# DerekRowell/AudioSDR

Hardware: AMD Instinct MI355X
Metric: Msamples/s through full SSB demod chain, batched 128-sample blocks (higher is better)
Workload: dtype f32

## Files before the change

audiosdr_amd/binding.py:

```python
import ctypes as C
import os

import numpy as np

BLOCK = 128
ALL = -1
STREAM_BATCH = (1 << 64) - 1
LSBmode, USBmode, CW_LSBmode, CW_USBmode, AMmode, SAMmode, WSPRmode = range(7)
(audioAM, audioCW, audioWSPR, audio2100, audio2300, audio2500, audio2700, audio2900, audio3100, audio3300,
 audioBypass) = range(11)
AGCoff, AGCfast, AGCmedium, AGCslow = range(4)
TAPS = ["SCALED_I", "SCALED_Q", "NB_I", "NB_Q", "IF_I", "IF_Q", "MIX_I", "MIX_Q", "DEMOD", "AUDIO_FILT", "AGC", "ALS"]

_HERE = os.path.dirname(os.path.abspath(__file__))


class AsdrError(RuntimeError):
    pass


def library_path():
    return os.path.join(_HERE, "libasdr_hip.so")


def library_sha256(path=None):
    import hashlib
    with open(path or library_path(), "rb") as f:
        return hashlib.sha256(f.read()).hexdigest()


_f, _i, _u = C.c_float, C.c_int, C.c_uint
_SETTERS_VOID = ["init", "enableAudioFilter", "disableAudioFilter", "enableALSfilter", "disableALSfilter",
                 "setALSfilterNotch", "setALSfilterPeak", "setALSfilterAdaptive", "setALSfilterStatic", "enableAGC",
                 "disableAGC", "enableNoiseBlanker", "disableNoiseBlanker"]
_SETTERS_F = ["setInputGain", "setIQgainBalance", "setOutputGain", "setAGCthreshold", "setAGCslope", "setAGCkneeWidth",
              "setAGCattackTime", "setAGCreleaseTime", "setAGChangTime", "setAGCstaticGain", "setNoiseBlankerThreshold",
              "setNoiseBlankerThresholdDb"]
_SETTERS_I = ["setMute", "setAudioFilter", "setAGCmode"]
_GETTERS_F = ["getTuningOffset", "getBPFlower", "getBPFupper", "getAGCthreshold", "getAGCslope", "getAGCkneeWidth",
              "getAGCattack", "getAGCrelease", "getAAGalphaAttack", "getAGCbetaAttack", "getAGCalphaRelease",
              "getAGCbetaRelease", "getAGCstaticGain", "getAMcarrierLevel", "getSAMfrequency"]
_GETTERS_I = ["getMute", "getAudioFilter", "ALSfilterIsEnabled", "ALSfilterIsNotch", "ALSfilterIsPeak",
              "ALSfilterIsAdaptive", "AGCisEnabled", "AGCisActive", "NoiseBlankerisEnabled", "NoiseBlankerDetection",
              "getSAMphaseLockStatus"]

EXPORTS = (["asdr_create", "asdr_destroy", "asdr_last_error", "asdr_n_channels", "asdr_update", "asdr_update_device",
            "asdr_synchronize", "asdr_setDemodMode", "asdr_getDemodMode", "asdr_setALSfilterParams", "asdr_getAGClookup",
            "asdr_read_status", "asdr_control_plane_flush", "asdr_params_uniform_groups", "asdr_get_chain_constants", "asdr_stream_pipeline_launches", "asdr_schedule_layout", "asdr_set_exact_unknown_mode", "asdr_get_exact_unknown_mode", "asdr_stream_pipeline_recoveries", "asdr_stream_pipeline_max_groups", "asdr_set_stream_fir_helpers", "asdr_stream_pipeline_h3_calls", "asdr_set_stream_pipeline", "asdr_set_sam_launch_form", "asdr_set_als_launch_form", "asdr_debug_set_stream_spin_limit", "asdr_debug_set_stream_max_groups", "asdr_enable_taps", "asdr_read_taps", "asdr_last_kernel_ms", "asdr_version",
            "asdr_kernel_timing_begin", "asdr_kernel_timing_end", "asdr_set_launch_timing", "asdr_region_timing_begin", "asdr_region_timing_end", "asdr_update_device_strided", "asdr_capture_open",
            "asdr_capture_close", "asdr_capture_capacity", "asdr_capture_position", "asdr_capture_rewind",
            "asdr_capture_device_ptr", "asdr_capture_update_device", "asdr_capture_read",
            "asdr_create_sharded", "asdr_n_shards", "asdr_shard", "asdr_shard_first_channel", "asdr_shard_device",
            "asdr_host_alloc", "asdr_host_free", "asdr_host_register", "asdr_host_unregister", "asdr_set_host_chunks",
            "asdr_host_path_info", "asdr_stream_pipeline_alloc_failures", "asdr_set_launch_split", "asdr_order_after", "asdr_order_before", "asdr_lane_calls", "asdr_sam_role_calls", "asdr_sam_chunk_calls", "asdr_als_role_calls", "asdr_set_lanes"] +
           ["asdr_" + n for n in _SETTERS_VOID + _SETTERS_F + _SETTERS_I + _GETTERS_F + _GETTERS_I])

_lib = None


def host_autopin(on=-1):
    return int(load_library().asdr_host_autopin(int(on)))


def host_autopin_clear():
    load_library().asdr_host_autopin_clear()


def host_autopin_info():
    out = (C.c_long * 4)()
    load_library().asdr_host_autopin_info(out)
    return {"registered_now": int(out[0]), "registrations": int(out[1]), "released": int(out[2]), "refused": int(out[3])}


def kernels_launched(reset=False):
    L = load_library()
    out = {}
    for i in range(L.asdr_kernels_count()):
        n = int(L.asdr_kernels_launches(i))
        if n:
            out[L.asdr_kernels_name(i).decode()] = n
    if reset:
        L.asdr_kernels_launches_reset()
    return out


def load_library(path=None):
    global _lib
    if _lib is not None and path is None:
        return _lib
    p = path or library_path()
    if not os.path.exists(p):
        raise AsdrError("%s not found: build it with `python -m audiosdr_amd.build` (hipcc, gfx950). "
                        "There is no CPU fallback." % p)
    L = C.CDLL(p)
    vp, i16p = C.c_void_p, C.POINTER(C.c_int16)
    L.asdr_create.argtypes = [_i, _i]; L.asdr_create.restype = vp
    L.asdr_destroy.argtypes = [vp]; L.asdr_destroy.restype = None
    L.asdr_last_error.restype = C.c_char_p
    L.asdr_version.restype = C.c_char_p
    L.asdr_set_pool_priority.argtypes = [_i]; L.asdr_set_pool_priority.restype = _i
    L.asdr_host_autopin.argtypes = [_i]; L.asdr_host_autopin.restype = _i
    L.asdr_host_autopin_clear.restype = None
    L.asdr_host_autopin_info.argtypes = [C.POINTER(C.c_long)]; L.asdr_host_autopin_info.restype = _i
    L.asdr_kernels_count.restype = _i
    L.asdr_kernels_name.argtypes = [_i]; L.asdr_kernels_name.restype = C.c_char_p
    L.asdr_kernels_launches.argtypes = [_i]; L.asdr_kernels_launches.restype = C.c_ulonglong
    L.asdr_kernels_launches_reset.restype = None
    L.asdr_n_channels.argtypes = [vp]; L.asdr_n_channels.restype = _i
    L.asdr_update.argtypes = [vp, i16p, i16p, i16p, _i]; L.asdr_update.restype = _i
    L.asdr_update_device.argtypes = [vp, vp, vp, vp, _i, vp]; L.asdr_update_device.restype = _i
    L.asdr_synchronize.argtypes = [vp]; L.asdr_synchronize.restype = _i
    L.asdr_update_device_strided.argtypes = [vp, vp, vp, vp, _i, C.c_long, C.c_long, vp]; L.asdr_update_device_strided.restype = _i
    L.asdr_capture_open.argtypes = [vp, C.c_long]; L.asdr_capture_open.restype = _i
    for n in ("asdr_capture_close", "asdr_capture_rewind"):
        getattr(L, n).argtypes = [vp]; getattr(L, n).restype = _i
    for n in ("asdr_capture_capacity", "asdr_capture_position"):
        getattr(L, n).argtypes = [vp]; getattr(L, n).restype = C.c_long
    L.asdr_capture_device_ptr.argtypes = [vp]; L.asdr_capture_device_ptr.restype = vp
    L.asdr_capture_update_device.argtypes = [vp, vp, vp, _i, C.c_long, vp]; L.asdr_capture_update_device.restype = _i
    L.asdr_capture_read.argtypes = [vp, _i, C.c_long, C.c_long, i16p]; L.asdr_capture_read.restype = _i
    L.asdr_last_kernel_ms.argtypes = [vp]; L.asdr_last_kernel_ms.restype = _f
    for n in _SETTERS_VOID:
        fn = getattr(L, "asdr_" + n); fn.argtypes = [vp, _i]; fn.restype = None
    for n in _SETTERS_F:
        fn = getattr(L, "asdr_" + n); fn.argtypes = [vp, _i, _f]; fn.restype = None
    for n in _SETTERS_I:
        fn = getattr(L, "asdr_" + n); fn.argtypes = [vp, _i, _i]; fn.restype = None
    for n in _GETTERS_F:
        fn = getattr(L, "asdr_" + n); fn.argtypes = [vp, _i]; fn.restype = _f
    for n in _GETTERS_I:
        fn = getattr(L, "asdr_" + n); fn.argtypes = [vp, _i]; fn.restype = _i
    L.asdr_setDemodMode.argtypes = [vp, _i, _i]; L.asdr_setDemodMode.restype = _f
    L.asdr_getDemodMode.argtypes = [vp, _i]; L.asdr_getDemodMode.restype = C.c_int16
    L.asdr_setALSfilterParams.argtypes = [vp, _i, _u, _f, _f]; L.asdr_setALSfilterParams.restype = None
    L.asdr_getAGClookup.argtypes = [vp, _i, _i]; L.asdr_getAGClookup.restype = _f
    i32p, fp = C.POINTER(C.c_int32), C.POINTER(C.c_float)
    L.asdr_read_status.argtypes = [vp, i32p, i32p, i32p, fp, fp]; L.asdr_read_status.restype = _i
    if path is None or hasattr(L, "asdr_get_chain_constants"):
        L.asdr_get_chain_constants.argtypes = [vp, _i, C.POINTER(C.c_float)]; L.asdr_get_chain_constants.restype = C.c_uint
    if path is None or hasattr(L, "asdr_control_plane_flush"):
        L.asdr_control_plane_flush.argtypes = [vp, C.POINTER(C.c_longlong)]; L.asdr_control_plane_flush.restype = _i
    if path is None or hasattr(L, "asdr_params_uniform_groups"):
        L.asdr_params_uniform_groups.argtypes = [vp, C.POINTER(C.c_long)]; L.asdr_params_uniform_groups.restype = _i
    L.asdr_enable_taps.argtypes = [vp, _i]; L.asdr_enable_taps.restype = _i
    L.asdr_read_taps.argtypes = [vp, fp]; L.asdr_read_taps.restype = _i
    L.asdr_kernel_timing_begin.argtypes = [vp, _i]; L.asdr_kernel_timing_begin.restype = _i
    if path is None or hasattr(L, "asdr_stream_pipeline_launches"):
        L.asdr_stream_pipeline_launches.argtypes = [vp]; L.asdr_stream_pipeline_launches.restype = C.c_long
    if path is None or hasattr(L, "asdr_set_stream_pipeline"):
        L.asdr_stream_pipeline_recoveries.argtypes = [vp]; L.asdr_stream_pipeline_recoveries.restype = C.c_long
        L.asdr_stream_pipeline_max_groups.argtypes = [vp]; L.asdr_stream_pipeline_max_groups.restype = _i
        if hasattr(L, "asdr_set_stream_fir_helpers"):
            L.asdr_set_stream_fir_helpers.argtypes = [vp, _i]; L.asdr_set_stream_fir_helpers.restype = _i
            L.asdr_stream_pipeline_h3_calls.argtypes = [vp]; L.asdr_stream_pipeline_h3_calls.restype = C.c_long
        L.asdr_set_stream_pipeline.argtypes = [vp, _i]; L.asdr_set_stream_pipeline.restype = _i
        L.asdr_set_sam_launch_form.argtypes = [vp, _i, _i]; L.asdr_set_sam_launch_form.restype = _i
        if hasattr(L, "asdr_set_als_launch_form"):
            L.asdr_set_als_launch_form.argtypes = [vp, _i]; L.asdr_set_als_launch_form.restype = _i
        L.asdr_debug_set_stream_spin_limit.argtypes = [vp, _u]; L.asdr_debug_set_stream_spin_limit.restype = _i
        L.asdr_debug_set_stream_max_groups.argtypes = [vp, _i]; L.asdr_debug_set_stream_max_groups.restype = _i
    if path is None or hasattr(L, "asdr_set_exact_unknown_mode"):
        L.asdr_set_exact_unknown_mode.argtypes = [vp, _i]; L.asdr_set_exact_unknown_mode.restype = _i
        L.asdr_get_exact_unknown_mode.argtypes = [vp]; L.asdr_get_exact_unknown_mode.restype = _i
    if path is None or hasattr(L, "asdr_schedule_layout"):
        L.asdr_schedule_layout.argtypes = [vp, C.POINTER(C.c_int)]; L.asdr_schedule_layout.restype = _i
    if path is None or hasattr(L, "asdr_region_timing_begin"):
        L.asdr_set_launch_timing.argtypes = [vp, _i]; L.asdr_set_launch_timing.restype = _i
        L.asdr_region_timing_begin.argtypes = [vp, vp]; L.asdr_region_timing_begin.restype = _i
        L.asdr_region_timing_end.argtypes = [vp, C.POINTER(C.c_float), C.POINTER(C.c_long)]; L.asdr_region_timing_end.restype = _i
    L.asdr_kernel_timing_end.argtypes = [vp, fp, _i]; L.asdr_kernel_timing_end.restype = _i
    if path is None or hasattr(L, "asdr_create_sharded"):
        L.asdr_create_sharded.argtypes = [_i, _i, C.POINTER(C.c_int)]; L.asdr_create_sharded.restype = vp
        L.asdr_n_shards.argtypes = [vp]; L.asdr_n_shards.restype = _i
        L.asdr_shard.argtypes = [vp, _i]; L.asdr_shard.restype = vp
        L.asdr_shard_first_channel.argtypes = [vp, _i]; L.asdr_shard_first_channel.restype = _i
        L.asdr_shard_device.argtypes = [vp, _i]; L.asdr_shard_device.restype = _i
        L.asdr_host_alloc.argtypes = [C.c_size_t]; L.asdr_host_alloc.restype = vp
        L.asdr_host_free.argtypes = [vp]; L.asdr_host_free.restype = None
        L.asdr_host_register.argtypes = [vp, C.c_size_t]; L.asdr_host_register.restype = _i
        L.asdr_host_unregister.argtypes = [vp]; L.asdr_host_unregister.restype = _i
        L.asdr_set_host_chunks.argtypes = [vp, _i]; L.asdr_set_host_chunks.restype = _i
        L.asdr_host_path_info.argtypes = [vp, C.POINTER(C.c_int)]; L.asdr_host_path_info.restype = _i
        L.asdr_stream_pipeline_alloc_failures.argtypes = [vp]; L.asdr_stream_pipeline_alloc_failures.restype = C.c_long
        L.asdr_set_launch_split.argtypes = [vp, _i, _i]; L.asdr_set_launch_split.restype = _i
        L.asdr_order_after.argtypes = [vp, vp]; L.asdr_order_after.restype = _i
        L.asdr_order_before.argtypes = [vp, vp]; L.asdr_order_before.restype = _i
        L.asdr_lane_calls.argtypes = [vp]; L.asdr_lane_calls.restype = C.c_long
        L.asdr_sam_role_calls.argtypes = [vp]; L.asdr_sam_role_calls.restype = C.c_long
        L.asdr_als_role_calls.argtypes = [vp]; L.asdr_als_role_calls.restype = C.c_long
        L.asdr_sam_chunk_calls.argtypes = [vp]; L.asdr_sam_chunk_calls.restype = C.c_long
        L.asdr_set_lanes.argtypes = [vp, _i, _i]; L.asdr_set_lanes.restype = _i
    if path is None or hasattr(L, "asdr_lanes_overlap_probe"):
        L.asdr_lanes_overlap_probe.argtypes = [vp]; L.asdr_lanes_overlap_probe.restype = _i
        L.asdr_lanes_enabled.argtypes = [vp]; L.asdr_lanes_enabled.restype = _i
        L.asdr_stream_pipeline_headroom_refusals.argtypes = [vp]; L.asdr_stream_pipeline_headroom_refusals.restype = C.c_long
    if path is None:
        _lib = L
    return L


class AudioSDRBatch:

    def __init__(self, n_channels, device=0, devices=None, _handle=None, _owner=None):
        self._L = load_library()
        self._owner = _owner
        if _handle is not None:
            self._h = _handle
        elif devices is not None:
            devs = (C.c_int * len(devices))(*[int(d) for d in devices])
            self._h = self._L.asdr_create_sharded(int(n_channels), len(devices), devs)
        else:
            self._h = self._L.asdr_create(int(n_channels), int(device))
        if not self._h:
            raise AsdrError("asdr_create failed: " + self._L.asdr_last_error().decode())
        self.n_channels = int(n_channels)
        self.device = int(device) if devices is None else None

    def close(self):
        if getattr(self, "_h", None):
            if self._owner is None:
                self._L.asdr_destroy(self._h)
            self._h = None

    @property
    def n_shards(self):
        return int(self._L.asdr_n_shards(self._h))

    def shard(self, g):
        h = self._L.asdr_shard(self._h, int(g))
        if not h:
            raise AsdrError("no such shard")
        lo, hi = self.shard_range(g)
        v = AudioSDRBatch(hi - lo, device=self._L.asdr_shard_device(self._h, int(g)), _handle=h, _owner=self)
        return v

    def shard_range(self, g):
        return int(self._L.asdr_shard_first_channel(self._h, int(g))), int(self._L.asdr_shard_first_channel(self._h, int(g) + 1))

    def order_after(self, stream):
        self._chk(self._L.asdr_order_after(self._h, C.c_void_p(stream)))

    def order_before(self, stream):
        self._chk(self._L.asdr_order_before(self._h, C.c_void_p(stream)))

    def lane_calls(self):
        return int(self._L.asdr_lane_calls(self._h))

    def sam_role_calls(self):
        return int(self._L.asdr_sam_role_calls(self._h))

    def sam_chunk_calls(self):
        return int(self._L.asdr_sam_chunk_calls(self._h))

    def als_role_calls(self):
        return int(self._L.asdr_als_role_calls(self._h))

    def lanes_overlap_probe(self):
        return int(self._L.asdr_lanes_overlap_probe(self._h))

    def lanes_enabled(self):
        return bool(self._L.asdr_lanes_enabled(self._h))

    def stream_pipeline_headroom_refusals(self):
        return int(self._L.asdr_stream_pipeline_headroom_refusals(self._h))

    def set_lanes(self, on=True, min_waves=0):
        self._chk(self._L.asdr_set_lanes(self._h, 1 if on else 0, int(min_waves)))

    def set_launch_split(self, pieces, min_waves=0):
        self._chk(self._L.asdr_set_launch_split(self._h, int(pieces), int(min_waves)))

    def set_host_chunks(self, chunks):
        self._chk(self._L.asdr_set_host_chunks(self._h, int(chunks)))

    def host_path_info(self):
        out = (C.c_int * 2)()
        self._chk(self._L.asdr_host_path_info(self._h, out))
        return {"chunks": int(out[0]), "pinned": bool(out[1])}

    def stream_pipeline_alloc_failures(self):
        return int(self._L.asdr_stream_pipeline_alloc_failures(self._h))

    def update_into(self, I, Q, out):
        n_blocks = I.size // (self.n_channels * BLOCK)
        p = C.POINTER(C.c_int16)
        self._chk(self._L.asdr_update(self._h, I.ctypes.data_as(p), Q.ctypes.data_as(p), out.ctypes.data_as(p), n_blocks))
        return out

    def __del__(self):
        try:
            self.close()
        except Exception:
            pass

    def _chk(self, rc):
        if rc != 0:
            raise AsdrError(self._L.asdr_last_error().decode())

    def update(self, I, Q):
        I = np.ascontiguousarray(I, dtype=np.int16)
        Q = np.ascontiguousarray(Q, dtype=np.int16)
        assert I.shape == Q.shape and I.size % (self.n_channels * BLOCK) == 0
        n_blocks = I.size // (self.n_channels * BLOCK)
        out = np.empty((self.n_channels, n_blocks, BLOCK), dtype=np.int16)
        p = C.POINTER(C.c_int16)
        self._chk(self._L.asdr_update(self._h, I.ctypes.data_as(p), Q.ctypes.data_as(p), out.ctypes.data_as(p), n_blocks))
        return out

    def update_device(self, dI, dQ, dOut, n_blocks, stream=0):
        self._chk(self._L.asdr_update_device(self._h, C.c_void_p(dI), C.c_void_p(dQ), C.c_void_p(dOut), int(n_blocks),
                                             C.c_void_p(stream)))

    def update_device_strided(self, dI, dQ, dOut, n_blocks, in_stride_blocks, out_stride_blocks, stream=0):
        self._chk(self._L.asdr_update_device_strided(self._h, C.c_void_p(dI), C.c_void_p(dQ), C.c_void_p(dOut), int(n_blocks),
                                                     int(in_stride_blocks), int(out_stride_blocks), C.c_void_p(stream)))

    def synchronize(self):
        self._chk(self._L.asdr_synchronize(self._h))

    def capture_open(self, capacity_blocks):
        self._chk(self._L.asdr_capture_open(self._h, int(capacity_blocks)))

    def capture_close(self):
        self._chk(self._L.asdr_capture_close(self._h))

    def capture_rewind(self):
        self._chk(self._L.asdr_capture_rewind(self._h))

    @property
    def capture_position(self):
        return int(self._L.asdr_capture_position(self._h))

    @property
    def capture_capacity(self):
        return int(self._L.asdr_capture_capacity(self._h))

    def capture_device_ptr(self):
        return int(self._L.asdr_capture_device_ptr(self._h) or 0)

    def capture_update_device(self, dI, dQ, n_blocks, in_stride_blocks=None, stream=0):
        self._chk(self._L.asdr_capture_update_device(self._h, C.c_void_p(dI), C.c_void_p(dQ), int(n_blocks),
                                                     int(n_blocks if in_stride_blocks is None else in_stride_blocks), C.c_void_p(stream)))

    def capture_read(self, ch, first_block=0, n_blocks=None):
        if n_blocks is None:
            n_blocks = self.capture_position - first_block
        out = np.empty(int(n_blocks) * BLOCK, dtype=np.int16)
        self._chk(self._L.asdr_capture_read(self._h, int(ch), int(first_block), int(n_blocks), out.ctypes.data_as(C.POINTER(C.c_int16))))
# ... 165 lines not shown
```

audiosdr_amd/csrc/asdr_device.h:

```cpp
#ifndef ASDR_DEVICE_H_
#define ASDR_DEVICE_H_

#include <stdint.h>

#define ASDR_N 128
#define ASDR_PLL_WRAP_MAX 64

#define ASDR_F_NB_EN        (1u << 0)
#define ASDR_F_AF_EN        (1u << 1)
#define ASDR_F_AGC_EN       (1u << 2)
#define ASDR_F_ALS_EN       (1u << 3)
#define ASDR_F_ALS_NOTCH    (1u << 4)
#define ASDR_F_ALS_ADAPTIVE (1u << 5)
#define ASDR_F_MUTED        (1u << 6)

#define ASDR_R_IF   (1u << 0)
#define ASDR_R_AF   (1u << 1)
#define ASDR_R_NB   (1u << 2)
#define ASDR_R_ALS  (1u << 3)
#define ASDR_R_IMG  (1u << 4)
#define ASDR_R_ALL  (1u << 5)

typedef struct {
  uint32_t mode;
// ... 31 lines not shown
} ChanSmall;

#define ASDR_S_AGC_ACTIVE  (1u << 0)
#define ASDR_S_NB_DETECTED (1u << 1)
#define ASDR_S_PLL_LOCKED  (1u << 2)

#define ASDR_NB_MASK_ROW 160
#define ASDR_NB_MASK_USED 138
#define ASDR_AGC_TAB_ROW 132

typedef struct {
  double inv_two_pi_d;
  double sin_index_scale_d;
  double half_pi_d;
  float if_center;
  float two_pi_f;
  float half_pi_f;
  float phase_inc_unit;
  float nb_alpha, nb_beta;
  float pll_b0, pll_b1, pll_a1;
  float pll_alpha_freq, pll_beta_freq, pll_f_conv, pll_lock_lo, pll_lock_hi;
} ChainConsts;

typedef struct {
  int32_t ch;
  uint32_t mode, flags;
  uint32_t lo;
} SlotInfo;
#define ASDR_LO_ENTRIES 8
#define ASDR_LO_WRITER 0x100u
#define ASDR_LO_WRITER_LANE(l) (0x100u << (l))

typedef struct {
  uint32_t key_phase, key_inc;
  float phase_end;
  uint32_t pad_;
  float c[ASDR_N], s[ASDR_N];
} LoEntry;

typedef struct {
  const ChanParams *params;
  ChanSmall *small;
  int16_t *nb_hist;
  uint8_t *nb_mask;
  float *hil_q, *hil_i, *als_x, *als_w;
  float *audio_prev;
  const float *agc_tab;
  const SlotInfo *sched;
  int32_t n_sched;
  int32_t n_channels;
  const int16_t *in_i, *in_q;
  int16_t *out;
  int32_t n_blocks;
  uint32_t nb_phase;
  uint32_t als_phase;
  LoEntry *lo_cache;
  uint32_t lo_parity;
  uint32_t lo_write;
  uint32_t lo_writer_bit;
  uint32_t direct_lo;
  int32_t direct_ch0;
  uint32_t direct_mode, direct_flags;
  int32_t in_stride;
  int32_t out_stride;
  float *taps;
  float *xch_a;
  float *xch_b;
  float *xch_c;
  uint32_t *stream_prog;
  uint32_t *stream_err;
  uint32_t stream_spin_limit;
  const uint32_t *run_if;
  int32_t stream_waves;
  float *xch_sam;
  uint32_t *sam_lock;
  uint32_t sam_set, sam_sets;
  uint32_t sam_set_stride, sam_lock_stride;
  float *als_stage;
  uint32_t als_stage_cur, als_stage_prev;
  LoEntry *lo_ring;
  ChainConsts k;
  ChanParams uni;
  uint32_t uni_valid;
  uint32_t pad_uni_;
} UpdateArgs;
#define ASDR_ALS_STAGE_SLOTS 32
#define ASDR_ALS_CHUNK 8
#define ASDR_STREAM_DEPTH 4
#define ASDR_LO_RING 8
#define ASDR_STREAM_SPIN_LIMIT (1u << 18)
#define ASDR_STREAM_FAIL 0xFFFFFFFFu
#define ASDR_SNAP_BYTES (448 + 1536 + ASDR_NB_MASK_ROW + 1024 + 1024 + 512)

#define ASDR_KERNEL_PLAIN 0
#define ASDR_KERNEL_SAM 1
#define ASDR_KERNEL_ALS 2
#define ASDR_KERNEL_ALS_SMALL 3
#define ASDR_KERNEL_SAM_ALS 4
#define ASDR_KERNEL_KINDS 5
#ifndef ASDR_SAM_WAVES
#define ASDR_SAM_WAVES 4
#endif

#endif
```

audiosdr_amd/csrc/asdr_host.cpp:

```cpp
#include <hip/hip_runtime.h>

#include <algorithm>
#include <atomic>
#include <chrono>
#include <condition_variable>
#include <functional>
#include <memory>
#include <mutex>
#include <thread>
#include <cmath>
#include <cstdio>
#include <cstring>
#include <string>
#include <unordered_map>
#include <vector>

#include "../../include/asdr.h"
#include "asdr_device.h"
#include "asdr_tables.h"

#ifndef ASDR_SAM_CHUNK
#define ASDR_SAM_CHUNK 8
#define ASDR_SAM_CHUNK_SETS 32
#define ASDR_SAM_CHUNK_MAX_WAVES 512
#endif
#ifndef ASDR_ALS_ROLE_MAX_WAVES
#define ASDR_ALS_ROLE_MAX_WAVES 512
#endif
#ifndef ASDR_PER_BLOCK_LAUNCH_WAVES
#define ASDR_PER_BLOCK_LAUNCH_WAVES 1024
#endif
#ifndef ASDR_STREAM_MAX_WAVES
#define ASDR_STREAM_MAX_WAVES 1024
#endif
#ifndef ASDR_STREAM_MIN_BLOCKS
#define ASDR_STREAM_MIN_BLOCKS 8
#endif
#ifndef ASDR_STREAM_SIDE_MARGIN
#define ASDR_STREAM_SIDE_MARGIN 16
#endif
#ifndef ASDR_STREAM_SIDE_WAVES
#define ASDR_STREAM_SIDE_WAVES 64
#endif
extern "C" int asdr_launch_stream(const UpdateArgs *a, hipStream_t stream, int fir_helpers);
extern "C" int asdr_stream_capacity(int device, int *compute_units, int fir_helpers);
extern "C" int asdr_launch_stream_snapshot(const UpdateArgs *a, void *snap, int restore, hipStream_t stream);
extern "C" int asdr_launch_stream_ack(uint32_t *err, hipStream_t stream);
extern "C" int asdr_kernels_upload_tables(void);
namespace { void autopin_batch_created(); void autopin_batch_gone(); }
extern "C" int asdr_launch_update(const UpdateArgs *a, int variant, int uniform, hipStream_t stream);
extern "C" int asdr_launch_sam_role(const UpdateArgs *a, int variant, int uniform, int role, hipStream_t stream);
extern "C" int asdr_launch_als_role(const UpdateArgs *a, int role, hipStream_t stream);
extern "C" int asdr_launch_als_stage_seed(const UpdateArgs *a, int ch0, int n, hipStream_t stream);
extern "C" int asdr_launch_reset(const UpdateArgs *a, const uint32_t *d_reset_bits, int first_row, int n_rows, hipStream_t stream);

namespace {

constexpr double kPI = 3.1415926535897932384626433832795;
constexpr float kFs = 44100.0f;
constexpr float kIFcenter = 6890.0f, kBWssb = 3000.0f, kBWcw = 1000.0f, kBWwspr = 1000.0f, kBWam = 8500.0f;

thread_local std::string g_err;
int fail(const std::string &m) { g_err = m; return -1; }
#define HIPCHK(expr)                                                                                   \
  do {                                                                                                 \
    hipError_t e_ = (expr);                                                                            \
    if (e_ != hipSuccess) return fail(std::string(#expr) + ": " + hipGetErrorString(e_));              \
  } while (0)

struct Chan {
  float in_gain = 1.0f, in_gain_i = 1.0f, in_gain_q = 1.0f, gain_balance = 1.0f;
  float output_gain = 0.5f, out_gain = 1.0f, current_out_gain = 1.0f;
  float freq_shift = 0.0f;
  uint16_t mode = 0;
  bool muted = true;
  int16_t current_filter = 0;
  bool af_en = false;
  int if_table = ASDR_TBL_IF_SSB, audio_table = ASDR_TBL_AUDIO_BASE + ASDR_audio2700;
  int16_t als_m = 55, als_delay = 3;
  float als_lambda = 0.5f;
  bool als_en = false, als_notch = true, als_adaptive = true;
  float agc_alpha_att = 0, agc_beta_att = 0, agc_alpha_rel = 0, agc_beta_rel = 0;
  float agc_attack_ms = 0, agc_release_ms = 0, agc_knee = 0, agc_slope = 0, agc_threshold = 0;
  float agc_static_gain = 10.0f;
  float agc_slot129 = 100.0f;
  uint32_t agc_hang_count = 0;
  bool agc_en = true;
  int agc_table = -1;
  float nb_threshold = 1.2f;
  bool nb_en = true;
};

struct AgcTable {
  float thr, slope, knee;
  float v[ASDR_AGC_TAB_ROW];
};

float log2_approx(float input) {
  int exponent;
  float mantissa = frexpf(fabsf(input), &exponent);
  return (((1.23149591368684f * mantissa - 4.11852516267426f) * mantissa + 6.02197014179219f) * mantissa -
          3.13396450166353f) + exponent;
}

void build_agc_table(AgcTable &t) {
  const float thr = t.thr, slope = t.slope, knee = t.knee;
  const float lin_lo = expf((float)(2.3025 * ((double)thr - (double)knee / 2.0) / 20.0));
  const float lin_hi = expf((float)(2.3025 * ((double)thr + (double)knee / 2.0) / 20.0));
  for (int i = 0; i < 130; i++) {
    const float input = (float)((double)(float)i / 128.0);
    const float in_db = (float)(6.026 * (double)log2_approx(input));
    if (input < lin_lo) {
      t.v[i] = 1.0f;
    } else if (input > lin_hi) {
      const float out_db = thr + (in_db - thr) * slope;
      t.v[i] = expf((float)(2.3025 * (double)(out_db - in_db) / 20.0));
    } else {
      const double u = (double)(in_db - thr) + (double)knee / 2.0;
      const float out_db = (float)((double)in_db + (((double)slope - 1.0) * u * u) / (2.0 * (double)knee));
      t.v[i] = expf((float)(2.3025 * (double)(out_db - in_db) / 20.0));
    }
  }
  t.v[130] = t.v[131] = 0.0f;
}

float time_constant(float ms) {
  return (float)exp(log(0.1) / ((double)(kFs * ms) / 1000.0));
}

}

namespace {
class CopyPool {
// ... 77 lines not shown
  size_t agc_tab_cap = 0;
  SlotInfo *d_sched = nullptr;
  uint32_t *d_reset = nullptr;
  int16_t *d_io[3] = {nullptr, nullptr, nullptr};
  int16_t *h_io[3] = {nullptr, nullptr, nullptr};
  size_t h_io_cap = 0;
  hipStream_t h2d_stream = nullptr, d2h_stream = nullptr;
  std::vector<hipEvent_t> ev_host;
  HostPlan host_plan;
  std::unique_ptr<CopyPool> copy_pool;
  int host_chunks_forced = 0;
  hipStream_t lane[ASDR_LANES + 1] = {};
  hipEvent_t ev_lane[ASDR_LANES + 1] = {};
  int n_lanes = 2, n_lanes_sam = 3;
  int sched_lanes = 2;
  bool lanes_pending = false;
  bool sched_sam_heavy = false;
  bool last_was_lanes = false;
  int lanes_min_waves = 1024;
  bool lanes_enabled = true;
  bool lanes_forced = false;
  long stat_lane_calls = 0;
  int launch_split = 1, launch_split_min_waves = 2048;
  int stat_host_chunks = 0, stat_host_pinned = 0;
  std::vector<asdr_batch *> shards;
  std::vector<int> shard_first;
  void *workers = nullptr;
  int16_t *d_capture = nullptr;
  long capture_cap = 0, capture_pos = 0;
  size_t io_cap = 0;
  bool taps_on = false;
  hipEvent_t ev0 = nullptr, ev1 = nullptr;
  bool ev_valid = false;
  bool time_calls = false;
  hipEvent_t rev0 = nullptr, rev1 = nullptr;
  hipStream_t region_stream = nullptr;
  bool region_on_lanes = false;
  long region_calls = -1;
  std::vector<hipEvent_t> tev;
  size_t tev_used = 0;
  hipStream_t last_stream = nullptr;
  hipEvent_t ev_last = nullptr;
  hipStream_t aux[ASDR_AUX_STREAMS] = {};
  hipEvent_t ev_fork = nullptr, ev_join[ASDR_AUX_STREAMS] = {};
  bool ev_last_valid = false;
  LoEntry *d_lo = nullptr;
  float *d_xch_a = nullptr, *d_xch_b = nullptr;
  uint32_t *d_stream_prog = nullptr;
  LoEntry *d_lo_ring = nullptr;
  bool sam_fused = false;
  int sam_split_min = 512;
  bool stream_pipeline = true;
  int stream_query_waves = 0;
  int stream_max_waves = 0;
  int stream_cap_workgroups = 0;
  int stream_cap_h3 = 0, stream_cus = 0;
  int stream_h3 = -1;
  long stat_stream_h3_calls = 0;
  uint32_t stream_spin_limit = ASDR_STREAM_SPIN_LIMIT;
  void *d_stream_snap = nullptr;
  long stat_stream_recoveries = 0;
  bool sam_split = false;
  int als_split_min = 0x7fffffff;
  bool als_split = false;
  float *d_xch_sam = nullptr;
  size_t xch_sam_slots = 0;
  hipEvent_t ev_role[6] = {};
  bool sam_role_streams = true;
  long stat_sam_role_calls = 0;
  float *d_xch_sam_chunk = nullptr; size_t xch_sam_chunk_slots = 0;
  long stat_sam_chunk_calls = 0;
  hipEvent_t ev_samc[3 * (ASDR_SAM_CHUNK_SETS / ASDR_SAM_CHUNK)] = {};
  float *d_als_stage = nullptr;
  hipEvent_t ev_als[3 * (ASDR_ALS_STAGE_SLOTS / ASDR_ALS_CHUNK)] = {};
  int als_role_stages = 3;
  bool als_role_streams = true;
  long stat_als_role_calls = 0;
  bool plain_uniform_ssb = false;
  bool stream_launched = false;
  long stat_stream_launches = 0;
  long stat_stream_headroom_refusals = 0;
  long stat_stream_alloc_failures = 0;
  uint32_t lo_parity = 0;
  uint32_t nb_phase = 0;
  uint32_t als_phase = 0;
  ChainConsts k{};
};

namespace {

int sharded_update(asdr_batch *b, const int16_t *I, const int16_t *Q, int16_t *out, int n_blocks);
void shard_workers_stop(asdr_batch *b);
inline bool is_sharded(const asdr_batch *b);

uint64_t agc_hash(float thr, float slope, float knee) {
  uint32_t a, b2, c;
  memcpy(&a, &thr, 4); memcpy(&b2, &slope, 4); memcpy(&c, &knee, 4);
  uint64_t h = 1469598103934665603ull;
  for (uint32_t w : {a, b2, c}) { h ^= w; h *= 1099511628211ull; }
  return h;
}

int find_agc_table(asdr_batch *b, float thr, float slope, float knee) {
  std::vector<int> &bucket = b->agc_index[agc_hash(thr, slope, knee)];
  for (int i : bucket) {
    const AgcTable &t = b->agc_pool[i];
    if (memcmp(&t.thr, &thr, 4) == 0 && memcmp(&t.slope, &slope, 4) == 0 && memcmp(&t.knee, &knee, 4) == 0) return i;
  }
  AgcTable t;
  t.thr = thr; t.slope = slope; t.knee = knee;
  build_agc_table(t);
  b->agc_pool.push_back(t);
  b->agc_refs.push_back(0);
  bucket.push_back((int)b->agc_pool.size() - 1);
  b->agc_pool_dirty = true;
  return (int)b->agc_pool.size() - 1;
}

void rebuild_agc(asdr_batch *b, Chan &c) {
  const int old = c.agc_table;
  c.agc_table = find_agc_table(b, c.agc_threshold, c.agc_slope, c.agc_knee);
  b->agc_refs[c.agc_table]++;
  b->agc_refs_changed = true;
  if (old >= 0 && old < (int)b->agc_refs.size() && b->agc_refs[old] > 0) b->agc_refs[old]--;
  c.agc_slot129 = b->agc_pool[c.agc_table].v[129];
}

void compact_agc_pool(asdr_batch *b) {
  if (!b->agc_refs_changed) return;
  b->agc_refs_changed = false;
  size_t live = 0;
  for (uint32_t r : b->agc_refs) live += (r != 0);
  if (b->agc_pool.size() < 64 || b->agc_pool.size() <= 2 * live) return;
  std::vector<int> remap(b->agc_pool.size(), -1);
  std::vector<AgcTable> pool;
  std::vector<uint32_t> refs;
  for (size_t i = 0; i < b->agc_pool.size(); i++)
    if (b->agc_refs[i]) { remap[i] = (int)pool.size(); pool.push_back(b->agc_pool[i]); refs.push_back(b->agc_refs[i]); }
  b->agc_pool.swap(pool); b->agc_refs.swap(refs);
  b->agc_index.clear();
  for (size_t i = 0; i < b->agc_pool.size(); i++) b->agc_index[agc_hash(b->agc_pool[i].thr, b->agc_pool[i].slope, b->agc_pool[i].knee)].push_back((int)i);
  for (Chan &c : b->ch) c.agc_table = remap[c.agc_table];
  b->agc_pool_dirty = true; b->all_dirty = true; b->sched_dirty = true;
}

void mark_reset(asdr_batch *b, int i, uint32_t bits) {
  b->reset[i] |= bits;
  b->reset_pending = true;
  if (i < b->reset_lo) b->reset_lo = i;
  if (i > b->reset_hi) b->reset_hi = i;
}

float set_mode(asdr_batch *b, int idx, int new_mode) {
  Chan &c = b->ch[idx];
  c.mode = (uint16_t)new_mode;
  int tbl = -1;
  if (c.mode == ASDR_USBmode) { c.freq_shift = (float)((double)kIFcenter - (double)kBWssb / 2.0); tbl = ASDR_TBL_IF_SSB; }
  else if (c.mode == ASDR_LSBmode) { c.freq_shift = (float)((double)kIFcenter + (double)kBWssb / 2.0); tbl = ASDR_TBL_IF_SSB; }
  else if (c.mode == ASDR_WSPRmode) { c.freq_shift = (float)((double)kIFcenter - (double)kBWssb / 2.0); tbl = ASDR_TBL_IF_WSPR; }
  else if (c.mode == ASDR_CW_USBmode) { c.freq_shift = (float)((double)kIFcenter - (double)kBWcw / 2.0); tbl = ASDR_TBL_IF_CW; }
  else if (c.mode == ASDR_CW_LSBmode) { c.freq_shift = (float)((double)kIFcenter + (double)kBWcw / 2.0); tbl = ASDR_TBL_IF_CW; }
  else if (c.mode == ASDR_AMmode || c.mode == ASDR_SAMmode) { c.freq_shift = kIFcenter; tbl = ASDR_TBL_IF_AM; }
  if (tbl >= 0) { c.if_table = tbl; mark_reset(b, idx, ASDR_R_IF); }
  return c.freq_shift;
}

// ... 384 lines not shown
    ok = ok && hipStreamSynchronize(s0) == hipSuccess && hipStreamSynchronize(s1) == hipSuccess;
    ok = ok && hipEventElapsedTime(&one, ev[0], ev[1]) == hipSuccess && hipEventElapsedTime(&both, ev[0], ev[2]) == hipSuccess;
    if (!ok) break;
    rounds++;
    if (std::max(one, both) < 1.5f * alone) votes++;
  }
  for (hipEvent_t e : ev) if (e) (void)hipEventDestroy(e);
  if (!ok || rounds == 0) { (void)hipGetLastError(); return -1; }
  const int verdict = (2 * votes > rounds) ? 1 : 0;
  g_lanes_probe_last[device] = verdict;
  if (verdict == 1 || ++g_lanes_probe_tries[device] >= 3) g_lanes_probe[device] = verdict;
  return verdict;
}
hipStream_t aux_stream(asdr_batch *b, int i) {
  if (!b->aux[i]) b->aux[i] = pool_stream(b->device, i + 1);
  return b->aux[i];
}
hipStream_t lane_stream(asdr_batch *b, int l) {
  if (!b->lane[l]) b->lane[l] = pool_stream(b->device, l);
  return b->lane[l];
}
bool needs_flush(const asdr_batch *b) {
  return b->all_dirty || !b->dirty.empty() || b->sched_dirty || b->agc_pool_dirty || b->reset_pending || b->agc_refs_changed;
}
int lanes_join_into(asdr_batch *b, hipStream_t stream) {
  for (int i = 0; i <= b->sched_lanes; i++) {
    const int l = (i == b->sched_lanes) ? ASDR_LANES : i;
    if (!b->lane[l]) continue;
    HIPCHK(hipEventRecord(b->ev_lane[l], b->lane[l])); HIPCHK(hipStreamWaitEvent(stream, b->ev_lane[l], 0));
  }
  return 0;
}
int sync_all(asdr_batch *b) {
  HIPCHK(hipStreamSynchronize(b->last_stream));
  HIPCHK(hipStreamSynchronize(b->stream));
  if (b->lanes_pending) { for (int l = 0; l < ASDR_LANES + 1; l++) if (b->lane[l]) HIPCHK(hipStreamSynchronize(b->lane[l])); b->lanes_pending = false; }

  return 0;
}

int check_stream_error(asdr_batch *b) {
  if (!b->stream_launched || !b->d_stream_prog) return 0;
  if (sync_all(b) != 0) return -1;
  uint32_t *word = b->d_stream_prog + 3 * ((b->n + 7) / 8) + 1, v[2] = {0, 0};
  HIPCHK(hipMemcpy(v, word, sizeof v, hipMemcpyDeviceToHost));
  b->stream_launched = false;
  b->stat_stream_recoveries = (long)v[1];
  if (v[0]) return fail("streaming pipeline: error word still set after the recovery launches (internal error)");
  return 0;
}

int read_small(asdr_batch *b, int ch, ChanSmall &s) {
  if (!b || ch < 0 || ch >= b->n) return fail("bad channel");
  if (is_sharded(b)) b = shard_of(b, ch);
  if (b->device == ASDR_NO_DEVICE) return fail("control-plane-only batch has no device state");
  HIPCHK(hipSetDevice(b->device));
  if (sync_all(b) != 0) return -1;
  if (check_stream_error(b) != 0) return -1;
  if (apply_resets(b, b->stream) != 0) return -1;
  HIPCHK(hipMemcpy(&s, b->d_small + ch, sizeof s, hipMemcpyDeviceToHost));
  return 0;
}

}

#define FOR_SHARDS(b, call) do { if (is_sharded(b)) { for (asdr_batch *sh_ : (b)->shards) { const int rc_ = (call); if (rc_ != 0) return rc_; } return 0; } } while (0)

extern "C" {

const char *asdr_last_error(void) { return g_err.c_str(); }
}
int asdr_internal_fail(const std::string &m) { return fail(m); }
extern "C" {
const char *asdr_version(void) { return "asdr-hip 0.1 (gfx950, wave64, -ffp-contract=off)"; }

asdr_batch_t *asdr_create(int n_channels, int device) {
  if (n_channels <= 0 || n_channels > (1 << 20)) { fail("n_channels must be in 1..1048576"); return nullptr; }
  asdr_batch *b = new asdr_batch();
  b->n = n_channels; b->device = device;
  b->sam_fused = getenv("ASDR_SAM_FUSED") != nullptr;
  b->sam_split_min = getenv("ASDR_SAM_SPLIT_MIN") ? atoi(getenv("ASDR_SAM_SPLIT_MIN")) : ASDR_SAM_SPLIT_MIN_CHANNELS;
  b->stream_pipeline = getenv("ASDR_NO_STREAM_PIPELINE") == nullptr;
  b->uniform_params = getenv("ASDR_NO_UNIFORM_PARAMS") == nullptr;
  b->als_split_min = getenv("ASDR_ALS_SPLIT_MIN") ? atoi(getenv("ASDR_ALS_SPLIT_MIN")) : 0x7fffffff;
  if (getenv("ASDR_LAUNCH_SPLIT")) b->launch_split = std::max(1, std::min(atoi(getenv("ASDR_LAUNCH_SPLIT")), 8));
  if (getenv("ASDR_LAUNCH_SPLIT_MIN_WAVES")) b->launch_split_min_waves = std::max(8, atoi(getenv("ASDR_LAUNCH_SPLIT_MIN_WAVES")));
  const size_t rows = (size_t)n_channels + 1;
  if (device != ASDR_NO_DEVICE) {
    int ndev = 0;
    if (hipGetDeviceCount(&ndev) != hipSuccess || ndev <= 0) { delete b; fail("no HIP device: libasdr_hip has no CPU path"); return nullptr; }
    if (device < 0 || device >= ndev) { delete b; fail("bad device ordinal"); return nullptr; }
    if (device >= 16) { delete b; fail("device ordinal >= 16: the per-device stream pool of this library has 16 entries"); return nullptr; }
    if (hipSetDevice(device) != hipSuccess) { delete b; fail("hipSetDevice failed"); return nullptr; }
    autopin_batch_created();
    bool ok = true;
    auto alloc = [&](void **p, size_t bytes) { if (ok && hipMalloc(p, bytes) != hipSuccess) ok = false; };
    alloc((void **)&b->d_params, rows * sizeof(ChanParams));
    alloc((void **)&b->d_small, rows * sizeof(ChanSmall));
    alloc((void **)&b->d_nb_hist, rows * 768 * sizeof(int16_t));
    alloc((void **)&b->d_nb_mask, rows * ASDR_NB_MASK_ROW * sizeof(uint8_t));
    alloc((void **)&b->d_hil_q, rows * 256 * sizeof(float));
    alloc((void **)&b->d_hil_i, rows * 256 * sizeof(float));
    alloc((void **)&b->d_als_x, rows * 256 * sizeof(float));
    alloc((void **)&b->d_als_w, rows * 128 * sizeof(float));
    alloc((void **)&b->d_audio_prev, rows * 128 * sizeof(float));
    if (ok && hipMemset(b->d_audio_prev, 0, rows * 128 * sizeof(float)) != hipSuccess) ok = false;
    alloc((void **)&b->d_sched, (rows + 32) * sizeof(SlotInfo));
    alloc((void **)&b->d_reset, rows * sizeof(uint32_t));
    alloc((void **)&b->d_lo, (1 + ASDR_LANES) * 2 * ASDR_LO_ENTRIES * sizeof(LoEntry));
    if (ok && hipMemset(b->d_lo, 0xFF, (1 + ASDR_LANES) * 2 * ASDR_LO_ENTRIES * sizeof(LoEntry)) != hipSuccess) ok = false;
    if (ok && hipStreamSynchronize(nullptr) != hipSuccess) ok = false;
    for (int i = 0; i < ASDR_LANES + 1 && ok; i++)
      if (hipEventCreateWithFlags(&b->ev_lane[i], hipEventDisableTiming) != hipSuccess) ok = false;
    b->lanes_enabled = getenv("ASDR_NO_LANES") == nullptr;
    b->sam_role_streams = getenv("ASDR_NO_SAM_ROLE_STREAMS") == nullptr;
    b->als_role_streams = getenv("ASDR_NO_ALS_ROLE_STREAMS") == nullptr;
    if (getenv("ASDR_ALS_ROLE_STAGES")) b->als_role_stages = atoi(getenv("ASDR_ALS_ROLE_STAGES")) == 2 ? 2 : 3;
    if (ok && (b->stream = pool_stream(device, 0)) == nullptr) ok = false;
    if (ok && hipEventCreate(&b->ev0) != hipSuccess) ok = false;
    if (ok && hipEventCreate(&b->ev1) != hipSuccess) ok = false;
    if (ok && hipEventCreate(&b->rev0) != hipSuccess) ok = false;
    if (ok && hipEventCreate(&b->rev1) != hipSuccess) ok = false;
    if (ok && hipEventCreateWithFlags(&b->ev_last, hipEventDisableTiming) != hipSuccess) ok = false;
    if (ok && hipEventCreateWithFlags(&b->ev_fork, hipEventDisableTiming) != hipSuccess) ok = false;
    for (int i = 0; i < ASDR_AUX_STREAMS && ok; i++)
      if (hipEventCreateWithFlags(&b->ev_join[i], hipEventDisableTiming) != hipSuccess) ok = false;
    if (ok && asdr_kernels_upload_tables() != 0) ok = false;
    if (ok) {
      int cus = 0;
      const int cap = asdr_stream_capacity(device, &cus, 1);
      const int cap3 = asdr_stream_capacity(device, nullptr, 3);
      b->stream_cap_h3 = cap3 > 0 ? cap3 : 0; b->stream_cus = cus;
      { const char *e = getenv("ASDR_STREAM_H3"); if (e) b->stream_h3 = atoi(e) != 0 ? 1 : 0; }
      b->stream_cap_workgroups = cap > 0 ? cap : 0;
      b->stream_max_waves = cap >= 3 ? cap / 3 : 0;
      if (b->stream_max_waves > ASDR_STREAM_MAX_WAVES) b->stream_max_waves = ASDR_STREAM_MAX_WAVES;
      b->stream_query_waves = b->stream_max_waves;
    }
    if (!ok) { fail("device allocation / table upload failed"); asdr_destroy(b); return nullptr; }
  }

  ChainConsts &k = b->k;
  k.if_center = kIFcenter;
  k.two_pi_f = (float)(2.0 * kPI);
  k.half_pi_f = (float)(0.5 * kPI);
  k.inv_two_pi_d = 1.0 / (double)k.two_pi_f;
  k.sin_index_scale_d = (65535.0 / (double)k.two_pi_f) * (1.0 + 0x1p-49);
  k.half_pi_d = kPI / 2.0;
  k.phase_inc_unit = k.two_pi_f / kFs;
  k.nb_alpha = 0.995f;
  k.nb_beta = (float)(1.0 - (double)k.nb_alpha);
  {
    const float wn = 0.07f, zeta = 0.707f, Ka = 1000.f;
    const float tau1 = Ka / (wn * wn);
    const float tau2 = 2 * zeta / wn;
    k.pll_b0 = (float)((double)(2 * Ka / tau1) * (1.0 + 2.0 * (double)tau2));
    k.pll_b1 = (float)((double)(2 * Ka / tau1) * (1.0 - 2.0 * (double)tau2));
    k.pll_a1 = -1.0f;
  }
  k.pll_alpha_freq = 0.995f;
  k.pll_beta_freq = (float)(1.0 - (double)k.pll_alpha_freq);
  k.pll_f_conv = kFs / k.two_pi_f;
  k.pll_lock_lo = (float)((double)kIFcenter - 1000.0);
  k.pll_lock_hi = (float)((double)kIFcenter + 1000.0);

  b->ch.assign(rows, Chan());
// ... 165 lines not shown
  {
    const uintptr_t in_bytes = ((uintptr_t)(b->n - 1) * (uintptr_t)in_stride_blocks + (uintptr_t)n_blocks) * ASDR_N * sizeof(int16_t);
    const uintptr_t out_bytes = ((uintptr_t)(b->n - 1) * (uintptr_t)out_stride_blocks + (uintptr_t)n_blocks) * ASDR_N * sizeof(int16_t);
    const uintptr_t o0 = (uintptr_t)dOut, o1 = o0 + out_bytes;
    for (uintptr_t i0 : {(uintptr_t)dI, (uintptr_t)dQ}) io_alias = io_alias || (o0 < i0 + in_bytes && i0 < o1);
  }
  int pipe_sub = -1, other_waves = 0;
  for (int i = 0; i < n_sub; i++) { if (subs[i].kind == ASDR_KERNEL_PLAIN && subs[i].uniform) pipe_sub = i; else other_waves += subs[i].slots / 8; }
  bool take_pipeline = parts == 1 && b->stream_pipeline && !io_alias && n_blocks >= ASDR_STREAM_MIN_BLOCKS && pipe_sub >= 0 && b->plain_uniform_ssb &&
                       other_waves <= ASDR_STREAM_SIDE_WAVES && !sam_split && !als_split &&
#ifndef ASDR_TIMELINE
                       !b->taps_on &&
#endif
                       subs[pipe_sub].slots / 8 <= b->stream_max_waves;
  if (take_pipeline && other_waves > 0 && b->stream_cap_workgroups > 0 &&
      3 * (subs[pipe_sub].slots / 8) + other_waves + ASDR_STREAM_SIDE_MARGIN > b->stream_cap_workgroups) { take_pipeline = false; b->stat_stream_headroom_refusals++; }
  if (take_pipeline) {
    if (!b->d_xch_a) {
      float *xa = nullptr, *xb = nullptr; uint32_t *prog = nullptr; LoEntry *ring = nullptr; void *snap = nullptr;
      const size_t n_prog = (size_t)(3 * ((b->n + 7) / 8) + 3);
      bool ok = hipMalloc(&xa, (size_t)(b->n + 1) * ASDR_STREAM_DEPTH * 2 * ASDR_N * sizeof(float)) == hipSuccess &&
                hipMalloc(&xb, (size_t)(b->n + 1) * ASDR_STREAM_DEPTH * (ASDR_N + 1) * sizeof(float)) == hipSuccess &&
                hipMalloc(&prog, n_prog * sizeof(uint32_t)) == hipSuccess &&
                hipMalloc(&ring, ASDR_LO_RING * sizeof(LoEntry)) == hipSuccess &&
                hipMalloc(&snap, (size_t)(((b->n + 7) / 8) * 8) * ASDR_SNAP_BYTES) == hipSuccess &&
                hipMemsetAsync(prog, 0, n_prog * sizeof(uint32_t), stream) == hipSuccess;
      if (!ok) {
        for (void *p : {(void *)xa, (void *)xb, (void *)prog, (void *)ring, snap}) if (p) hipFree(p);
        (void)hipGetLastError();
        b->stream_pipeline = false; b->stat_stream_alloc_failures++; take_pipeline = false;
      } else {
        b->d_xch_a = xa; b->d_xch_b = xb; b->d_stream_prog = prog; b->d_lo_ring = ring; b->d_stream_snap = snap;
      }
    }
  }
  if (take_pipeline) {
    const UpdateArgs a_side = a;
    const int w = subs[pipe_sub].slots / 8;
    HIPCHK(hipMemsetAsync(b->d_stream_prog, 0, (size_t)(3 * w + 1) * sizeof(uint32_t), stream));
    if (n_sub > 1) HIPCHK(hipEventRecord(b->ev_fork, stream));
    a.sched = b->d_sched + subs[pipe_sub].first; a.n_sched = subs[pipe_sub].slots;
    a.direct_ch0 = -1; a.uni_valid = 0u;
    if (b->kind_direct[ASDR_KERNEL_PLAIN]) { const SlotInfo &s0 = b->sched[subs[pipe_sub].first]; a.direct_ch0 = s0.ch; a.direct_mode = s0.mode; a.direct_flags = s0.flags; a.direct_lo = s0.lo; set_uni(b, a, s0.ch); }
    a.lo_write = 0u;
    a.xch_a = b->d_xch_a; a.xch_b = b->d_xch_b; a.xch_c = b->d_xch_b + (size_t)(b->n + 1) * ASDR_STREAM_DEPTH * ASDR_N; a.stream_prog = b->d_stream_prog; a.stream_err = b->d_stream_prog + 3 * ((b->n + 7) / 8) + 1;
    a.stream_waves = w; a.lo_ring = b->d_lo_ring; a.stream_spin_limit = b->stream_spin_limit;
    if (e0) HIPCHK(hipEventRecord(e0, stream));
    if (asdr_launch_stream_snapshot(&a, b->d_stream_snap, 0, stream) != 0) return fail("stream snapshot launch failed");
    const bool h3 = b->stream_h3 != 0 && b->stream_cap_h3 > 0 && 3 * w + other_waves + ASDR_STREAM_SIDE_MARGIN <= b->stream_cap_h3 &&
                    (b->stream_h3 == 1 || 3 * w <= b->stream_cus);
    if (h3) b->stat_stream_h3_calls++;
    if (asdr_launch_stream(&a, stream, h3 ? 3 : 1) != 0) return fail("stream kernel launch failed");
    if (asdr_launch_stream_snapshot(&a, b->d_stream_snap, 1, stream) != 0) return fail("stream restore launch failed");
    {
      UpdateArgs f = a;
      f.run_if = a.stream_err; f.stream_waves = 0; f.xch_a = nullptr; f.xch_b = nullptr; f.xch_c = nullptr; f.stream_prog = nullptr; f.lo_ring = nullptr;
      if (asdr_launch_update(&f, ASDR_KERNEL_PLAIN, 1, stream) != 0) return fail("stream fallback launch failed");
    }
    if (asdr_launch_stream_ack(a.stream_err, stream) != 0) return fail("stream acknowledge launch failed");
    {
      int n_aux = 0;
      for (int i = 0; i < n_sub; i++) {
        if (i == pipe_sub) continue;
        hipStream_t s = aux_stream(b, n_aux++);
        if (!s) return fail("stream creation failed");
        HIPCHK(hipStreamWaitEvent(s, b->ev_fork, 0));
        UpdateArgs o = a_side;
        o.sched = b->d_sched + subs[i].first; o.n_sched = subs[i].slots; o.direct_ch0 = -1; o.uni_valid = 0u; o.lo_write = 1u;
        if (subs[i].uniform && b->kind_direct[subs[i].kind]) { const SlotInfo &s0 = b->sched[subs[i].first]; o.direct_ch0 = s0.ch; o.direct_mode = s0.mode; o.direct_flags = s0.flags; o.direct_lo = s0.lo; set_uni(b, o, s0.ch); }
        if (asdr_launch_update(&o, subs[i].kind, subs[i].uniform, s) != 0) return fail("update kernel launch failed");
        HIPCHK(hipEventRecord(b->ev_join[n_aux - 1], s));
      }
      for (int j = 0; j < n_aux; j++) HIPCHK(hipStreamWaitEvent(stream, b->ev_join[j], 0));
    }
    if (e1) HIPCHK(hipEventRecord(e1, stream));
    b->stream_launched = true; b->stat_stream_launches++;
    b->ev_last_valid = true;
    b->ev_valid = (e0 != nullptr && e0 == b->ev0);
    if (b->region_calls >= 0) b->region_calls++;
    b->last_stream = stream; b->last_was_lanes = false;
    b->nb_phase = (b->nb_phase + (uint32_t)(n_blocks % 3)) % 3u;
    b->als_phase = (b->als_phase + (uint32_t)n_blocks) & 1u;
    b->lo_parity ^= 1u;
    return 0;
  }
  const int n_launch = per_block ? n_blocks : 1;
  float *const taps = a.taps;
  if (e0 && part == 0) HIPCHK(hipEventRecord(e0, stream));
  if (use_lanes) {
    if (batch_stream) {
      if (b->ev_last_valid && !b->last_was_lanes) {
        HIPCHK(hipEventRecord(b->ev_last, b->last_stream));
        for (int i = 0; i <= b->sched_lanes; i++) { hipStream_t ls = lane_stream(b, i == b->sched_lanes ? ASDR_LANES : i); if (!ls) return fail("stream creation failed"); HIPCHK(hipStreamWaitEvent(ls, b->ev_last, 0)); }
      }
    } else {
      HIPCHK(hipEventRecord(b->ev_fork, stream));
      for (int i = 0; i <= b->sched_lanes; i++) { hipStream_t ls = lane_stream(b, i == b->sched_lanes ? ASDR_LANES : i); if (!ls) return fail("stream creation failed"); HIPCHK(hipStreamWaitEvent(ls, b->ev_fork, 0)); }
    }
    const int NL = b->sched_lanes;
    for (int l = 0; l <= NL; l++) {
      hipStream_t ls = lane_stream(b, (l == NL) ? ASDR_LANES : l);
      if (!ls) return fail("stream creation failed");
      for (int lb = 0; lb < n_launch; lb++) {
        for (int i = 0; i < n_sub; i++) {
          const Sub &su = subs[i];
          const long w = su.slots / 8;
          int lo = (int)(w * l / NL) * 8, cnt = (int)(w * (l + 1) / NL) * 8 - lo;
          if (l == NL) { lo = 0; cnt = su.uniform ? 0 : su.slots; } else if (!su.uniform) cnt = 0;
          const int first = su.first + lo;
          if (cnt == 0) continue;
          UpdateArgs al = a;
          al.sched = b->d_sched + first; al.n_sched = cnt;
          al.direct_ch0 = -1; al.uni_valid = 0u;
          if (su.uniform && b->kind_direct[su.kind]) { const SlotInfo &s0 = b->sched[su.first]; al.direct_ch0 = s0.ch + lo; al.direct_mode = s0.mode; al.direct_flags = s0.flags; al.direct_lo = s0.lo; set_uni(b, al, s0.ch); }
          al.lo_cache = b->d_lo + (size_t)(1 + (l % ASDR_LANES)) * 2 * ASDR_LO_ENTRIES;
          al.lo_write = 1u;
          al.lo_writer_bit = ASDR_LO_WRITER_LANE(l % ASDR_LANES);
          if (sam_split && (su.kind == ASDR_KERNEL_SAM || su.kind == ASDR_KERNEL_SAM_ALS)) set_sam_rows(al, su.kind, first, 0);
          const int form = (als_split && su.kind == ASDR_KERNEL_ALS_SMALL && su.uniform) ? 2 : su.uniform;
          if (per_block) {
            al.in_i = dI + (size_t)lb * ASDR_N; al.in_q = dQ + (size_t)lb * ASDR_N; al.out = dOut + (size_t)lb * ASDR_N; al.n_blocks = 1;
            al.nb_phase = (b->nb_phase + (uint32_t)(lb % 3)) % 3u;
            al.als_phase = (b->als_phase + (uint32_t)lb) & 1u;
            al.lo_parity = b->lo_parity ^ (uint32_t)(lb & 1);
          }
          if (asdr_launch_update(&al, su.kind, form, ls) != 0) return fail("update kernel launch failed");
        }
      }
    }
    if (!batch_stream) { if (lanes_join_into(b, stream) != 0) return -1; b->lanes_pending = false; b->last_was_lanes = false; b->last_stream = stream; }
    else { b->lanes_pending = true; b->last_was_lanes = true; }
    b->ev_last_valid = true; b->ev_valid = false; b->stat_lane_calls++;
    if (b->region_calls >= 0) b->region_calls++;
    b->nb_phase = (b->nb_phase + (uint32_t)(n_blocks % 3)) % 3u;
    b->als_phase = (b->als_phase + (uint32_t)n_blocks) & 1u;
    b->lo_parity ^= (uint32_t)(n_launch & 1);
    return 0;
  }
  struct Item { int sub, first, slots; };
  Item items[ASDR_AUX_STREAMS + 1]; int n_items = 0;
  for (int i = 0; i < n_sub; i++) {
    const long w = subs[i].slots / 8;
    const int lo = (int)(w * part / parts) * 8, cnt = (int)(w * (part + 1) / parts) * 8 - lo;
    if (cnt == 0) continue;
    int pieces = 1;
    if (b->launch_split > 1 && cnt / 8 >= b->launch_split_min_waves) pieces = std::min(b->launch_split, ASDR_AUX_STREAMS + 1 - n_items - (n_sub - 1 - i));
    if (pieces < 1) pieces = 1;
    for (int q = 0; q < pieces; q++) {
      const int qlo = (int)((long)(cnt / 8) * q / pieces) * 8, qhi = (int)((long)(cnt / 8) * (q + 1) / pieces) * 8;
      if (qhi > qlo && n_items < ASDR_AUX_STREAMS + 1) items[n_items++] = Item{i, subs[i].first + lo + qlo, qhi - qlo};
    }
  }
  int main_item = 0;
  for (int i = 1; i < n_items; i++) if (items[i].slots > items[main_item].slots) main_item = i;
  const bool sam_roles = b->sam_role_streams && per_block && n_launch >= 2 && parts == 1 && n_items == 1 && taps == nullptr && sam_split &&
                         (subs[items[0].sub].kind == ASDR_KERNEL_SAM || subs[items[0].sub].kind == ASDR_KERNEL_SAM_ALS);
  hipStream_t s_pre = nullptr, s_pll = nullptr;
  if (sam_roles) {
    s_pre = aux_stream(b, 0); s_pll = aux_stream(b, 1);
    if (!s_pre || !s_pll) return fail("stream creation failed");
    for (int i = 0; i < 6; i++) if (!b->ev_role[i]) HIPCHK(hipEventCreateWithFlags(&b->ev_role[i], hipEventDisableTiming));
    HIPCHK(hipEventRecord(b->ev_fork, stream));
    HIPCHK(hipStreamWaitEvent(s_pre, b->ev_fork, 0)); HIPCHK(hipStreamWaitEvent(s_pll, b->ev_fork, 0));
    b->stat_sam_role_calls++;
  }
  bool sam_chunks = sam_roles && subs[items[0].sub].kind == ASDR_KERNEL_SAM && subs[items[0].sub].uniform && n_blocks >= 2 * ASDR_SAM_CHUNK &&
                    items[0].slots <= 8 * ASDR_SAM_CHUNK_MAX_WAVES && getenv("ASDR_NO_SAM_CHUNKS") == nullptr;
  auto chunk_tiles = [&](int slots) -> bool {
    if ((size_t)slots <= b->xch_sam_chunk_slots) return true;
    if (hipStreamSynchronize(stream) != hipSuccess) return false;
    float *grown = nullptr;
    const size_t per_set = (size_t)slots * 2 * ASDR_N * sizeof(float) + (size_t)slots * sizeof(uint32_t);
    if (hipMalloc(&grown, ASDR_SAM_CHUNK_SETS * per_set) != hipSuccess) { (void)hipGetLastError(); return false; }
    if (b->d_xch_sam_chunk) hipFree(b->d_xch_sam_chunk);
    b->d_xch_sam_chunk = grown; b->xch_sam_chunk_slots = (size_t)slots;
    return true;
  };
  if (sam_chunks && !chunk_tiles(items[0].slots)) sam_chunks = false;
  int parity_launches_sam = -1;
  if (sam_chunks) {
    constexpr int S = ASDR_SAM_CHUNK_SETS, G = ASDR_SAM_CHUNK, R = S / G;
    static_assert(S % G == 0 && R >= 4, "tile sets for four chunks");
    for (int i = 0; i < 3 * R; i++) if (!b->ev_samc[i]) HIPCHK(hipEventCreateWithFlags(&b->ev_samc[i], hipEventDisableTiming));
    const int i0 = items[0].sub, first0 = items[0].first;
    const size_t slots = b->xch_sam_chunk_slots;
    a.sched = b->d_sched + first0; a.n_sched = items[0].slots; a.direct_ch0 = -1; a.uni_valid = 0u; a.lo_write = 1u;
    if (b->kind_direct[subs[i0].kind]) { const SlotInfo &s0 = b->sched[subs[i0].first]; a.direct_ch0 = s0.ch; a.direct_mode = s0.mode; a.direct_flags = s0.flags; a.direct_lo = s0.lo; set_uni(b, a, s0.ch); }
    a.xch_sam = b->d_xch_sam_chunk; a.sam_lock = reinterpret_cast<uint32_t *>(b->d_xch_sam_chunk + (size_t)S * slots * 2 * ASDR_N);
    a.sam_sets = (uint32_t)S; a.sam_set_stride = (uint32_t)(slots * 2 * ASDR_N); a.sam_lock_stride = (uint32_t)slots;
    a.taps = nullptr;
    const int n_chunks = (n_blocks + G - 1) / G;
    auto chunk_args = [&](int k) {
      const int b0 = k * G, g = (n_blocks - b0 < G) ? n_blocks - b0 : G;
      a.in_i = dI + (size_t)b0 * ASDR_N; a.in_q = dQ + (size_t)b0 * ASDR_N; a.out = dOut + (size_t)b0 * ASDR_N; a.n_blocks = g;
      a.nb_phase = (b->nb_phase + (uint32_t)(b0 % 3)) % 3u;
      a.als_phase = (b->als_phase + (uint32_t)b0) & 1u;
      a.lo_parity = b->lo_parity ^ (uint32_t)(k & 1);
      a.sam_set = (uint32_t)(b0 % S);
    };
    for (int k = 0; k <= n_chunks; k++) {
      if (k < n_chunks) {
        const int kr = k % R;
        chunk_args(k);
        if (asdr_launch_sam_role(&a, ASDR_KERNEL_SAM, 1, 0, stream) != 0) return fail("update kernel launch failed");
        HIPCHK(hipEventRecord(b->ev_samc[kr], stream)); HIPCHK(hipStreamWaitEvent(s_pll, b->ev_samc[kr], 0));
        if (asdr_launch_sam_role(&a, ASDR_KERNEL_SAM, 1, 1, s_pll) != 0) return fail("update kernel launch failed");
        HIPCHK(hipEventRecord(b->ev_samc[R + kr], s_pll));
      }
      if (k >= 1) {
        chunk_args(k - 1);
        HIPCHK(hipStreamWaitEvent(stream, b->ev_samc[R + (k - 1) % R], 0));
        if (asdr_launch_sam_role(&a, ASDR_KERNEL_SAM, 1, 2, stream) != 0) return fail("update kernel launch failed");
      }
    }
    parity_launches_sam = n_chunks;
    b->stat_sam_chunk_calls++;
  }
  const bool als_role_call = als_roles && n_items == 1 && taps == nullptr;
  int parity_launches = n_launch;
  if (als_role_call) {
    constexpr int S = ASDR_ALS_STAGE_SLOTS, G = ASDR_ALS_CHUNK, R = S / G;
    static_assert(S % G == 0 && R >= 3, "the stage holds at least three chunks");
    hipStream_t s_chain = aux_stream(b, 0);
    if (!s_chain) return fail("stream creation failed");
    for (int i = 0; i < 2 * R; i++) if (!b->ev_als[i]) HIPCHK(hipEventCreateWithFlags(&b->ev_als[i], hipEventDisableTiming));
    HIPCHK(hipEventRecord(b->ev_fork, stream));
    HIPCHK(hipStreamWaitEvent(s_chain, b->ev_fork, 0));
    const int i0 = items[0].sub, first0 = items[0].first;
    a.sched = b->d_sched + first0; a.n_sched = items[0].slots; a.direct_ch0 = -1; a.uni_valid = 0u; a.lo_write = 1u;
    if (b->kind_direct[subs[i0].kind]) { const SlotInfo &s0 = b->sched[subs[i0].first]; a.direct_ch0 = s0.ch; a.direct_mode = s0.mode; a.direct_flags = s0.flags; a.direct_lo = s0.lo; set_uni(b, a, s0.ch); }
    a.als_stage = b->d_als_stage; a.als_stage_cur = 0u; a.als_stage_prev = (uint32_t)(S - 1); a.als_phase = b->als_phase;
    if (asdr_launch_als_stage_seed(&a, 0, b->n, s_chain) != 0) return fail("update kernel launch failed");
    const int n_chunks = (n_blocks + G - 1) / G;
    static_assert(ASDR_SAM_CHUNK == ASDR_ALS_CHUNK, "the two chunked forms share the tile sets");
    constexpr int RT = ASDR_SAM_CHUNK_SETS / G;
    static_assert(RT == R, "the front stage's wait indexes ev_als[(k - RT) % R]: the event of back chunk k - RT only while tile sets and stage slots hold the same number of chunks");
    hipStream_t s_front = nullptr;
    bool three = b->als_role_stages == 3 && chunk_tiles(items[0].slots);
    if (three) { s_front = aux_stream(b, 1); if (!s_front) three = false; }
    if (three) {
      for (int i = 2 * R; i < 3 * R; i++) if (!b->ev_als[i]) HIPCHK(hipEventCreateWithFlags(&b->ev_als[i], hipEventDisableTiming));
      HIPCHK(hipStreamWaitEvent(s_front, b->ev_fork, 0));
      const size_t slots = b->xch_sam_chunk_slots;
      a.xch_sam = b->d_xch_sam_chunk; a.sam_lock = reinterpret_cast<uint32_t *>(b->d_xch_sam_chunk + (size_t)ASDR_SAM_CHUNK_SETS * slots * 2 * ASDR_N);
      a.sam_sets = (uint32_t)ASDR_SAM_CHUNK_SETS; a.sam_set_stride = (uint32_t)(slots * 2 * ASDR_N); a.sam_lock_stride = (uint32_t)slots;
    }
    for (int k = 0; k < n_chunks; k++) {
      const int b0 = k * G, g = (n_blocks - b0 < G) ? n_blocks - b0 : G;
      a.in_i = dI + (size_t)b0 * ASDR_N; a.in_q = dQ + (size_t)b0 * ASDR_N; a.out = dOut + (size_t)b0 * ASDR_N; a.n_blocks = g;
      a.nb_phase = (b->nb_phase + (uint32_t)(b0 % 3)) % 3u;
      a.als_phase = (b->als_phase + (uint32_t)b0) & 1u;
      a.lo_parity = b->lo_parity ^ (uint32_t)(k & 1);
      a.als_stage_cur = (uint32_t)(b0 % S); a.als_stage_prev = (uint32_t)((b0 + S - 1) % S);
      a.sam_set = (uint32_t)(b0 % ASDR_SAM_CHUNK_SETS);
      if (three) {
        if (k >= RT) HIPCHK(hipStreamWaitEvent(s_front, b->ev_als[(k - RT) % R], 0));
        if (asdr_launch_als_role(&a, 2, s_front) != 0) return fail("update kernel launch failed");
        HIPCHK(hipEventRecord(b->ev_als[2 * R + k % R], s_front)); HIPCHK(hipStreamWaitEvent(s_chain, b->ev_als[2 * R + k % R], 0));
      }
      if (k >= R - 1) HIPCHK(hipStreamWaitEvent(s_chain, b->ev_als[R + (k + 1) % R], 0));
      if (asdr_launch_als_role(&a, three ? 3 : 0, s_chain) != 0) return fail("update kernel launch failed");
      HIPCHK(hipEventRecord(b->ev_als[k % R], s_chain)); HIPCHK(hipStreamWaitEvent(stream, b->ev_als[k % R], 0));
      if (asdr_launch_als_role(&a, 1, stream) != 0) return fail("update kernel launch failed");
      HIPCHK(hipEventRecord(b->ev_als[R + k % R], stream));
    }
    parity_launches = n_chunks;
    b->stat_als_role_calls++;
  }
  if (parity_launches_sam >= 0) parity_launches = parity_launches_sam;
  for (int lb = 0; lb < ((als_role_call || sam_chunks) ? 0 : n_launch); lb++) {
    if (per_block) {
      a.in_i = dI + (size_t)lb * ASDR_N; a.in_q = dQ + (size_t)lb * ASDR_N; a.out = dOut + (size_t)lb * ASDR_N; a.n_blocks = 1;
      a.nb_phase = (b->nb_phase + (uint32_t)(lb % 3)) % 3u;
      a.als_phase = (b->als_phase + (uint32_t)lb) & 1u;
      a.lo_parity = b->lo_parity ^ (uint32_t)(lb & 1);
      a.taps = (lb == n_launch - 1) ? taps : nullptr;
    }
    if (n_items > 1) HIPCHK(hipEventRecord(b->ev_fork, stream));
    int n_aux = 0;
    for (int it = 0; it < n_items; it++) {
      const int i = items[it].sub, first = items[it].first;
      hipStream_t s = (it == main_item) ? stream : aux_stream(b, n_aux++);
      if (!s && it != main_item) return fail("stream creation failed");
      if (it != main_item) HIPCHK(hipStreamWaitEvent(s, b->ev_fork, 0));
      a.sched = b->d_sched + first; a.n_sched = items[it].slots;
      a.direct_ch0 = -1; a.uni_valid = 0u;
      a.lo_write = 1u;
      if (subs[i].uniform && b->kind_direct[subs[i].kind]) {
        const SlotInfo &s0 = b->sched[subs[i].first];
        a.direct_ch0 = s0.ch + (first - subs[i].first); a.direct_mode = s0.mode; a.direct_flags = s0.flags; a.direct_lo = s0.lo; set_uni(b, a, s0.ch);
        if (first != subs[i].first) a.lo_write = 0u;
      }
      const bool sam3 = sam_split && (subs[i].kind == ASDR_KERNEL_SAM || subs[i].kind == ASDR_KERNEL_SAM_ALS);
      if (sam3) set_sam_rows(a, subs[i].kind, first, sam_roles ? (lb & 1) : 0);
      const int form = (als_split && subs[i].kind == ASDR_KERNEL_ALS_SMALL && subs[i].uniform) ? 2 : subs[i].uniform;
      if (sam_roles) {
        const int pa = lb & 1;
        if (lb >= 2) HIPCHK(hipStreamWaitEvent(s_pre, b->ev_role[4 + pa], 0));
        if (asdr_launch_sam_role(&a, subs[i].kind, form, 0, s_pre) != 0) return fail("update kernel launch failed");
        HIPCHK(hipEventRecord(b->ev_role[pa], s_pre)); HIPCHK(hipStreamWaitEvent(s_pll, b->ev_role[pa], 0));
        if (asdr_launch_sam_role(&a, subs[i].kind, form, 1, s_pll) != 0) return fail("update kernel launch failed");
        HIPCHK(hipEventRecord(b->ev_role[2 + pa], s_pll)); HIPCHK(hipStreamWaitEvent(stream, b->ev_role[2 + pa], 0));
        if (asdr_launch_sam_role(&a, subs[i].kind, form, 2, stream) != 0) return fail("update kernel launch failed");
        HIPCHK(hipEventRecord(b->ev_role[4 + pa], stream));
        continue;
      }
      if (asdr_launch_update(&a, subs[i].kind, form, s) != 0) return fail("update kernel launch failed");
      if (it != main_item) HIPCHK(hipEventRecord(b->ev_join[n_aux - 1], s));
    }
    for (int j = 0; j < n_aux; j++) HIPCHK(hipStreamWaitEvent(stream, b->ev_join[j], 0));
  }
  if (part + 1 < parts) return 0;
  if (e1) HIPCHK(hipEventRecord(e1, stream));
  b->ev_last_valid = true;
  b->ev_valid = (e0 != nullptr && e0 == b->ev0);
  if (b->region_calls >= 0) b->region_calls++;
  b->last_stream = stream; b->last_was_lanes = false;
  b->nb_phase = (b->nb_phase + (uint32_t)(n_blocks % 3)) % 3u;
  b->als_phase = (b->als_phase + (uint32_t)n_blocks) & 1u;
  b->lo_parity ^= (uint32_t)(parity_launches & 1);
  return 0;
}

extern "C" {
int asdr_update_device_strided(asdr_batch_t *b, const int16_t *dI, const int16_t *dQ, int16_t *dOut, int n_blocks,
                               long in_stride_blocks, long out_stride_blocks, void *stream_) {
  if (is_sharded(b)) {
    if (!dI || !dQ) return 0;
    if (!dOut) return fail("null output");
    for (asdr_batch *sh : b->shards) if (sh->device != b->shards[0]->device || sh->device == ASDR_NO_DEVICE)
      return fail("sharded batch over several devices: device pointers go to the shards (asdr_shard), host rows to asdr_update");
    for (size_t g = 0; g < b->shards.size(); g++) {
      const size_t f = (size_t)b->shard_first[g];
      if (update_device_part(b->shards[g], dI + f * (size_t)in_stride_blocks * ASDR_N, dQ + f * (size_t)in_stride_blocks * ASDR_N,
                             dOut + f * (size_t)out_stride_blocks * ASDR_N, n_blocks, in_stride_blocks, out_stride_blocks, stream_, 0, 1) != 0) return -1;
    }
    return 0;
  }
  return update_device_part(b, dI, dQ, dOut, n_blocks, in_stride_blocks, out_stride_blocks, stream_, 0, 1);
}

int asdr_update_device(asdr_batch_t *b, const int16_t *dI, const int16_t *dQ, int16_t *dOut, int n_blocks, void *stream_) {
  return asdr_update_device_strided(b, dI, dQ, dOut, n_blocks, n_blocks, n_blocks, stream_);
}

int asdr_capture_open(asdr_batch_t *b, long capacity_blocks) {
  if (!b) return fail("null batch");
  FOR_SHARDS(b, asdr_capture_open(sh_, capacity_blocks));
  if (b->device == ASDR_NO_DEVICE) return fail("control-plane-only batch (ASDR_NO_DEVICE): the capture sink lives in HBM");
  if (capacity_blocks <= 0 || capacity_blocks > 0x7fffffffL) return fail("bad capture capacity");
  HIPCHK(hipSetDevice(b->device));
  if (b->d_capture) { HIPCHK(hipDeviceSynchronize()); HIPCHK(hipFree(b->d_capture)); b->d_capture = nullptr; }
  const size_t bytes = (size_t)b->n * (size_t)capacity_blocks * ASDR_N * sizeof(int16_t);
  if (hipMalloc(&b->d_capture, bytes) != hipSuccess) { b->d_capture = nullptr; return fail("capture sink: out of device memory"); }
  b->capture_cap = capacity_blocks; b->capture_pos = 0;
  return 0;
}

int asdr_capture_close(asdr_batch_t *b) {
  if (!b) return fail("null batch");
  FOR_SHARDS(b, asdr_capture_close(sh_));
  if (b->d_capture) { HIPCHK(hipSetDevice(b->device)); HIPCHK(hipDeviceSynchronize()); HIPCHK(hipFree(b->d_capture)); }
  b->d_capture = nullptr; b->capture_cap = 0; b->capture_pos = 0;
  return 0;
}

long asdr_capture_capacity(const asdr_batch_t *b) { return b ? (is_sharded(b) ? b->shards[0]->capture_cap : b->capture_cap) : 0; }
long asdr_capture_position(const asdr_batch_t *b) { return b ? (is_sharded(b) ? b->shards[0]->capture_pos : b->capture_pos) : 0; }
int16_t *asdr_capture_device_ptr(asdr_batch_t *b) { return (b && !is_sharded(b)) ? b->d_capture : nullptr; }
int asdr_capture_rewind(asdr_batch_t *b) { if (!b) return fail("null batch"); FOR_SHARDS(b, asdr_capture_rewind(sh_)); b->capture_pos = 0; return 0; }

int asdr_capture_update_device(asdr_batch_t *b, const int16_t *dI, const int16_t *dQ, int n_blocks, long in_stride_blocks, void *stream) {
  if (!b) return fail("null batch");
  if (is_sharded(b)) {
    if (!dI || !dQ) return 0;
    for (asdr_batch *sh : b->shards) if (sh->device != b->shards[0]->device || sh->device == ASDR_NO_DEVICE)
      return fail("sharded batch over several devices: device pointers go to the shards (asdr_shard)");
    for (size_t g = 0; g < b->shards.size(); g++) {
      const size_t f = (size_t)b->shard_first[g] * (size_t)in_stride_blocks * ASDR_N;
      if (asdr_capture_update_device(b->shards[g], dI + f, dQ + f, n_blocks, in_stride_blocks, stream) != 0) return -1;
    }
    return 0;
  }
  if (!b->d_capture) return fail("capture sink is not open");
  if (!dI || !dQ) return 0;
  if (n_blocks <= 0) return 0;
  if (b->capture_pos + n_blocks > b->capture_cap) return fail("capture sink overflow");
  int16_t *dst = b->d_capture + (size_t)b->capture_pos * ASDR_N;
  if (asdr_update_device_strided(b, dI, dQ, dst, n_blocks, in_stride_blocks, b->capture_cap, stream) != 0) return -1;
  b->capture_pos += n_blocks;
  return 0;
}

int asdr_capture_read(asdr_batch_t *b, int ch, long first_block, long n_blocks, int16_t *host_out) {
  if (!b) return fail("null batch");
  if (is_sharded(b)) { asdr_batch *sh = shard_of(b, ch); if (!sh) return fail("bad channel"); return asdr_capture_read(sh, ch, first_block, n_blocks, host_out); }
  if (!b->d_capture) return fail("capture sink is not open");
  if (ch < 0 || ch >= b->n) return fail("bad channel");
  if (first_block < 0 || n_blocks < 0 || first_block + n_blocks > b->capture_pos) return fail("capture read beyond the write position");
  if (n_blocks == 0) return 0;
  if (!host_out) return fail("null output");
  HIPCHK(hipSetDevice(b->device));
  if (sync_all(b) != 0) return -1;
// ... 288 lines not shown
  ShardWorkers &w = *static_cast<ShardWorkers *>(b->workers);
  int dev0 = -1;
  const bool have_dev = hipGetDevice(&dev0) == hipSuccess;
  if (!have_dev) (void)hipGetLastError();
  ShardWorkers::Job j; j.I = I; j.Q = Q; j.out = out; j.n_blocks = n_blocks;
  { std::lock_guard<std::mutex> lk(w.m); w.job = j; w.pending = G - 1; w.gen++; }
  w.cv_go.notify_all();
  ShardWorkers::run_shard(b, 0, j, w.rc[0], w.err[0]);
  { std::unique_lock<std::mutex> lk(w.m); w.cv_done.wait(lk, [&] { return w.pending == 0; }); }
  if (have_dev) (void)hipSetDevice(dev0);
  for (size_t g = 0; g < G; g++) if (w.rc[g] != 0) return fail("shard " + std::to_string(g) + ": " + w.err[g]);
  return 0;
}

}

extern "C" {
int asdr_update(asdr_batch_t *b, const int16_t *I, const int16_t *Q, int16_t *out, int n_blocks) {
  if (!b) return fail("null batch");
  if (is_sharded(b)) return sharded_update(b, I, Q, out, n_blocks);
  if (b->device == ASDR_NO_DEVICE) return fail("control-plane-only batch (ASDR_NO_DEVICE): the signal path needs a HIP device");
  if (!I || !Q) return 0;
  if (!out) return fail("null output");
  if (n_blocks <= 0) return 0;
  return host_update(b, I, Q, out, n_blocks);
}

void *asdr_host_alloc(size_t bytes) {
  void *p = nullptr;
  if (hipHostMalloc(&p, bytes ? bytes : 1, hipHostMallocPortable) != hipSuccess) { (void)hipGetLastError(); fail("asdr_host_alloc: hipHostMalloc failed"); return nullptr; }
  return p;
}
void asdr_host_free(void *p) { if (p) (void)hipHostFree(p); }
int asdr_host_register(void *p, size_t bytes) {
  if (!p || !bytes) return fail("asdr_host_register: null buffer");
  HIPCHK(hipHostRegister(p, bytes, hipHostRegisterPortable));
  return 0;
}
int asdr_host_unregister(void *p) {
  if (!p) return fail("asdr_host_unregister: null buffer");
  HIPCHK(hipHostUnregister(p));
  return 0;
}
int asdr_set_pool_priority(int level) {
  if (level < 0 || level > 2) return fail("asdr_set_pool_priority: 0 = normal, 1 = highest, 2 = lowest");
  if (g_pool_created) return fail("asdr_set_pool_priority: the stream pool exists already (call it before the first asdr_create)");
  g_pool_priority = level;
  return 0;
}
int asdr_host_autopin(int on) { std::lock_guard<std::mutex> lk(g_autopin.m); const int was = g_autopin.on() ? 1 : 0; if (on >= 0) g_autopin.enabled = on ? 1 : 0; return was; }
void asdr_host_autopin_clear(void) { g_autopin.clear(); }
int asdr_host_autopin_info(long out[4]) {
  if (!out) return fail("null output");
  std::lock_guard<std::mutex> lk(g_autopin.m);
  long n_reg = 0; for (const AutoPin::Ent &e : g_autopin.ents) n_reg += e.registered ? 1 : 0;
  out[0] = n_reg; out[1] = g_autopin.stat_registered; out[2] = g_autopin.stat_evicted; out[3] = g_autopin.stat_failed;
  return 0;
}
int asdr_order_before(asdr_batch_t *b, void *stream_) {
  if (!b) return fail("null batch");
  FOR_SHARDS(b, asdr_order_before(sh_, stream_));
  if (b->device == ASDR_NO_DEVICE) return 0;
  if (stream_ == ASDR_STREAM_BATCH) return fail("asdr_order_before: name one of your own streams");
  HIPCHK(hipSetDevice(b->device));
  hipStream_t stream = (hipStream_t)stream_;
  if (b->lanes_pending && lanes_join_into(b, stream) != 0) return -1;
  if (b->ev_last_valid && b->last_stream != stream && !b->last_was_lanes) {
    HIPCHK(hipEventRecord(b->ev_last, b->last_stream));
    HIPCHK(hipStreamWaitEvent(stream, b->ev_last, 0));
  }
  return 0;
}
int asdr_order_after(asdr_batch_t *b, void *stream_) {
  if (!b) return fail("null batch");
  FOR_SHARDS(b, asdr_order_after(sh_, stream_));
  if (b->device == ASDR_NO_DEVICE) return 0;
  if (stream_ == ASDR_STREAM_BATCH) return fail("asdr_order_after: name one of your own streams");
  HIPCHK(hipSetDevice(b->device));
  HIPCHK(hipEventRecord(b->ev_fork, (hipStream_t)stream_));
  for (int l = 0; l < ASDR_LANES + 1; l++) if (b->lane[l] || l < b->sched_lanes || l == ASDR_LANES) { hipStream_t ls = lane_stream(b, l); if (!ls) return fail("stream creation failed"); HIPCHK(hipStreamWaitEvent(ls, b->ev_fork, 0)); }
  HIPCHK(hipStreamWaitEvent(b->stream, b->ev_fork, 0));
  return 0;
}
long asdr_lane_calls(asdr_batch_t *b) {
  if (is_sharded(b)) { long t = 0; for (asdr_batch *sh : b->shards) t += sh->stat_lane_calls; return t; }
  return b ? b->stat_lane_calls : -1;
}
int asdr_lanes_overlap_probe(asdr_batch_t *b) {
  if (!b) return -1;
  if (is_sharded(b)) { int r = 1; for (asdr_batch *sh : b->shards) { const int v = asdr_lanes_overlap_probe(sh); if (v < r) r = v; } return r; }
  return (b->device >= 0 && b->device < kPoolDevices) ? g_lanes_probe_last[b->device] : -1;
}
int asdr_lanes_enabled(asdr_batch_t *b) {
  if (!b) return -1;
  if (is_sharded(b)) { for (asdr_batch *sh : b->shards) if (!asdr_lanes_enabled(sh)) return 0; return 1; }
  if (!b->lanes_enabled) return 0;
  const int probe = (b->device >= 0 && b->device < kPoolDevices) ? g_lanes_probe_last[b->device] : -1;
  return (probe == 0 && !b->lanes_forced) ? 0 : 1;
}
long asdr_sam_chunk_calls(asdr_batch_t *b) {
  if (is_sharded(b)) { long t = 0; for (asdr_batch *sh : b->shards) t += sh->stat_sam_chunk_calls; return t; }
  return b ? b->stat_sam_chunk_calls : -1;
}
long asdr_als_role_calls(asdr_batch_t *b) {
  if (is_sharded(b)) { long t = 0; for (asdr_batch *sh : b->shards) t += sh->stat_als_role_calls; return t; }
  return b ? b->stat_als_role_calls : -1;
}
long asdr_sam_role_calls(asdr_batch_t *b) {
  if (is_sharded(b)) { long t = 0; for (asdr_batch *sh : b->shards) t += sh->stat_sam_role_calls; return t; }
  return b ? b->stat_sam_role_calls : -1;
}
int asdr_set_lanes(asdr_batch_t *b, int on, int min_waves) {
  if (!b) return fail("null batch");
  if (on < 0 || on > ASDR_LANES) return fail("lanes: 0 (off), 1 (on), or the number of lanes 2..8");
  FOR_SHARDS(b, asdr_set_lanes(sh_, on, min_waves));
  if (b->device != ASDR_NO_DEVICE && b->lanes_pending) { HIPCHK(hipSetDevice(b->device)); if (sync_all(b) != 0) return -1; }
  b->lanes_enabled = on != 0;
  b->lanes_forced = on != 0;
  if (on >= 2) { b->n_lanes = on; b->n_lanes_sam = on; b->sched_dirty = true; }
  if (min_waves > 0) b->lanes_min_waves = std::max(2 * ASDR_LANES, min_waves);
  return 0;
}
int asdr_set_launch_split(asdr_batch_t *b, int pieces, int min_waves) {
  if (!b) return fail("null batch");
  if (pieces < 1 || pieces > 8) return fail("launch split must be in 1..8");
  FOR_SHARDS(b, asdr_set_launch_split(sh_, pieces, min_waves));
  b->launch_split = pieces;
  if (min_waves > 0) b->launch_split_min_waves = std::max(8, min_waves);
  return 0;
}
int asdr_set_host_chunks(asdr_batch_t *b, int chunks) {
  if (!b) return fail("null batch");
  if (chunks < 0 || chunks > 4096) return fail("bad chunk count");
  if (is_sharded(b)) { for (asdr_batch *s : b->shards) s->host_chunks_forced = chunks; return 0; }
  b->host_chunks_forced = chunks;
  return 0;
}
int asdr_debug_host_plan(asdr_batch_t *b, int chunks, int *bound, int *need_in, int *last_part) {
  if (!b || is_sharded(b)) return fail("asdr_debug_host_plan: a plain batch");
  if (chunks < 1 || chunks > b->n || b->sched_dirty) return fail("asdr_debug_host_plan: bad chunk count, or no schedule yet");
  HostPlan hp;
  build_host_plan(b, hp, chunks);
  for (int j = 0; j <= chunks; j++) if (bound) bound[j] = hp.bound[j];
  for (int j = 0; j < chunks; j++) { if (need_in) need_in[j] = hp.need_in[j]; if (last_part) last_part[j] = hp.last_part[j]; }
  return 0;
}
int asdr_debug_part_slots(asdr_batch_t *b, int part, int parts, int *out) {
  if (!b || is_sharded(b) || !out || parts < 1 || part < 0 || part >= parts || b->sched_dirty) return fail("asdr_debug_part_slots: bad argument");
  int n = 0;
  auto sub = [&](int first, int slots) {
    const long w = slots / 8;
    const int lo = (int)(w * part / parts) * 8, cnt = (int)(w * (part + 1) / parts) * 8 - lo;
    if (cnt > 0 && n < 16) { out[2 * n] = first + lo; out[2 * n + 1] = cnt; n++; }
  };
  if (b->left_slots > 0) sub(b->left_first, b->left_slots);
  for (int k = 0; k < ASDR_KERNEL_KINDS; k++) {
    const int nu = b->kind_uniform_slots[k], nm = b->kind_slots[k] - nu;
    if (nu > 0) sub(b->kind_first[k], nu);
    if (nm > 0) sub(b->kind_first[k] + nu, nm);
  }
  return n;
}
int asdr_debug_schedule(asdr_batch_t *b, int *channels, int cap) {
  if (!b || is_sharded(b) || b->sched_dirty) return fail("asdr_debug_schedule: no schedule yet");
  for (size_t i = 0; i < b->sched.size() && (int)i < cap; i++) channels[i] = b->sched[i].ch;
  return (int)b->sched.size();
// ... 452 lines not shown
```

audiosdr_amd/csrc/asdr_kernels.hip:

```cpp
#include <hip/hip_runtime.h>
#include <stdint.h>
#include <stddef.h>
#include <string.h>
#include <stdlib.h>
#include <type_traits>

#include "asdr_device.h"
#include "asdr_tables.h"
#include "../../include/asdr.h"

#define W0 0
#define W1 128
#define PH 256
#define XP 0
#ifndef ASDR_STRIDE
#define ASDR_STRIDE 388
#endif
#ifndef ASDR_AGC_QUIET_PATH
#define ASDR_AGC_QUIET_PATH 1
#endif
#ifndef ASDR_MW_OWN_STORES
#define ASDR_MW_OWN_STORES 1
#endif
#ifndef ASDR_AGC_LEAN
// ... 316 lines not shown
        v2f t = B0 * P[2 + k]; t += B1 * P[1 + k]; t += B2 * P[k];
        p[k] = t.x; p[k + 4] = t.y;
      }
    }
    } else
#endif
    {
#pragma unroll
    for (int j = 0; j < C; ++j) {
      const float xm1 = (j >= 1) ? x[j - 1] : x1, xm2 = (j >= 2) ? x[j - 2] : ((j == 1) ? x1 : x2);
      float t = b0 * x[j]; t += b1 * xm1; t += b2 * xm2;
      p[j] = t;
    }
    }
#pragma unroll
    for (int j = 0; j < C; ++j) {
      const float ym1 = (j >= 1) ? y[j - 1] : y1, ym2 = (j >= 2) ? y[j - 2] : ((j == 1) ? y1 : y2);
      float t = p[j] + a1 * ym1; t += a2 * ym2;
      y[j] = t;
    }
    const bool act = !EDGE || ((cn >= 0) && (cn < ASDR_N / C));
    if (act) { x1 = x[C - 1]; x2 = x[C - 2]; y1 = y[C - 1]; y2 = y[C - 2]; }
#pragma unroll
    for (int j = 0; j < C; ++j) yo[j] = y[j];
    if (on && act && st == 3) {
#pragma unroll
      for (int q = 0; q < C / 4; ++q) reinterpret_cast<float4 *>(row)[cn * (C / 4) + q] = make_float4(y[4 * q], y[4 * q + 1], y[4 * q + 2], y[4 * q + 3]);
    }
  };
#if defined(ASDR_PIPE_ONE_LOOP) || ASDR_PIPE_CHUNK != 8
#pragma unroll 1
  for (int c = 0; c < NSTEP; ++c) step(std::true_type{}, c);
#else
#pragma unroll 1
  for (int c = 0; c < 3; ++c) step(std::true_type{}, c);
#pragma unroll 1
  for (int c = 3; c < 15; c += 2) { step(std::false_type{}, c); step(std::false_type{}, c + 1); }
  step(std::false_type{}, 15);
#pragma unroll 1
  for (int c = 16; c < NSTEP; ++c) step(std::true_type{}, c);
#endif
  if constexpr (SIGNAL) { if (sig) asm volatile("ds_write_b32 %0, %1" :: "v"(prog_lds), "v"(ASDR_N / C) : "memory"); }
  sv[0] = x1; sv[1] = x2; sv[2] = y1; sv[3] = y2;
}

__device__ __forceinline__ void load16(const float *p, float *v) {
  const float4 *q = reinterpret_cast<const float4 *>(p);
#pragma unroll
  for (int r = 0; r < 4; ++r) { float4 t = q[r]; v[4 * r] = t.x; v[4 * r + 1] = t.y; v[4 * r + 2] = t.z; v[4 * r + 3] = t.w; }
}
__device__ __forceinline__ void load8(const float *p, float *v) {
  const float4 *q = reinterpret_cast<const float4 *>(p);
  const float4 a = q[0], b = q[1];
  v[0] = a.x; v[1] = a.y; v[2] = a.z; v[3] = a.w; v[4] = b.x; v[5] = b.y; v[6] = b.z; v[7] = b.w;
}
__device__ __forceinline__ void load4(const float *p, float *v) {
  const float4 a = *reinterpret_cast<const float4 *>(p);
  v[0] = a.x; v[1] = a.y; v[2] = a.z; v[3] = a.w;
}
__device__ __forceinline__ void store4(float *p, const float *v) { *reinterpret_cast<float4 *>(p) = make_float4(v[0], v[1], v[2], v[3]); }
__device__ __forceinline__ void store4_nt(float *p, const float *v) {
  typedef float f4v __attribute__((ext_vector_type(4)));
  const f4v tv = {v[0], v[1], v[2], v[3]};
  __builtin_nontemporal_store(tv, reinterpret_cast<f4v *>(p));
}
#ifndef ASDR_NT_LOADS
#define ASDR_NT_LOADS 2
#endif
__device__ __forceinline__ int4 load_int4_nt(const int4 *p) {
  typedef int i4v __attribute__((ext_vector_type(4)));
  const i4v t = __builtin_nontemporal_load(reinterpret_cast<const i4v *>(p));
  return make_int4(t[0], t[1], t[2], t[3]);
}
__device__ __forceinline__ void load4_nt(const float *p, float *v) {
  typedef float f4v __attribute__((ext_vector_type(4)));
  const f4v t = __builtin_nontemporal_load(reinterpret_cast<const f4v *>(p));
  v[0] = t[0]; v[1] = t[1]; v[2] = t[2]; v[3] = t[3];
}
__device__ __forceinline__ void store_int4_nt(int4 *p, int4 v) {
  typedef int i4v __attribute__((ext_vector_type(4)));
  const i4v tv = {v.x, v.y, v.z, v.w};
  __builtin_nontemporal_store(tv, reinterpret_cast<i4v *>(p));
}
__device__ __forceinline__ void store4e(float *p, const float *v) { *reinterpret_cast<float4 *>(p) = make_float4(v[0], v[2], v[4], v[6]); }
__device__ __forceinline__ void store8(float *p, const float *v) {
  float4 *q = reinterpret_cast<float4 *>(p);
  q[0] = make_float4(v[0], v[1], v[2], v[3]); q[1] = make_float4(v[4], v[5], v[6], v[7]);
}

__device__ __forceinline__ double div_i16_by_32767(double x) {
  return __builtin_fma(x, 0x1.0002000400080p-15, x * 0x1.0002000400080p-75);
}
__device__ __forceinline__ void scale8(const int16_t *s, double g, float *out, bool unit = false) {
  if (unit) {
#pragma unroll
    for (int j = 0; j < 8; ++j) { const float x = (float)s[j]; out[j] = __builtin_fmaf(x, 0x1.0002p-15f, x * 0x1.0002p-45f); }
    return;
  }
#pragma unroll
  for (int j = 0; j < 8; ++j) {
#ifdef ASDR_OLD_SCALE
    out[j] = (float)(div_by_const((double)s[j], 32767.0, 1.0 / 32767.0) * g);
#else
    out[j] = (float)(div_i16_by_32767((double)s[j]) * g);
#endif
    if ((j & 1) == 1) SCHED_FENCE();
  }
}
#define ASDR_MASK_MAGIC 0x14c4005000006ull
__device__ __forceinline__ float mask_decode_byte(float tabv, uint32_t group4, uint32_t word, int k) {
  const uint32_t sh = (k == 0) ? (word << 2) : (word >> (8 * k - 2));
  const uint32_t addr = (sh & 0x1Cu) | group4;
  return __int_as_float(__builtin_amdgcn_ds_bpermute((int)addr, __float_as_int(tabv)));
}
__device__ __forceinline__ uint32_t mask_encode(float v) {
  const uint32_t idx = (__float_as_uint(v) >> 21) & 0x1Fu;
  return (uint32_t)(ASDR_MASK_MAGIC >> ((idx * 3u - 36u) & 63u)) & 7u;
}
__device__ __forceinline__ uint32_t mask_encode4(float4 mv) {
  const uint32_t c0 = mask_encode(mv.x), c1 = mask_encode(mv.y), c2 = mask_encode(mv.z), c3 = mask_encode(mv.w);
  return c0 | (c1 << 8) | (c2 << 16) | (c3 << 24);
}

#define ALS_TAP(q, wh) ((((q) & 1) ? (wh) : 0) + ((q) >> 1))
template <bool CHECKED, int WH>
__device__ __forceinline__ float als_dot(const float *w, const float *x, int top, int M) {
  float y = 0.0f;
  int q = 0;
#pragma unroll 2
  for (; q + 4 <= M; q += 4) {
    const float2 we = *reinterpret_cast<const float2 *>(w + (q >> 1)), wo = *reinterpret_cast<const float2 *>(w + WH + (q >> 1));
    const int t = top - q;
    float x0, x1, x2, x3;
    if (CHECKED) {
      x0 = (t >= 0 && t < 256) ? x[t] : 0.0f; x1 = (t - 1 >= 0 && t - 1 < 256) ? x[t - 1] : 0.0f;
      x2 = (t - 2 >= 0 && t - 2 < 256) ? x[t - 2] : 0.0f; x3 = (t - 3 >= 0 && t - 3 < 256) ? x[t - 3] : 0.0f;
    } else {
      x0 = x[t]; x1 = x[t - 1]; x2 = x[t - 2]; x3 = x[t - 3];
    }
    float p;
    p = we.x * x0; y += p; p = wo.x * x1; y += p; p = we.y * x2; y += p; p = wo.y * x3; y += p;
  }
  for (; q < M; ++q) {
    const int t = top - q;
    const float xv = CHECKED ? ((t >= 0 && t < 256) ? x[t] : 0.0f) : x[t];
    const float p = w[ALS_TAP(q, WH)] * xv;
    y += p;
  }
  return y;
}

__device__ __forceinline__ float dpp_row_shl4(float v) {
  return __int_as_float(__builtin_amdgcn_update_dpp(0, __float_as_int(v), 0x104, 0xF, 0xF, true));
}

struct AlsGroup { float4 w; float x0, x1, x2, x3; };
__device__ __forceinline__ void als_group_load(AlsGroup &G, const float *wh, const float *xh, int g) {
  G.w = *reinterpret_cast<const float4 *>(wh + 4 * g);
  G.x0 = xh[-8 * g]; G.x1 = xh[-8 * g - 2]; G.x2 = xh[-8 * g - 4]; G.x3 = xh[-8 * g - 6];
}
__device__ __forceinline__ float als_group_sum(float y, const AlsGroup &G) {
  const float p0 = G.w.x * G.x0, p1 = G.w.y * G.x1, p2 = G.w.z * G.x2, p3 = G.w.w * G.x3;
  y += p0; y += dpp_row_shl4(p0); y += p1; y += dpp_row_shl4(p1);
  y += p2; y += dpp_row_shl4(p2); y += p3; y += dpp_row_shl4(p3);
  return y;
}
// ... 353 lines not shown
#pragma unroll 1
      for (int ep = -1; ep < 32; ++ep) {
        const int base = (ep < 0) ? 0 : 4 * ep + 1;
        const int cntn = (ep < 0) ? 1 : ((ep == 31) ? 3 : 4);
        const int n = base + (s8 & 3);
        const bool mine = als_en && adaptive && (s8 < cntn);
        if (als_safe) {
          const int i = 128 + n, h = s8 >> 2;
          float y = 0.0f;
          if (als_m_default) y = als_dot_split_const<ALS_M_DEFAULT>(L + AW + WH * h, L + XB + (i - D - h), h);
          else if (als_m_uniform) y = als_dot_split_uniform(L + AW + WH * h, L + XB + (i - D - h), M_u, h);
          else if (als_en && adaptive) y = als_dot_split(L + AW + WH * h, L + XB + (i - D - h), M, h);
          if (mine) {
            const float e = L[XB + i] - y;
            L[OUT + n] = notch ? e : y;
            if ((n & 3) == 0) L[SCR] = e;
          }
        } else if (mine) {
          if constexpr (!COMPACT) {
            const int i = 128 + n;
            const float y = als_dot<true, WH>(L + AW, L + XB, i - D, M);
            const float e = L[XB + i] - y;
            L[OUT + n] = notch ? e : y;
            if ((n & 3) == 0) L[SCR] = e;
          }
        }
        WAVE_SYNC();
        const int nu = (ep < 0) ? 0 : 4 * ep + 4;
        if (als_en && adaptive && nu < ASDR_N) {
          const float e = L[SCR];
          const int iu = 128 + nu;
          if (als_m_default) {
            als_tap_update_const<ALS_M_DEFAULT>(L + XB + iu - D - s8, L + AW + ALS_TAP(s8, WH), e, lam, s8);
          } else if (als_m_uniform && als_safe) {
            const float *xq = L + XB + iu - D - s8;
            float *wq = L + AW + ALS_TAP(s8, WH);
            const int nk = (M_u - s8 + 7) >> 3, nk_max = (M_u + 7) >> 3;
#pragma unroll 1
            for (int k0 = 0; k0 < nk_max; k0 += 8) {
              float xv[8], wv[8];
#pragma unroll
              for (int j = 0; j < 8; ++j) { xv[j] = xq[-8 * (k0 + j)]; wv[j] = wq[4 * (k0 + j)]; }
#pragma unroll
              for (int j = 0; j < 8; ++j) { const float gq = e * xv[j]; const float dq = lam * gq; const float wn = wv[j] + dq; wv[j] = (k0 + j < nk) ? wn : wv[j]; }
#pragma unroll
              for (int j = 0; j < 8; ++j) wq[4 * (k0 + j)] = wv[j];
            }
          } else if (als_safe) {
#pragma unroll 2
            for (int q = s8; q < M; q += 8) { const float gq = e * L[XB + iu - D - q]; const float dq = lam * gq; L[AW + ALS_TAP(q, WH)] += dq; }
          } else {
            if constexpr (!COMPACT) {
              for (int q = s8; q < M; q += 8) { const float gq = e * (((iu - D - q) >= 0 && (iu - D - q) < 256) ? L[XB + (iu - D - q)] : 0.0f); const float dq = lam * gq; L[AW + ALS_TAP(q, WH)] += dq; }
            }
          }
        }
        WAVE_SYNC();
      }
    }
}
template <int STRIDE, bool HAS_ALS, bool HAS_SAM, bool UNIFORM, int WAVES, int ROLE = 0, bool ONEBLK_ = false, int FIR_HELPERS = 1, bool UPAR = false>
__device__ __forceinline__ void asdr_update_body(const UpdateArgs &a, float *lds_wg) {
  constexpr bool C16 = (STRIDE == 320);
  constexpr bool PRE_ROLE = (ROLE == 4 || ROLE == 8), POST_ROLE = (ROLE == 5 || ROLE == 9 || ROLE == 10), LOOPED_ROLE = (ROLE == 7 || ROLE == 8 || ROLE == 9 || ROLE == 10);
  constexpr bool DO1 = (ROLE == 0 || ROLE == 1 || PRE_ROLE || ROLE == 6 || ROLE == 7), DO2 = (ROLE == 0 || ROLE == 2 || POST_ROLE || ROLE == 6 || ROLE == 7),
                 DO3 = (ROLE == 0 || ROLE == 3 || POST_ROLE || ROLE == 6 || ROLE == 7);
  constexpr bool TO_ALS = (ROLE == 6 || ROLE == 7 || ROLE == 10);
#ifndef ASDR_ALS_FULL_OPT
#define ASDR_ALS_FULL_OPT 2
#endif
  constexpr bool ALS_LOOPFREE = (ASDR_ONEBLK_ALS != 0) && (ONEBLK_ || (ROLE >= 4 && !LOOPED_ROLE && ASDR_ONEBLK_ROLES));
  constexpr bool ALS_FULL_OPT = (ASDR_ALS_FULL_OPT >= 1) && ASDR_COMPACT_ROWS(STRIDE) && ALS_LOOPFREE,
                 ALS_FULL_OPT2 = (ASDR_ALS_FULL_OPT >= 2) && ASDR_COMPACT_ROWS(STRIDE) && ALS_LOOPFREE;
  constexpr bool STREAM = (ROLE >= 1 && ROLE <= 3);
  constexpr bool PIPE_PK = ((ASDR_PIPE_PK_MASK & 1) && HAS_ALS) || ((ASDR_PIPE_PK_MASK & 2) && !HAS_ALS && !HAS_SAM && ROLE == 0) ||
                           ((ASDR_PIPE_PK_MASK & 4) && (HAS_SAM || ROLE > 3)) || ((ASDR_PIPE_PK_MASK & 8) && STREAM);
  if (ROLE == 0 && a.run_if != nullptr && *a.run_if == 0u) return;
  constexpr bool MW = (WAVES > 1) && !HAS_SAM && (ROLE == 0);
  constexpr int MW_SHARE = MW ? ASDR_MW_SHARE : 0;
  const int wave = (WAVES > 1) ? (int)(threadIdx.x >> 6) : 0;
#ifndef ASDR_MW_ROT
#define ASDR_MW_ROT 0
#endif
  const uint32_t mw_b = blockIdx.x;
  const uint32_t mw_rot = (ASDR_MW_ROT == 0) ? mw_b : (ASDR_MW_ROT == 1) ? (mw_b >> 3) : (ASDR_MW_ROT == 2) ? ((mw_b >> 3) + (mw_b >> 8)) :
                          (ASDR_MW_ROT == 3) ? ((mw_b * 0x9E3779B1u) >> 30) : (ASDR_MW_ROT == 4) ? ((mw_b >> 3) % 3u) : (mw_b >> 5);
  const int mw_rel = MW ? (int)(((uint32_t)wave - mw_rot) & (uint32_t)(WAVES - 1)) : 0;
  float *const mwx = lds_wg + WAVES * 8 * STRIDE;
#ifndef ASDR_MW_STRAGGLER_PRIO
#define ASDR_MW_STRAGGLER_PRIO 0
#endif
  int *const mw_prog = reinterpret_cast<int *>(lds_wg + WAVES * 8 * STRIDE + 8 * WAVES * 16 + 260);
  int *const mw_flags = mw_prog + 4;
  constexpr bool PIPE_AGC = MW && WAVES == 4 && (MW_SHARE & 7) == 7 && (ASDR_MW_AGC_PIPELINED != 0) && (ASDR_AGC_LEAN != 0) && (ASDR_MW_OWN_STORES != 0) && ABL_ON(ABL_AGC) && ABL_ON(ABL_AF) && ABL_ON(ABL_NB);
  if constexpr (PIPE_AGC) { if (threadIdx.x < 3) mw_flags[1 + threadIdx.x] = 0; }
  if constexpr (MW && ASDR_MW_STRAGGLER_PRIO != 0) { if ((threadIdx.x & 63) == 0) mw_prog[wave] = 0; }
  auto mw_straggler = [&](int point) {
    if constexpr (MW && ASDR_MW_STRAGGLER_PRIO != 0) {
      if ((threadIdx.x & 63) == 0) mw_prog[wave] = point;
      const int4 pr = *reinterpret_cast<const int4 *>(mw_prog);
      const int behind = (pr.x < point) + (pr.y < point) + (pr.z < point) + (pr.w < point);
      const bool last = __builtin_amdgcn_readfirstlane(behind) == 0;
      if (last) __builtin_amdgcn_s_setprio(ASDR_MW_STRAGGLER_PRIO); else __builtin_amdgcn_s_setprio(0);
    }
  };
  constexpr int MWX = 16;
  auto mw_channel = [&](int q) -> int { const int sidx = (int)blockIdx.x * (8 * WAVES) + q; return (sidx < a.n_sched) ? a.direct_ch0 + sidx : a.n_channels; };
  const int wave_g = STREAM ? (int)blockIdx.x % a.stream_waves : (int)blockIdx.x * WAVES + wave;
  float *const lds = lds_wg + wave * 8 * STRIDE;
  const int lane = threadIdx.x & 63, c8 = lane >> 3, s8_ = lane & 7;
#ifndef ASDR_MW_SINE_LDS
#define ASDR_MW_SINE_LDS 0
#endif
  constexpr bool MW_SINE = MW && (ASDR_MW_SINE_LDS != 0);
  constexpr bool MW_SINE_LAZY = MW_SINE && (ASDR_MW_SINE_LDS == 2) && (MW_SHARE & 2) != 0 && WAVES == 4;
  constexpr bool SINE_LDS = HAS_SAM || (MW_SINE && !MW_SINE_LAZY);
  constexpr bool SINE_LDS_PC = HAS_SAM || MW_SINE;
  float *const sine_tab = HAS_SAM ? lds_wg + WAVES * 8 * STRIDE : (MW_SINE ? lds_wg + WAVES * 8 * STRIDE + 8 * WAVES * 16 : nullptr);
  float *const sine = SINE_LDS ? sine_tab : nullptr;
  int *const mw_sflag = reinterpret_cast<int *>(lds_wg + WAVES * 8 * STRIDE + 8 * WAVES * 16 + 260) + 8;
  if (HAS_SAM) for (int i = lane; i < ASDR_SINE_TABLE_LEN; i += 64) sine_tab[i] = c_sine[i];
  if (MW_SINE && !MW_SINE_LAZY) { for (int i = (int)threadIdx.x; i < ASDR_SINE_TABLE_LEN; i += 64 * WAVES) sine_tab[i] = c_sine[i]; __syncthreads(); }

  int4 slot = make_int4(a.n_channels, 0, 0, 0);
  const bool mw_pad = MW && (wave_g * 8 >= a.n_sched);
  if (UNIFORM && a.direct_ch0 >= 0) slot = make_int4(mw_pad ? a.n_channels : a.direct_ch0 + wave_g * 8 + c8, (int)a.direct_mode, (int)a.direct_flags, (int)((a.direct_lo & 0xFFu) | (wave_g == 0 ? a.lo_writer_bit : 0u)));
  else if (WAVES == 1 || wave_g * 8 < a.n_sched) slot = *reinterpret_cast<const int4 *>(a.sched + wave_g * 8 + c8);
  else { const ChanParams *pd = a.params + a.n_channels; slot.y = (int)pd->mode; slot.z = (int)pd->flags; }
  const int ch_ = slot.x;
  const bool valid = (UNIFORM && !mw_pad) || (ch_ < a.n_channels);
  const int loff_ = c8 * STRIDE;
#define P (*Pp)
  const ChainConsts K = a.k;
  auto pv = [](float x) -> float { if constexpr (UPAR) asm volatile("" : "+v"(x)); return x; };

  const uint32_t mode = UNIFORM ? (uint32_t)__builtin_amdgcn_readfirstlane(slot.y) : (uint32_t)slot.y;
  const uint32_t pflags = UNIFORM ? (uint32_t)__builtin_amdgcn_readfirstlane(slot.z) : (uint32_t)slot.z;
  const uint32_t lo_slot = UNIFORM ? (uint32_t)__builtin_amdgcn_readfirstlane(slot.w) : 0u;
  const bool is_ssb = DO2 && ((mode == ASDR_USBmode) || (mode == ASDR_LSBmode) || (mode == ASDR_CW_USBmode) ||
                              (mode == ASDR_CW_LSBmode) || (mode == ASDR_WSPRmode));
#ifndef ASDR_MW_NO_AM
#define ASDR_MW_NO_AM 0
#endif
  const bool is_am = !C16 && !(MW && ASDR_MW_NO_AM) && (mode == ASDR_AMmode), is_sam = (HAS_SAM || ROLE >= 4) && (mode == ASDR_SAMmode);
  const bool sub_q = (mode == ASDR_USBmode) || (mode == ASDR_CW_USBmode) || (mode == ASDR_WSPRmode);
  const bool nb_en = DO1 && (pflags & ASDR_F_NB_EN), af_en = DO3 && (pflags & ASDR_F_AF_EN), agc_en = DO3 && (pflags & ASDR_F_AGC_EN);
  if constexpr (MW_SINE_LAZY) {
    if (!(ABL_ON(ABL_NB) && __any(nb_en))) {
      for (int i = (int)threadIdx.x; i < ASDR_SINE_TABLE_LEN; i += 64 * WAVES) sine_tab[i] = c_sine[i];
      __syncthreads();
    }
  }
  const bool als_en = HAS_ALS && (pflags & ASDR_F_ALS_EN);
  const bool muted = pflags & ASDR_F_MUTED;
  const float two_pi = K.two_pi_f;
  WAVE_SYNC();
  uint32_t seen_in = 0u, seen_free = 0u, seen_lo = 0u, sig_pending = 0u;
  float carry_phase = 0.0f, carry_fsh = 0.0f;
  uint32_t carry_hs = 0u;
#ifndef ASDR_STREAM_PREFETCH_IN
#define ASDR_STREAM_PREFETCH_IN 1
#endif
  int4 pf_in[4] = {make_int4(0, 0, 0, 0), make_int4(0, 0, 0, 0), make_int4(0, 0, 0, 0), make_int4(0, 0, 0, 0)};
#ifndef ASDR_STREAM_R2_ONE_TRIP
#define ASDR_STREAM_R2_ONE_TRIP 1
#endif
#ifndef ASDR_STREAM_R2_PREFETCH
#define ASDR_STREAM_R2_PREFETCH 1
#endif
  constexpr bool R2_ONE_TRIP = (ROLE == 2) && (FIR_HELPERS == 3) && (ASDR_STREAM_R2_ONE_TRIP != 0);
  constexpr bool R2_PREFETCH = R2_ONE_TRIP && (ASDR_STREAM_R2_PREFETCH != 0);
  v4f r2n_key = (v4f){0.f, 0.f, 0.f, 0.f}, r2n_c4[4], r2n_s4[4], r2n_vi[4], r2n_vq[4];
  bool r2_pref = false;
  uint32_t r2_look_in = 0u, r2_look_lo = 0u;
#ifndef ASDR_STREAM_R1_CARRY
#define ASDR_STREAM_R1_CARRY 0
#endif
  float4 r1_if_s4 = make_float4(0.f, 0.f, 0.f, 0.f);
  float r1_if_cf[5] = {0.f, 0.f, 0.f, 0.f, 0.f}, r1_gain_i = 0.f, r1_gain_q = 0.f;
  uint32_t *const my_prog = STREAM ? a.stream_prog + (ROLE - 1) * a.stream_waves + wave_g : nullptr;

  constexpr bool ONEBLK = (!HAS_ALS || ASDR_ONEBLK_ALS) && (ONEBLK_ || (ROLE >= 4 && !LOOPED_ROLE && ASDR_ONEBLK_ROLES));
  constexpr bool UNIT_OK = (ASDR_UNIT_SCALE != 0) && ((ONEBLK && ROLE == 0) || ROLE == 1);
  static_assert(!C16 || (ONEBLK && UNIFORM && !HAS_ALS && !HAS_SAM && WAVES == 1 && ROLE == 0), "the 16-waves-per-CU form is the plain uniform one-block kernel");
#pragma unroll 1
  for (int blk = 0; blk < (ONEBLK ? 1 : a.n_blocks); ++blk) {
    int s8 = s8_; asm volatile("" : "+v"(s8));
    int loff = loff_; asm volatile("" : "+v"(loff));
    int ch = ch_; asm volatile("" : "+v"(ch));
    int lane_i = lane; asm volatile("" : "+v"(lane_i));
#ifdef ASDR_TIMELINE
    if (STREAM && a.taps != nullptr && wave_g == 0 && lane == 0) (reinterpret_cast<unsigned long long *>(a.taps) + 64 * (3 + ROLE) + 32 * (blk & 1))[16] = clock64();
#endif
    if (STREAM) {
      uint32_t *prog = a.stream_prog, *err = a.stream_err;
      const uint32_t b1 = (uint32_t)blk + 1u, freed = (blk >= ASDR_STREAM_DEPTH) ? (uint32_t)(blk - ASDR_STREAM_DEPTH + 1) : 0u;
      const bool need_in = (ROLE != 1) && seen_in < b1, need_free = (ROLE != 3) && seen_free < freed;
      if ((need_in || need_free) && sig_pending) { stream_signal(my_prog, sig_pending, lane); sig_pending = 0u; }
      if (need_in) { seen_in = stream_wait(prog + (ROLE - 2) * a.stream_waves + wave_g, b1, err, a.stream_spin_limit); if (seen_in == ASDR_STREAM_FAIL) break; }
      if (need_free) { seen_free = stream_wait(prog + ROLE * a.stream_waves + wave_g, freed, err, a.stream_spin_limit); if (seen_free == ASDR_STREAM_FAIL) break; }
    }
    const ChanParams *Pp = UPAR ? &a.uni : row_ptr(a.params, (uint32_t)ch * (uint32_t)sizeof(ChanParams));
    ChanSmall *S = row_ptr(a.small, (uint32_t)ch * (uint32_t)sizeof(ChanSmall));
    float *L = lds + loff;
    int *Li = reinterpret_cast<int *>(L);
    constexpr bool PLB = (ASDR_PIPE_BANK_SELECT != 0);
#define pl_st (PLB ? ((lane_i & 15) >> 2) : (s8 & 3))
#define pl_iq (PLB ? (lane_i & 1) : (s8 >> 2))
#define pl_c (PLB ? (2 * (lane_i >> 4) + ((lane_i >> 1) & 1)) : (lane_i >> 3))
#define pa_c (PLB ? (2 * (lane_i >> 4) + (lane_i & 1)) : (lane_i >> 3))
#define pa_real (PLB ? ((lane_i & 3) < 2) : ((lane_i & 7) < 4))
#if ASDR_PIPE_BANK_SELECT
#define PL_CH(c) (__builtin_amdgcn_ds_bpermute((c) << 5, ch))
#define Sp row_ptr(a.small, (uint32_t)PL_CH(pl_c) * (uint32_t)sizeof(ChanSmall))
#define Spa row_ptr(a.small, (uint32_t)PL_CH(pa_c) * (uint32_t)sizeof(ChanSmall))
#define Ppl (UPAR ? &a.uni : row_ptr(a.params, (uint32_t)PL_CH(pl_c) * (uint32_t)sizeof(ChanParams)))
#define Ppa (UPAR ? &a.uni : row_ptr(a.params, (uint32_t)PL_CH(pa_c) * (uint32_t)sizeof(ChanParams)))
#define Lp (lds + pl_c * STRIDE)
#define Lpa (lds + pa_c * STRIDE)
#else
#define PL_CH(c) ch
#define Sp S
#define Spa S
#define Ppl Pp
#define Ppa Pp
#define Lp L
#define Lpa L
#endif
    const bool af_en_pa = (PLB && !UNIFORM) ? (__builtin_amdgcn_ds_bpermute(pa_c << 5, af_en ? 1 : 0) != 0) : af_en;
    const int k0 = 16 * s8, kA = 8 * s8, kF = 4 * s8;
    const bool lead = (s8 == 0);
#ifdef ASDR_TIMELINE
    const int tl_wg = ((int)blockIdx.x == 0) ? 0 : (((int)blockIdx.x == 683) ? 1 : (((int)blockIdx.x == 1365) ? 2 : (((int)blockIdx.x == 2047) ? 3 : -1)));
    const int tl_slot = STREAM ? ((wave_g == 0) ? 2 * (3 + ROLE) + (blk & 1) : -1)
                               : (MW ? ((tl_wg < 0) ? -1 : 4 * tl_wg + wave)
                                     : ((wave_g == 0) ? 0 : ((wave_g == 2731) ? 1 : ((wave_g == 5461) ? 2 : ((wave_g == 8191) ? 3 : -1)))));
    unsigned long long *tl = reinterpret_cast<unsigned long long *>(a.taps) + 32 * (tl_slot < 0 ? 0 : tl_slot);
#define TL(i) do { if (a.taps != nullptr && tl_slot >= 0 && lane == 0) tl[i] = clock64(); } while (0)
    const bool tap_on = false;
    TL(0);
    if (MW && a.taps != nullptr && tl_slot >= 0 && lane == 0) { uint32_t hw; asm volatile("s_getreg_b32 %0, hwreg(HW_REG_HW_ID)" : "=s"(hw)); tl[29] = hw; }
#else
#define TL(i) do { } while (0)
    const bool tap_on = (a.taps != nullptr) && valid && (blk == a.n_blocks - 1);
#endif
    float *tap_base = tap_on ? a.taps + (size_t)ch * ASDR_N + kA : nullptr;
    const size_t tap_stride = (size_t)a.n_channels * ASDR_N;
#define TAP8(id, h, v) do { if (tap_on) store8(tap_base + (size_t)(id) * tap_stride + 64 * (h), v); } while (0)
#define TAP4(id, m, v) do { if (tap_on) store4(tap_base - kA + kF + (size_t)(id) * tap_stride + 32 * (m), v); } while (0)
#define TAP_ROW(id, rowoff) do { if (tap_on) { for (int h_ = 0; h_ < 2; ++h_) { float tv_[8]; load8(L + (rowoff) + kA + 64 * h_, tv_); \
                                  store8(tap_base + (size_t)(id) * tap_stride + 64 * h_, tv_); } } } while (0)

    uint32_t status = S->status;
    const uint32_t status_in = status;
    const bool mix_early = is_ssb || (DO2 && is_am);
    float mphase = 0.0f, minc = 0.0f, mphase_end = 0.0f;
    float fsh_raw = 0.0f;
    if (mix_early) {
      if (ROLE == 2 && blk > 0) { mphase = carry_phase; fsh_raw = carry_fsh; }
      else { mphase = is_ssb ? S->phase_ssb : S->phase_am; fsh_raw = P.freq_shift; }
    }
    const float nb_thr = P.nb_threshold;
    const uint32_t lo_e = (lo_slot & 0xFFu) ? (lo_slot & 0xFFu) - 1u : 0u;
    const bool lo_has = (ROLE == 2) || ((lo_slot & 0xFFu) != 0u);
    const LoEntry *lo_rd = (ROLE == 2) ? a.lo_ring + (blk % ASDR_LO_RING) : a.lo_cache + (a.lo_parity & 1u) * ASDR_LO_ENTRIES + lo_e;
    uint32_t lo_kp, lo_ki;
    float lo_end;
    v4f r2_c4[4], r2_s4[4], r2_vi[4], r2_vq[4];
    if (ROLE == 2) {
      v4f key;
      if (R2_PREFETCH && r2_pref) {
        key = r2n_key;
#pragma unroll
        for (int m = 0; m < 4; ++m) { r2_c4[m] = r2n_c4[m]; r2_s4[m] = r2n_s4[m]; r2_vi[m] = r2n_vi[m]; r2_vq[m] = r2n_vq[m]; }
        r2_pref = false;
      } else {
      if (seen_lo < (uint32_t)blk + 1u) { seen_lo = stream_wait(a.stream_prog + 3 * a.stream_waves, (uint32_t)blk + 1u, a.stream_err, a.stream_spin_limit); if (seen_lo == ASDR_STREAM_FAIL) break; }
      if (R2_ONE_TRIP) {
        const float *lp = lo_rd->c + 4 * s8_, *xp = a.xch_a + ((size_t)ch * ASDR_STREAM_DEPTH + (size_t)(blk % ASDR_STREAM_DEPTH)) * (2 * ASDR_N) + 4 * s8_;
        asm volatile("global_load_dwordx4 %0, %17, off sc1\n\t"
                     "global_load_dwordx4 %1, %18, off sc1\n\tglobal_load_dwordx4 %2, %18, off offset:128 sc1\n\tglobal_load_dwordx4 %3, %18, off offset:256 sc1\n\tglobal_load_dwordx4 %4, %18, off offset:384 sc1\n\t"
                     "global_load_dwordx4 %5, %18, off offset:512 sc1\n\tglobal_load_dwordx4 %6, %18, off offset:640 sc1\n\tglobal_load_dwordx4 %7, %18, off offset:768 sc1\n\tglobal_load_dwordx4 %8, %18, off offset:896 sc1\n\t"
                     "global_load_dwordx4 %9, %19, off sc1\n\tglobal_load_dwordx4 %10, %19, off offset:128 sc1\n\tglobal_load_dwordx4 %11, %19, off offset:256 sc1\n\tglobal_load_dwordx4 %12, %19, off offset:384 sc1\n\t"
                     "global_load_dwordx4 %13, %19, off offset:512 sc1\n\tglobal_load_dwordx4 %14, %19, off offset:640 sc1\n\tglobal_load_dwordx4 %15, %19, off offset:768 sc1\n\tglobal_load_dwordx4 %16, %19, off offset:896 sc1\n\t"
                     "s_waitcnt vmcnt(0)"
                     : "=&v"(key), "=&v"(r2_c4[0]), "=&v"(r2_c4[1]), "=&v"(r2_c4[2]), "=&v"(r2_c4[3]), "=&v"(r2_s4[0]), "=&v"(r2_s4[1]), "=&v"(r2_s4[2]), "=&v"(r2_s4[3]),
                       "=&v"(r2_vi[0]), "=&v"(r2_vi[1]), "=&v"(r2_vi[2]), "=&v"(r2_vi[3]), "=&v"(r2_vq[0]), "=&v"(r2_vq[1]), "=&v"(r2_vq[2]), "=&v"(r2_vq[3])
                     : "v"(lo_rd), "v"(lp), "v"(xp) : "memory");
      } else
      asm volatile("global_load_dwordx4 %0, %1, off sc1\n\ts_waitcnt vmcnt(0)" : "=&v"(key) : "v"(lo_rd) : "memory");
      }
      lo_kp = __float_as_uint(key[0]); lo_ki = __float_as_uint(key[1]); lo_end = key[2];
    } else {
      lo_kp = lo_rd->key_phase; lo_ki = lo_rd->key_inc; lo_end = lo_rd->phase_end;
    }
    const uint32_t ns = (a.nb_phase + (uint32_t)blk) % 3u;
    const uint32_t hs = (ROLE == 2 && blk > 0) ? carry_hs : (S->hil_slot & 1u);
    const uint32_t ns_mid = (ns + 1u) % 3u, ns_new = (ns + 2u) % 3u;
    float carrier_now = 0.0f;
    bool carrier_fresh = false;
    const size_t io = ((size_t)ch * a.in_stride + blk) * ASDR_N + kA;
    const size_t io_out = ((size_t)ch * a.out_stride + blk) * ASDR_N + kA;
    const bool nb_wave = ABL_ON(ABL_NB) && __any(nb_en);
    int16_t *hist = row_ptr(a.nb_hist, (uint32_t)ch * 1536u);
    uint32_t *mrow = reinterpret_cast<uint32_t *>(row_ptr(a.nb_mask, (uint32_t)ch * ASDR_NB_MASK_ROW + 4u * (uint32_t)s8));

    union Raw8 { int4 v; int16_t s[8]; };
    Raw8 ri[2], rq[2], roi[2], roq[2], rmi[2], rmq[2];
    ri[0].v = ri[1].v = rq[0].v = rq[1].v = make_int4(0, 0, 0, 0);
    roi[0].v = roi[1].v = roq[0].v = roq[1].v = rmi[0].v = rmi[1].v = rmq[0].v = rmq[1].v = make_int4(0, 0, 0, 0);
    uint32_t mkc[5] = {0x01010101u, 0x01010101u, 0x01010101u, 0x01010101u, 0x01010101u};
    float gain_i, gain_q;
    if (ROLE == 1 && ASDR_STREAM_R1_CARRY && blk > 0) { gain_i = r1_gain_i; gain_q = r1_gain_q; }
    else { gain_i = pv(P.in_gain_i); gain_q = pv(P.in_gain_q); if (ROLE == 1) { r1_gain_i = gain_i; r1_gain_q = gain_q; } }
    float g_oi = gain_i, g_oq = gain_q, g_mi = 0.0f, g_mq = 0.0f, nb_avg0 = 0.0f;
    uint32_t agc_hc_early = 0u, agc_hang_early = 0u;
    bool agc_piped = false;
    if (nb_wave && nb_en) {
      g_oi = S->nb_gain[ns][0]; g_oq = S->nb_gain[ns][1]; g_mi = S->nb_gain[ns_mid][0]; g_mq = S->nb_gain[ns_mid][1];
      nb_avg0 = S->nb_avg;
      if constexpr (PIPE_AGC) { agc_hc_early = S->agc_hang_counter; agc_hang_early = P.agc_hang_count; }
      const int4 *old4 = reinterpret_cast<const int4 *>(hist + ns * 256 + kA), *mid4 = reinterpret_cast<const int4 *>(hist + ns_mid * 256 + kA);
#if ASDR_NT_LOADS >= 2
      rmi[0].v = mid4[0]; rmi[1].v = mid4[8]; rmq[0].v = mid4[16]; rmq[1].v = mid4[24];
      roi[0].v = load_int4_nt(old4); roi[1].v = load_int4_nt(old4 + 8); roq[0].v = load_int4_nt(old4 + 16); roq[1].v = load_int4_nt(old4 + 24);
#else
      rmi[0].v = mid4[0]; rmi[1].v = mid4[8]; rmq[0].v = mid4[16]; rmq[1].v = mid4[24];
      roi[0].v = old4[0]; roi[1].v = old4[8]; roq[0].v = old4[16]; roq[1].v = old4[24];
#endif
#pragma unroll
      for (int r = 0; r < 5; ++r) mkc[r] = mrow[8 * r];
      if constexpr (C16) {
        const uint32_t all1 = (mkc[0] & mkc[1] & mkc[2] & mkc[3] & mkc[4]) == 0x01010101u && (mkc[0] | mkc[1] | mkc[2] | mkc[3] | mkc[4]) == 0x01010101u ? 0x01010101u : 0u;
#pragma unroll
        for (int r = 0; r < 5; ++r) mkc[r] = all1;
      }
    }
    if (DO1 && valid) {
      const int4 *pi = reinterpret_cast<const int4 *>(a.in_i + io);
      const int4 *pq = reinterpret_cast<const int4 *>(a.in_q + io);
      if constexpr (ROLE == 1 && ASDR_STREAM_PREFETCH_IN != 0) {
        if (blk == 0) { ri[0].v = load_int4_nt(pi); ri[1].v = load_int4_nt(pi + 8); rq[0].v = load_int4_nt(pq); rq[1].v = load_int4_nt(pq + 8); }
        else { ri[0].v = pf_in[0]; ri[1].v = pf_in[1]; rq[0].v = pf_in[2]; rq[1].v = pf_in[3]; }
      } else {
#if ASDR_NT_LOADS >= 1
      ri[0].v = load_int4_nt(pi); ri[1].v = load_int4_nt(pi + 8); rq[0].v = load_int4_nt(pq); rq[1].v = load_int4_nt(pq + 8);
#else
      ri[0].v = pi[0]; ri[1].v = pi[8]; rq[0].v = pq[0]; rq[1].v = pq[8];
#endif
      }
    }
    if (mix_early) minc = (is_ssb ? -fsh_raw : -K.if_center) * K.phase_inc_unit;
    bool ph_ready = false;
    bool lo_hit = false;
    if ((blk == 0 || ROLE == 2) && lo_has) lo_hit = __all(mix_early && __float_as_uint(mphase) == lo_kp && __float_as_uint(minc) == lo_ki);
    if (lo_hit && lead) { if (is_ssb) S->phase_ssb = lo_end; else S->phase_am = lo_end; }

    if (nb_wave) {
    } else if (DO1) {
      const bool unit_in = UNIT_OK && (UPAR ? (a.uni.in_gain_i == 1.0f && a.uni.in_gain_q == 1.0f) : __all(gain_i == 1.0f && gain_q == 1.0f));
#pragma unroll
      for (int h = 0; h < 2; ++h) {
        float xi[8], xq[8];
        scale8(ri[h].s, (double)gain_i, xi, unit_in); scale8(rq[h].s, (double)gain_q, xq, unit_in);
        TAP8(ASDR_TAP_SCALED_I, h, xi); TAP8(ASDR_TAP_SCALED_Q, h, xq);
        store8(L + W0 + kA + 64 * h, xi); store8(L + W1 + kA + 64 * h, xq);
        SCHED_FENCE();
      }
    }

    float4 if_s4 = make_float4(0.f, 0.f, 0.f, 0.f);
    float if_cf[5] = {0.f, 0.f, 0.f, 0.f, 0.f};
    bool if_pre = false;
    auto load_if_rows_early = [&]() {
      if_s4 = *reinterpret_cast<const float4 *>(&Sp->if_state[pl_iq][4 * pl_st]);
      const float *cf = &c_bq_pool[Ppl->if_table][5 * pl_st];
#pragma unroll
      for (int z = 0; z < 5; ++z) if_cf[z] = cf[z];
      if_pre = true;
    };
    TL(1);
    if (nb_wave) {
      float vio[16], vqo[16], mgm[16], mgt[8];
      if (!nb_en) {
#pragma unroll
        for (int h = 0; h < 2; ++h) { roi[h].v = ri[h].v; roq[h].v = rq[h].v; }
      }
      const bool own_tail = (s8 >= 1);
      if (C16 && nb_en) {
        int4 *ni = reinterpret_cast<int4 *>(hist + ns_new * 256 + kA);
        store_int4_nt(ni, ri[0].v); store_int4_nt(ni + 8, ri[1].v); store_int4_nt(ni + 16, rq[0].v); store_int4_nt(ni + 24, rq[1].v);
        if (lead) { S->nb_gain[ns_new][0] = gain_i; S->nb_gain[ns_new][1] = gain_q; }
      }
      const bool unit_ring = UNIT_OK && __all(g_oi == 1.0f && g_oq == 1.0f && (!nb_en || (g_mi == 1.0f && g_mq == 1.0f)));
      auto env4 = [&](const float *pw4, float *mg4) {
        if (unit_ring) {
#pragma unroll
          for (int j = 0; j < 4; ++j) mg4[j] = fast_sqrt1_short(pw4[j]);
        } else {
#pragma unroll
          for (int j = 0; j < 4; ++j) mg4[j] = fast_sqrt1(pw4[j]);
        }
      };
      if constexpr (C16) {
        auto mid_piece = [&](int h) {
          float vim[8], vqm[8], bm8[8], pw[8];
          scale8(rmi[h].s, (double)g_mi, vim, unit_ring); scale8(rmq[h].s, (double)g_mq, vqm, unit_ring);
#pragma unroll
          for (int j = 0; j < 8; ++j) pw[j] = vim[j] * vim[j] + vqm[j] * vqm[j];
          env4(pw, mgm + 8 * h); env4(pw + 4, mgm + 8 * h + 4);
#pragma unroll
          for (int j = 0; j < 8; ++j) bm8[j] = K.nb_beta * mgm[8 * h + j];
          if (nb_en) store8(L + NB_B + 50 + kA + 64 * h, bm8);
        };
        mid_piece(0);
        __builtin_amdgcn_sched_barrier(0);
        if (own_tail) {
          float tio[8], tqo[8], bm8[8], pw[8];
          scale8(roi[1].s, (double)g_oi, tio, unit_ring); scale8(roq[1].s, (double)g_oq, tqo, unit_ring);
#pragma unroll
          for (int j = 0; j < 8; ++j) pw[j] = tio[j] * tio[j] + tqo[j] * tqo[j];
          env4(pw, mgt); env4(pw + 4, mgt + 4);
#pragma unroll
          for (int j = 0; j < 8; ++j) bm8[j] = K.nb_beta * mgt[j];
          if (nb_en) { if (s8 >= 2) store8(L + kA - 12, bm8); else *reinterpret_cast<float4 *>(L) = make_float4(bm8[4], bm8[5], bm8[6], bm8[7]); }
        } else {
#pragma unroll
          for (int j = 0; j < 8; ++j) mgt[j] = 0.0f;
        }
        __builtin_amdgcn_sched_barrier(0);
        mid_piece(1);
      } else {
#pragma unroll
      for (int h = 0; h < 2; ++h) {
        float vim[8], vqm[8], bm8[8], pw[8];
        scale8(roi[h].s, (double)g_oi, vio + 8 * h, unit_ring); scale8(roq[h].s, (double)g_oq, vqo + 8 * h, unit_ring);
        scale8(rmi[h].s, (double)g_mi, vim, unit_ring); scale8(rmq[h].s, (double)g_mq, vqm, unit_ring);
#pragma unroll
        for (int j = 0; j < 8; ++j) pw[j] = vim[j] * vim[j] + vqm[j] * vqm[j];
        env4(pw, mgm + 8 * h); env4(pw + 4, mgm + 8 * h + 4);
#pragma unroll
        for (int j = 0; j < 8; ++j) bm8[j] = K.nb_beta * mgm[8 * h + j];
        if (nb_en) store8(L + NB_B + 50 + kA + 64 * h, bm8);
      }
      if (own_tail) {
        float bm8[8], pw[8];
#pragma unroll
        for (int j = 0; j < 8; ++j) pw[j] = vio[8 + j] * vio[8 + j] + vqo[8 + j] * vqo[8 + j];
        env4(pw, mgt); env4(pw + 4, mgt + 4);
#pragma unroll
        for (int j = 0; j < 8; ++j) bm8[j] = K.nb_beta * mgt[j];
        if (nb_en) { if (s8 >= 2) store8(L + kA - 12, bm8); else *reinterpret_cast<float4 *>(L) = make_float4(bm8[4], bm8[5], bm8[6], bm8[7]); }
      } else {
#pragma unroll
        for (int j = 0; j < 8; ++j) mgt[j] = 0.0f;
      }
      }
      if (nb_en && !C16) {
        int4 *ni = reinterpret_cast<int4 *>(hist + ns_new * 256 + kA);
#ifndef ASDR_TEMPORAL_RINGS
        store_int4_nt(ni, ri[0].v); store_int4_nt(ni + 8, ri[1].v); store_int4_nt(ni + 16, rq[0].v); store_int4_nt(ni + 24, rq[1].v);
#else
        ni[0] = ri[0].v; ni[8] = ri[1].v; ni[16] = rq[0].v; ni[24] = rq[1].v;
#endif
        if (lead) { S->nb_gain[ns_new][0] = gain_i; S->nb_gain[ns_new][1] = gain_q; }
      }
      if (tap_on) {
#pragma unroll
        for (int h = 0; h < 2; ++h) { float xi[8], xq[8]; scale8(ri[h].s, (double)gain_i, xi); scale8(rq[h].s, (double)gain_q, xq);
                                      TAP8(ASDR_TAP_SCALED_I, h, xi); TAP8(ASDR_TAP_SCALED_Q, h, xq); }
      }
      WAVE_SYNC();
      TL(2);
#ifndef ASDR_MW_IF_PRE
#define ASDR_MW_IF_PRE 1
#endif
      if (DO1 && ABL_ON(ABL_IF) && (WAVES == 1 || (MW && ASDR_MW_IF_PRE)) && !C16) {
        if_s4 = *reinterpret_cast<const float4 *>(&Sp->if_state[pl_iq][4 * pl_st]);
        const float *cf = &c_bq_pool[Ppl->if_table][5 * pl_st];
#pragma unroll
        for (int z = 0; z < 5; ++z) if_cf[z] = cf[z];
        if_pre = true;
      }
#ifndef ASDR_CHAIN_CONSTS_IN_VGPRS
#define ASDR_CHAIN_CONSTS_IN_VGPRS 0
#endif
#ifndef ASDR_MW_OWN_STORES
#define ASDR_MW_OWN_STORES 1
#endif
      float nb_avg_end = 0.0f;
      auto nb_chain = [&](float *Lc, ChanSmall *Sc, float avg0, float phase0, float inc, bool chain_phase, bool want_phase, bool en, bool ssb) -> float {
        float avg = avg0, phase = phase0;
        float nb_alpha_v = K.nb_alpha, two_pi_v = two_pi;
        if constexpr (!C16 && ONEBLK && ASDR_CHAIN_CONSTS_IN_VGPRS) asm("" : "+v"(nb_alpha_v), "+v"(two_pi_v));
        const bool up = !(inc < 0.0f);
        const float wrapv = up ? -two_pi : two_pi, lim = up ? two_pi : 0.0f;
        const uint32_t flip = up ? 0u : 0x80000000u;
#pragma unroll
        for (int u = 0; u < 2; ++u) { const float bmu = Lc[NB_B + u]; Lc[NB_B + u] = avg; const float aa = nb_alpha_v * avg; avg = aa + bmu; }
        float bm[8];
        load8(Lc + NB_B + 2, bm);
        int c_tail = 0;
        if constexpr (C16) {
          float bn[8];
          const int n_both = chain_phase ? 16 : 0;
#pragma unroll 1
          for (int c = 0; c < 22; c += 2) {
#pragma unroll
            for (int half = 0; half < 2; ++half) {
              float *cur = half ? bn : bm, *nxt = half ? bm : bn;
              load8(Lc + NB_B + 2 + 8 * ((c + half < 21) ? c + half + 1 : 21), nxt);
              if (c < n_both) {
                float pe[4];
#pragma unroll
                for (int u = 0; u < 8; ++u) {
                  const float a0 = avg; const float aa = nb_alpha_v * avg; avg = aa + cur[u]; cur[u] = a0;
                  if ((u & 1) == 0) pe[u >> 1] = phase;
                  const float t = phase + inc, tw = t + wrapv;
                  phase = (__uint_as_float(__float_as_uint(t) ^ flip) > lim) ? tw : t;
                }
                store4(Lc + PH + 4 * (c + half), pe);
              } else {
#pragma unroll
                for (int u = 0; u < 8; ++u) { const float a0 = avg; const float aa = nb_alpha_v * avg; avg = aa + cur[u]; cur[u] = a0; }
              }
              store8(Lc + NB_B + 2 + 8 * (c + half), cur);
            }
          }
          c_tail = n_both;
        } else {
        if (chain_phase) {
        c_tail = 16;
        if (!(HAS_ALS && !ALS_FULL_OPT2) && __all(inc < 0.0f)) {
#pragma unroll 1
          for (int c = 0; c < 16; c += 2) {
            float av[8], bn[8], pv[8];
#pragma unroll
            for (int half = 0; half < 2; ++half) {
              float *cur = half ? bn : bm, *nxt = half ? bm : bn;
              load8(Lc + NB_B + 2 + 8 * (c + half + 1), nxt);
#pragma unroll
              for (int u = 0; u < 8; ++u) {
                av[u] = avg; const float aa = nb_alpha_v * avg; avg = aa + cur[u];
                pv[u] = phase;
// ... 333 lines not shown
        pf_in[0] = load_int4_nt(pi); pf_in[1] = load_int4_nt(pi + 8); pf_in[2] = load_int4_nt(pq); pf_in[3] = load_int4_nt(pq + 8);
      }
    }
    if (DO1 && ABL_ON(ABL_IF)) {
      const int iq = pl_iq, st = pl_st;
      float sv[4];
      if (HAS_ALS && !ALS_FULL_OPT && !if_pre) load_if_rows();
      sv[0] = if_s4.x; sv[1] = if_s4.y; sv[2] = if_s4.z; sv[3] = if_s4.w;
      CHAIN_PRIO_ON();
      biquad_pipe<PIPE_PK>(Lp + (iq ? W1 : W0), true, st, if_cf, sv);
      CHAIN_PRIO_OFF();
      *reinterpret_cast<float4 *>(&Sp->if_state[iq][4 * st]) = make_float4(sv[0], sv[1], sv[2], sv[3]);
      if (ROLE == 1 && ASDR_STREAM_R1_CARRY) {
        r1_if_s4 = make_float4(sv[0], sv[1], sv[2], sv[3]);
#pragma unroll
        for (int z = 0; z < 5; ++z) r1_if_cf[z] = if_cf[z];
      }
    }
    if (C16 && lo_hit) store4(lds + (lane_i >> 4) * STRIDE + PH + ((4 * lane_i) & 63), lo4);
    WAVE_SYNC();
    TL(5);
    mw_straggler(2);
    if (DO1) { TAP_ROW(ASDR_TAP_IF_I, W0); TAP_ROW(ASDR_TAP_IF_Q, W1); }
    auto store_status_bits = [&](uint32_t mask) {
      if (lead && ((status ^ status_in) & mask) != 0u) { atomicAnd(&S->status, ~mask); atomicOr(&S->status, status & mask); }
    };
    if (ROLE == 1 || ROLE == 2) {
      float *xa = a.xch_a + ((size_t)ch * ASDR_STREAM_DEPTH + (size_t)(blk % ASDR_STREAM_DEPTH)) * (2 * ASDR_N) + kF;
      if (ROLE == 1) {
        v4f vi[4], vq[4];
#pragma unroll
        for (int m = 0; m < 4; ++m) { vi[m] = *reinterpret_cast<const v4f *>(L + W0 + kF + 32 * m); vq[m] = *reinterpret_cast<const v4f *>(L + W1 + kF + 32 * m); }
        xch_store4x4(xa, vi[0], vi[1], vi[2], vi[3]); xch_store4x4(xa + ASDR_N, vq[0], vq[1], vq[2], vq[3]);
        store_status_bits(ASDR_S_NB_DETECTED);
#ifndef ASDR_STREAM_LATE_SIGNAL
#define ASDR_STREAM_LATE_SIGNAL 1
#endif
        if (ASDR_STREAM_LATE_SIGNAL) sig_pending = (uint32_t)blk + 1u;
        else stream_signal(a.stream_prog + wave_g, (uint32_t)blk + 1u, lane);
        continue;
      } else {
        v4f vi[4], vq[4];
        if (R2_ONE_TRIP) {
#pragma unroll
          for (int m = 0; m < 4; ++m) { vi[m] = r2_vi[m]; vq[m] = r2_vq[m]; }
          if (sig_pending) asm volatile("s_waitcnt vmcnt(0)" ::: "memory");
        } else { xch_load4x4(xa, vi[0], vi[1], vi[2], vi[3]); xch_load4x4(xa + ASDR_N, vq[0], vq[1], vq[2], vq[3]); }
        if (sig_pending) { if (lane == 0) __hip_atomic_store(my_prog, sig_pending, __ATOMIC_RELAXED, __HIP_MEMORY_SCOPE_AGENT); sig_pending = 0u; }
#pragma unroll
        for (int m = 0; m < 4; ++m) { *reinterpret_cast<v4f *>(L + W0 + kF + 32 * m) = vi[m]; *reinterpret_cast<v4f *>(L + W1 + kF + 32 * m) = vq[m]; }
        WAVE_SYNC();
        if constexpr (R2_PREFETCH) {
          r2_look_in = __hip_atomic_load(a.stream_prog + wave_g, __ATOMIC_RELAXED, __HIP_MEMORY_SCOPE_AGENT);
          r2_look_lo = __hip_atomic_load(a.stream_prog + 3 * a.stream_waves, __ATOMIC_RELAXED, __HIP_MEMORY_SCOPE_AGENT);
        }
      }
    }

    const uint32_t sam_set_k = (LOOPED_ROLE && a.sam_sets > 1u) ? (a.sam_set + (uint32_t)blk) % a.sam_sets : 0u;
    float *const sam_tile = (ROLE >= 4) ? a.xch_sam + (size_t)sam_set_k * a.sam_set_stride + (size_t)wave_g * (2 * ASDR_N * 8) : nullptr;
    float *const sam_lds = lds + (4 * (lane_i & 1)) * STRIDE + (((lane_i >> 1) & 1) ? W1 : W0) + (lane_i >> 2);
    if (PRE_ROLE) {
#pragma unroll
      for (int k = 0; k < 8; ++k) {
        const float *src = sam_lds + 16 * k;
        *reinterpret_cast<float4 *>(sam_tile + 4 * (lane_i + 64 * k)) = make_float4(src[0], src[STRIDE], src[2 * STRIDE], src[3 * STRIDE]);
      }
      store_status_bits(ASDR_S_NB_DETECTED);
      continue;
    }
    bool pll_locked = false;
    auto pll_run = [&](float *Lc, ChanSmall *Sc) -> bool {
      return pll_loop<HAS_ALS, 4>(Sc, K, sine, two_pi,
        [&](int i, float *xr, float *xi) {
          const float4 r4 = *reinterpret_cast<const float4 *>(Lc + W0 + i), i4 = *reinterpret_cast<const float4 *>(Lc + W1 + i);
          xr[0] = r4.x; xr[1] = r4.y; xr[2] = r4.z; xr[3] = r4.w; xi[0] = i4.x; xi[1] = i4.y; xi[2] = i4.z; xi[3] = i4.w; },
        [&](int i, const float *xr, const float *xi) {
          *reinterpret_cast<float4 *>(Lc + W0 + i) = make_float4(xr[0], xr[1], xr[2], xr[3]);
          *reinterpret_cast<float4 *>(Lc + W1 + i) = make_float4(xi[0], xi[1], xi[2], xi[3]); });
    };
    if constexpr (HAS_SAM && WAVES > 1) {
      __syncthreads();
      if (ABL_ON(ABL_SAM) && wave == 0 && lane_i < 8 * WAVES) {
        const int sj = (int)blockIdx.x * WAVES * 8 + lane_i;
        int chj = a.n_channels; uint32_t modej = a.params[a.n_channels].mode;
        if (sj < a.n_sched) { const int4 sl = *reinterpret_cast<const int4 *>(a.sched + sj); chj = sl.x; modej = (uint32_t)sl.y; }
        if (modej == ASDR_SAMmode) {
          float *Lc = lds_wg + lane_i * STRIDE;
          const bool lk = pll_run(Lc, row_ptr(a.small, (uint32_t)chj * (uint32_t)sizeof(ChanSmall)));
          reinterpret_cast<int *>(Lc)[SCR0] = lk ? 1 : 0;
        }
      }
      __syncthreads();
      if (is_sam) {
        pll_locked = Li[SCR0] != 0;
        if (lead) status = (status & ~ASDR_S_PLL_LOCKED) | (pll_locked ? ASDR_S_PLL_LOCKED : 0u);
      }
    } else if (HAS_SAM && ABL_ON(ABL_SAM) && __any(is_sam)) {
      if (is_sam && lead) {
        const bool lk = pll_run(L, S);
        status = (status & ~ASDR_S_PLL_LOCKED) | (lk ? ASDR_S_PLL_LOCKED : 0u);
        Li[SCR0] = lk ? 1 : 0;
      }
      WAVE_SYNC();
      if (is_sam) pll_locked = Li[SCR0] != 0;
    }
    if (POST_ROLE) {
      float4 pc[8];
#pragma unroll
      for (int k = 0; k < 8; ++k) pc[k] = *reinterpret_cast<const float4 *>(sam_tile + 4 * (lane_i + 64 * k));
#pragma unroll
      for (int k = 0; k < 8; ++k) {
        float *dst = sam_lds + 16 * k;
        dst[0] = pc[k].x; dst[STRIDE] = pc[k].y; dst[2 * STRIDE] = pc[k].z; dst[3 * STRIDE] = pc[k].w;
      }
      if (is_sam) pll_locked = a.sam_lock[(size_t)sam_set_k * a.sam_lock_stride + wave_g * 8 + c8] != 0u;
      WAVE_SYNC();
    }
    const bool do_env = DO2 && (is_am || (is_sam && !pll_locked));
    const bool do_mix = is_ssb || do_env;

    if (do_mix && !mix_early) { mphase = S->phase_am; minc = -K.if_center * K.phase_inc_unit; }
    const bool ph_seq = do_mix && !ph_ready && !lo_hit;
    if (__any(ph_seq)) {
      if (ph_seq && lead) {
        float phase = mphase;
        const bool up = !(minc < 0.0f);
        const float wrapv = up ? -two_pi : two_pi, lim = up ? two_pi : 0.0f;
        const uint32_t flip = up ? 0u : 0x80000000u;
#pragma unroll 1
        for (int i = 0; i < ASDR_N; i += 8) {
          float pv[8];
#pragma unroll
          for (int u = 0; u < 8; ++u) {
            pv[u] = phase;
            const float t = phase + minc, tw = t + wrapv;
            phase = (__uint_as_float(__float_as_uint(t) ^ flip) > lim) ? tw : t;
          }
          if constexpr (C16) store4e(L + PH + (i >> 1), pv); else store8(L + PH + i, pv);
        }
        if (is_ssb) S->phase_ssb = phase; else S->phase_am = phase;
        mphase_end = phase;
      }
      WAVE_SYNC();
    }
    if (ROLE == 2) {
      const float endp = __int_as_float(__builtin_amdgcn_ds_bpermute((lane_i & ~7) << 2, __float_as_int(mphase_end)));
      carry_phase = lo_hit ? lo_end : endp;
      carry_fsh = fsh_raw;
    }
    const uint32_t ph_first = (uint32_t)__builtin_amdgcn_readfirstlane((int)__float_as_uint(mphase));
    const uint32_t inc_first = (uint32_t)__builtin_amdgcn_readfirstlane((int)__float_as_uint(minc));
    const bool mix_uni = __all(do_mix && __float_as_uint(mphase) == ph_first && __float_as_uint(minc) == inc_first);
    TL(6);
    auto phase_step = [&](float p, float inc) -> float {
      const bool up = !(inc < 0.0f);
      const float wrapv = up ? -two_pi : two_pi, lim = up ? two_pi : 0.0f;
      const uint32_t flip = up ? 0u : 0x80000000u;
      const float t = p + inc, tw = t + wrapv;
      return (__uint_as_float(__float_as_uint(t) ^ flip) > lim) ? tw : t;
    };
    if (ABL_ON(ABL_MIX) && mix_uni && !lo_hit) {
      float ph2[2];
      if constexpr (C16) { ph2[0] = lds[PH + lane_i]; ph2[1] = phase_step(ph2[0], minc); WAVE_SYNC(); }
      else { const float2 p2 = *reinterpret_cast<const float2 *>(lds + PH + 2 * lane); ph2[0] = p2.x; ph2[1] = p2.y; }
      float c2[2], s2[2];
      sincos_batch<2, SINE_LDS>(sine, ph2, c2, s2, two_pi, SinIndexK{K.inv_two_pi_d, K.sin_index_scale_d}, K.half_pi_d);
      if constexpr (C16) {
        *reinterpret_cast<float2 *>(lds + (lane_i >> 5) * STRIDE + PH + ((2 * lane_i) & 63)) = make_float2(c2[0], c2[1]);
        *reinterpret_cast<float2 *>(lds + (2 + (lane_i >> 5)) * STRIDE + PH + ((2 * lane_i) & 63)) = make_float2(s2[0], s2[1]);
      } else {
      *reinterpret_cast<float2 *>(lds + STRIDE + PH + 2 * lane) = make_float2(c2[0], c2[1]);
      *reinterpret_cast<float2 *>(lds + 2 * STRIDE + PH + 2 * lane) = make_float2(s2[0], s2[1]);
      }
      WAVE_SYNC();
    }
    constexpr bool QN_DIRECT_K = UNIFORM && ABL_ON(ABL_MIX) && (ASDR_MIX_KEEP_Q != 0);
    const bool qn_direct = QN_DIRECT_K && is_ssb;
    float qn[16];
    DEFINE_ALL_PATHS(qn, 16);
    if constexpr (C16) {
      if (ABL_ON(ABL_MIX) && do_mix) {
#define C16_MIX_LOOP(STAGED)                                                                                                                  \
          _Pragma("unroll")                                                                                                                   \
          for (int m = 0; m < 4; ++m) {                                                                                                       \
            float cc[4], sn[4], vi[4], vq[4], mi[4], mq[4];                                                                                   \
            load4(L + W0 + kF + 32 * m, vi); load4(L + W1 + kF + 32 * m, vq);                                                                 \
            if (STAGED) {                                                                                                                     \
              load4(lds + (m >> 1) * STRIDE + PH + 32 * (m & 1) + kF, cc); load4(lds + (2 + (m >> 1)) * STRIDE + PH + 32 * (m & 1) + kF, sn); \
            } else {                                                                                                                          \
              float ph[4];                                                                                                                    \
              const float2 e2 = *reinterpret_cast<const float2 *>(L + PH + ((kF + 32 * m) >> 1));                                             \
              ph[0] = e2.x; ph[1] = phase_step(e2.x, minc); ph[2] = e2.y; ph[3] = phase_step(e2.y, minc);                                     \
              sincos_batch<4, SINE_LDS>(sine, ph, cc, sn, two_pi, SinIndexK{K.inv_two_pi_d, K.sin_index_scale_d}, K.half_pi_d);                         \
            }                                                                                                                                 \
            _Pragma("unroll")                                                                                                                 \
            for (int j = 0; j < 4; ++j) {                                                                                                     \
              mi[j] = vi[j] * cc[j] - vq[j] * sn[j];                                                                                          \
              mq[j] = vq[j] * cc[j] + vi[j] * sn[j];                                                                                          \
            }                                                                                                                                 \
            if (qn_direct) {                                                                                                                  \
              _Pragma("unroll")                                                                                                               \
              for (int j = 0; j < 4; ++j) qn[4 * m + j] = mq[j];                                                                              \
            } else { store4(L + W0 + kF + 32 * m, mi); store4(L + W1 + kF + 32 * m, mq); }                                                    \
            store4_nt(hi_ring + hs * 128 + 32 * m, mi);                                                                                       \
          }
        if (lo_hit || mix_uni) { C16_MIX_LOOP(true) }
        else {
          DEFINE_ALL_PATHS(hq_o, 16); DEFINE_ALL_PATHS(hq_m, 16);
          C16_MIX_LOOP(false)
#pragma unroll
          for (int m = 0; m < 4; ++m) { load4(hq_ring + hs * 128 + 32 * m, hq_o + 4 * m); load4(hq_ring + (hs ^ 1u) * 128 + 32 * m, hq_m + 4 * m); }
        }
      }
    } else
    if (ABL_ON(ABL_MIX) && do_mix) {
#pragma unroll
      for (int m = 0; m < 4; ++m) {
        float cc[4], sn[4], vi[4], vq[4], mi[4], mq[4];
        load4(L + W0 + kF + 32 * m, vi); load4(L + W1 + kF + 32 * m, vq);
        if (lo_hit) {
          if (RING_PREFETCH) {
#pragma unroll
            for (int j = 0; j < 4; ++j) { cc[j] = lo_c[4 * m + j]; sn[j] = lo_s[4 * m + j]; }
          } else { load4(lo_rd->c + kF + 32 * m, cc); load4(lo_rd->s + kF + 32 * m, sn); }
        } else if (mix_uni) {
          load4(lds + STRIDE + PH + kF + 32 * m, cc); load4(lds + 2 * STRIDE + PH + kF + 32 * m, sn);
        } else {
          float ph[4];
          load4(L + PH + kF + 32 * m, ph);
#ifndef ASDR_MIX_SERIAL_LOOKUPS
          sincos_batch<4, SINE_LDS_PC>(SINE_LDS_PC ? sine_tab : nullptr, ph, cc, sn, two_pi, SinIndexK{K.inv_two_pi_d, K.sin_index_scale_d}, K.half_pi_d);
#else
#pragma unroll
          for (int j = 0; j < 4; ++j) {
            cc[j] = cos_f32(sine, ph[j], two_pi, SinIndexK{K.inv_two_pi_d, K.sin_index_scale_d}, K.half_pi_d); sn[j] = sin_f32(sine, ph[j], two_pi, SinIndexK{K.inv_two_pi_d, K.sin_index_scale_d});
            if ((j & 1) == 1) SCHED_FENCE();
          }
#endif
        }
#pragma unroll
        for (int j = 0; j < 4; ++j) {
          mi[j] = vi[j] * cc[j] - vq[j] * sn[j];
          mq[j] = vq[j] * cc[j] + vi[j] * sn[j];
        }
        if (qn_direct) {
#pragma unroll
          for (int j = 0; j < 4; ++j) qn[4 * m + j] = mq[j];
        } else { store4(L + W0 + kF + 32 * m, mi); store4(L + W1 + kF + 32 * m, mq); }
#ifndef ASDR_TEMPORAL_RINGS
        if (is_ssb) store4_nt(hi_ring + hs * 128 + 32 * m, mi);
#else
        if (is_ssb) store4(hi_ring + hs * 128 + 32 * m, mi);
#endif
      }
    }

    float4 af_s4 = make_float4(0.f, 0.f, 0.f, 0.f);
    float af_cf[5] = {0.f, 0.f, 0.f, 0.f, 0.f};
    float agc_gain_in = 0.f, agc_old0 = 0.f, agc_carrier0 = 0.f;
    uint32_t agc_hc0 = 0u;
    int agc_tab_idx = 0;
    const bool mw_audio_duty = (MW_SHARE & 1) && (mw_rel == 1 || mw_rel == 2);
    const int mw_casc = PLB ? (4 * (lane_i >> 4) + (lane_i & 3)) : (lane_i >> 2);
    ChanSmall *mw_af_S = S;
    auto load_af_agc_state = [&]() {
    ChanSmall *const Saf = PLB ? Spa : S; const ChanParams *const Paf = PLB ? Ppa : Pp;
    if (ABL_ON(ABL_AF) && (((MW_SHARE & 1) != 0) ? af_en : af_en_pa)) {
      if constexpr ((MW_SHARE & 1) != 0) {
        if (mw_audio_duty) {
          const int chq = mw_channel(16 * (mw_rel - 1) + mw_casc);
          mw_af_S = row_ptr(a.small, (uint32_t)chq * (uint32_t)sizeof(ChanSmall));
          af_s4 = *reinterpret_cast<const float4 *>(&mw_af_S->af_state[4 * pl_st]);
          const float *cf = &c_bq_pool[(UPAR ? &a.uni : row_ptr(a.params, (uint32_t)chq * (uint32_t)sizeof(ChanParams)))->audio_table][5 * pl_st];
#pragma unroll
          for (int z = 0; z < 5; ++z) af_cf[z] = cf[z];
        }
      } else {
      af_s4 = *reinterpret_cast<const float4 *>(&Saf->af_state[4 * pl_st]);
      const float *cf = &c_bq_pool[Paf->audio_table][5 * pl_st];
#pragma unroll
      for (int z = 0; z < 5; ++z) af_cf[z] = cf[z];
      }
    }
    if (ABL_ON(ABL_AGC) && agc_en) {
      agc_gain_in = S->agc_gain; agc_old0 = S->agc_old_abs; agc_hc0 = S->agc_hang_counter; agc_carrier0 = S->am_carrier;
      agc_tab_idx = P.agc_table;
    }
    };
    if constexpr (!C16) load_af_agc_state();
    TL(7);
    if (__any(is_ssb)) {
      if (is_ssb && !qn_direct) {
#pragma unroll
        for (int m = 0; m < 4; ++m) load4(L + W1 + kF + 32 * m, qn + 4 * m);
      }
      WAVE_SYNC();
      if constexpr (C16) {
#pragma unroll
        for (int m = 0; m < 4; ++m) {
#pragma unroll
          for (int j = 0; j < 4; ++j) {
            const int k = kF + 32 * m + j;
            if (k >= 1) L[XP + k - 1] = hq_o[4 * m + j];
            L[XP + 127 + k] = hq_m[4 * m + j];
            if (k < 63) L[XP + 255 + k] = qn[4 * m + j];
          }
          store4_nt(hq_ring + hs * 128 + 32 * m, qn + 4 * m);
        }
        if (lead) S->hil_slot = hs ^ 1u;
        WAVE_SYNC();
        TL(8);
        v2f fa[4], fb[4];
#pragma unroll
        for (int e = 0; e < 4; ++e) { fa[e] = (v2f){0.0f, 0.0f}; fb[e] = (v2f){0.0f, 0.0f}; }
        if (ABL_ON(ABL_HIL)) hilbert_fir<0, 4, false>(L, 4 * s8, fa);
        WAVE_SYNC();
        {
          float t[32];
#pragma unroll
          for (int q = 0; q < 8; ++q) load4(L + XP + 64 + 32 * s8 + 4 * q, t + 4 * q);
          WAVE_SYNC();
#pragma unroll
          for (int q = 0; q < 8; ++q) store4(L + XP + 32 * s8 + 4 * q, t + 4 * q);
        }
#pragma unroll
        for (int m = 0; m < 4; ++m) {
#pragma unroll
          for (int j = 0; j < 4; ++j) { const int k = kF + 32 * m + j; if (k >= 63 && k < 127) L[XP + 191 + k] = qn[4 * m + j]; }
        }
        WAVE_SYNC();
        if (ABL_ON(ABL_HIL)) hilbert_fir<0, 4, false>(L, 4 * s8, fb);
        WAVE_SYNC();
        TL(9);
        load_af_agc_state();
#pragma unroll
        for (int m = 0; m < 4; ++m) load4(hi_ring + (hs ^ 1u) * 128 + 32 * m, idl + 4 * m);
        *reinterpret_cast<float4 *>(L + W1 + 8 * s8) = make_float4(fa[0][0], fa[0][1], fa[1][0], fa[1][1]);
        *reinterpret_cast<float4 *>(L + W1 + 8 * s8 + 4) = make_float4(fa[2][0], fa[2][1], fa[3][0], fa[3][1]);
        *reinterpret_cast<float4 *>(L + W1 + 64 + 8 * s8) = make_float4(fb[0][0], fb[0][1], fb[1][0], fb[1][1]);
        *reinterpret_cast<float4 *>(L + W1 + 64 + 8 * s8 + 4) = make_float4(fb[2][0], fb[2][1], fb[3][0], fb[3][1]);
        WAVE_SYNC();
      } else {
      if (is_ssb) {
        if (!RING_PREFETCH) {
#pragma unroll
          for (int m = 0; m < 4; ++m) {
            load4(hq_ring + hs * 128 + 32 * m, hq_o + 4 * m);
            load4(hq_ring + (hs ^ 1u) * 128 + 32 * m, hq_m + 4 * m);
          }
        }
        constexpr bool HIST_B128 = MW && WAVES == 4 && (ASDR_MW_HIST_B128 != 0);
        if constexpr (HIST_B128) {
          hilbert_hist_store16<false>(L + XP + kF, hq_o, hq_m[0], s8 == 7);
          __builtin_amdgcn_sched_barrier(0);
          hilbert_hist_store16<false>(L + XP + 128 + kF, hq_m, qn[0], s8 == 7);
          __builtin_amdgcn_sched_barrier(0);
          hilbert_hist_store16<true>(L + XP + 256 + kF, qn, 0.0f, s8 == 7);
        } else {
#pragma unroll
        for (int m = 0; m < 4; ++m) {
#pragma unroll
          for (int j = 0; j < 4; ++j) {
            const int k = kF + 32 * m + j;
            if (k >= 1) L[XP + k - 1] = hq_o[4 * m + j];
            L[XP + 127 + k] = hq_m[4 * m + j];
          }
        }
        }
#pragma unroll
        for (int m = 0; m < 4; ++m) {
          if constexpr (!HIST_B128) {
#pragma unroll
          for (int j = 0; j < 4; ++j) L[XP + 255 + kF + 32 * m + j] = qn[4 * m + j];
          }
#ifndef ASDR_TEMPORAL_RINGS
          store4_nt(hq_ring + hs * 128 + 32 * m, qn + 4 * m);
#else
          store4(hq_ring + hs * 128 + 32 * m, qn + 4 * m);
#endif
        }
        if (lead) S->hil_slot = hs ^ 1u;
        carry_hs = hs ^ 1u;
      }
      WAVE_SYNC();
      TL(8);
      mw_straggler(3);
      if constexpr (R2_PREFETCH) {
        const uint32_t b2 = (uint32_t)blk + 2u;
        if (blk + 1 < a.n_blocks && (seen_in < b2 || seen_lo < b2)) {
          const uint32_t ui = (uint32_t)__builtin_amdgcn_readfirstlane((int)r2_look_in), ul = (uint32_t)__builtin_amdgcn_readfirstlane((int)r2_look_lo);
          asm volatile("" ::: "memory");
          if (ui != ASDR_STREAM_FAIL && ui > seen_in) seen_in = ui;
          if (ul != ASDR_STREAM_FAIL && ul > seen_lo) seen_lo = ul;
        }
        if (blk + 1 < a.n_blocks && seen_in != ASDR_STREAM_FAIL && seen_lo != ASDR_STREAM_FAIL && seen_in >= b2 && seen_lo >= b2) {
          const LoEntry *ln = a.lo_ring + ((blk + 1) % ASDR_LO_RING);
          const float *lp = ln->c + kF, *xp = a.xch_a + ((size_t)ch * ASDR_STREAM_DEPTH + (size_t)((blk + 1) % ASDR_STREAM_DEPTH)) * (2 * ASDR_N) + kF;
          r2n_key = ld_sc1_v4(reinterpret_cast<const float *>(ln));
#pragma unroll
          for (int m = 0; m < 4; ++m) { r2n_c4[m] = ld_sc1_v4(lp + 32 * m); r2n_s4[m] = ld_sc1_v4(lp + ASDR_N + 32 * m); r2n_vi[m] = ld_sc1_v4(xp + 32 * m); r2n_vq[m] = ld_sc1_v4(xp + ASDR_N + 32 * m); }
          r2_pref = true;
        }
      }
#ifndef ASDR_UPAR_IDL_EARLY
#define ASDR_UPAR_IDL_EARLY 1
#endif
      constexpr bool IDL_EARLY = (ROLE == 2) || (UPAR && ASDR_UPAR_IDL_EARLY != 0);
      if (IDL_EARLY && is_ssb) {
#pragma unroll
        for (int m = 0; m < 4; ++m) load4(hi_ring + (hs ^ 1u) * 128 + 32 * m, idl + 4 * m);
      }
      constexpr int FIR_NE = (ROLE == 2) ? 8 / (FIR_HELPERS + 1) : 8;
      v2f acc2[FIR_NE];
#pragma unroll
      for (int e = 0; e < FIR_NE; ++e) acc2[e] = (v2f){0.0f, 0.0f};
      if (ROLE == 2) __syncthreads();
      if constexpr (MW && WAVES == 4 && ASDR_MW_FIR_RING != 0 && ASDR_FIR_TAPS_IN_VGPRS == 0) { if (ABL_ON(ABL_HIL) && is_ssb) hilbert_fir_ring(L, k0 >> 1, acc2); }
      else if (ABL_ON(ABL_HIL) && is_ssb) hilbert_fir<0, FIR_NE>(L, k0 >> 1, acc2);
      if (ROLE == 2) __syncthreads(); else WAVE_SYNC();
      TL(9);
      if (!IDL_EARLY && is_ssb) {
#pragma unroll
        for (int m = 0; m < 4; ++m) {
#if ASDR_NT_LOADS >= 4
          load4_nt(hi_ring + (hs ^ 1u) * 128 + 32 * m, idl + 4 * m);
#else
          load4(hi_ring + (hs ^ 1u) * 128 + 32 * m, idl + 4 * m);
#endif
        }
      }
      if (is_ssb) {
#pragma unroll
        for (int e = 0; e < FIR_NE; e += 2) *reinterpret_cast<float4 *>(L + W1 + k0 + 2 * e) = make_float4(acc2[e][0], acc2[e][1], acc2[e + 1][0], acc2[e + 1][1]);
      }
      if (ROLE == 2) __syncthreads(); else WAVE_SYNC();
      }
      if (is_ssb) {
        const uint32_t sgn = sub_q ? 0x80000000u : 0u;
#pragma unroll
        for (int m = 0; m < 4; ++m) {
          float qh[4], au[4];
          load4(L + W1 + kF + 32 * m, qh);
#pragma unroll
          for (int j = 0; j < 4; ++j) au[j] = idl[4 * m + j] + __uint_as_float(__float_as_uint(qh[j]) ^ sgn);
          store4(L + W0 + kF + 32 * m, au);
          TAP4(ASDR_TAP_MIX_I, m, idl + 4 * m); TAP4(ASDR_TAP_MIX_Q, m, qh);
        }
      }
    }

    if (ABL_ON(ABL_ENV) && __any(do_env)) {
      WAVE_SYNC();
      {
        const int iq = pl_iq, st = pl_st;
        const bool do_env_p = PLB ? (__builtin_amdgcn_ds_bpermute(pl_c << 5, do_env ? 1 : 0) != 0) : do_env;
        float sv[4];
        ChanSmall *const Simg = Sp;
        const float4 s4 = *reinterpret_cast<const float4 *>(&Simg->img_state[iq][4 * st]);
        sv[0] = s4.x; sv[1] = s4.y; sv[2] = s4.z; sv[3] = s4.w;
// ... 1082 lines not shown
  return hipGetLastError() == hipSuccess ? 0 : -1;
}
extern "C" int asdr_stream_capacity(int device, int *compute_units, int fir_helpers) {
  int per_cu = 0;
  hipDeviceProp_t prop;
  if (hipGetDeviceProperties(&prop, device) != hipSuccess) return -1;
  if ((fir_helpers == 3 ? hipOccupancyMaxActiveBlocksPerMultiprocessor(&per_cu, asdr_stream_kernel_h3, 256, 0)
                        : hipOccupancyMaxActiveBlocksPerMultiprocessor(&per_cu, asdr_stream_kernel, 128, 0)) != hipSuccess) return -1;
  if (compute_units) *compute_units = prop.multiProcessorCount;
  return per_cu * prop.multiProcessorCount;
}

template <bool RESTORE>
__device__ __forceinline__ void stream_snapshot_body(const UpdateArgs &a, uint4 *snap) {
  if (RESTORE && *a.stream_err == 0u) return;
  const int t = threadIdx.x;
  for (int j = 0; j < 8; ++j) {
    const int slot = (int)blockIdx.x * 8 + j;
    if (slot >= a.n_sched) return;
    const int ch = (a.direct_ch0 >= 0) ? a.direct_ch0 + slot : a.sched[slot].ch;
    if (ch >= a.n_channels) continue;
    uint4 *dst = snap + (size_t)slot * (ASDR_SNAP_BYTES / 16);
    for (int p = t; p < ASDR_SNAP_BYTES / 16; p += 256) {
      uint4 *row; int q = p;
      if (q < 28) row = reinterpret_cast<uint4 *>(a.small + ch);
      else if ((q -= 28) < 96) row = reinterpret_cast<uint4 *>(a.nb_hist + (size_t)ch * 768);
      else if ((q -= 96) < ASDR_NB_MASK_ROW / 16) row = reinterpret_cast<uint4 *>(a.nb_mask + (size_t)ch * ASDR_NB_MASK_ROW);
      else if ((q -= ASDR_NB_MASK_ROW / 16) < 64) row = reinterpret_cast<uint4 *>(a.hil_q + (size_t)ch * 256);
      else if ((q -= 64) < 64) row = reinterpret_cast<uint4 *>(a.hil_i + (size_t)ch * 256);
      else { q -= 64; row = a.audio_prev ? reinterpret_cast<uint4 *>(a.audio_prev + (size_t)ch * 128) : nullptr; }
      if (row == nullptr) continue;
      if (RESTORE) row[q] = dst[p]; else dst[p] = row[q];
    }
  }
}
extern "C" __global__ __launch_bounds__(256) void asdr_stream_snapshot_kernel(UpdateArgs a, uint4 *snap) { stream_snapshot_body<false>(a, snap); }
extern "C" __global__ __launch_bounds__(256) void asdr_stream_restore_kernel(UpdateArgs a, uint4 *snap) { stream_snapshot_body<true>(a, snap); }
extern "C" __global__ void asdr_stream_ack_kernel(uint32_t *err) {
  if (threadIdx.x == 0 && blockIdx.x == 0 && err[0] != 0u) { err[1] += 1u; err[0] = 0u; }
}
extern "C" int asdr_launch_stream_snapshot(const UpdateArgs *a, void *snap, int restore, hipStream_t stream) {
  const int groups = a->n_sched / 8;
  if (groups <= 0) return 0;
  if (restore) ASDR_LAUNCH(asdr_stream_restore_kernel, dim3(groups), dim3(256), 0, stream, *a, reinterpret_cast<uint4 *>(snap));
  else ASDR_LAUNCH(asdr_stream_snapshot_kernel, dim3(groups), dim3(256), 0, stream, *a, reinterpret_cast<uint4 *>(snap));
  return hipGetLastError() == hipSuccess ? 0 : -1;
}
extern "C" int asdr_launch_stream_ack(uint32_t *err, hipStream_t stream) {
  ASDR_LAUNCH(asdr_stream_ack_kernel, dim3(1), dim3(64), 0, stream, err);
  return hipGetLastError() == hipSuccess ? 0 : -1;
}

extern "C" __global__ void asdr_reset_kernel(UpdateArgs a, const uint32_t *reset_bits, int first_row, int n_rows) {
  if ((int)blockIdx.x >= n_rows) return;
  const int ch = first_row + blockIdx.x;
  const uint32_t r = reset_bits[ch];
  if (!r) return;
  const int t = threadIdx.x;
  ChanSmall *S = a.small + ch;
  const bool all = r & ASDR_R_ALL;
  if (all) {
    uint32_t *w = reinterpret_cast<uint32_t *>(S);
    for (int i = t; i < (int)(sizeof(ChanSmall) / 4); i += 128) w[i] = 0u;
    a.hil_i[(size_t)ch * 256 + t] = 0.0f; a.hil_i[(size_t)ch * 256 + 128 + t] = 0.0f;
    a.hil_q[(size_t)ch * 256 + t] = 0.0f; a.hil_q[(size_t)ch * 256 + 128 + t] = 0.0f;
    if (a.audio_prev != nullptr) a.audio_prev[(size_t)ch * 128 + t] = 0.0f;
  }
  __syncthreads();
  if (all && t == 0) { S->nb_avg = 10.0f; S->status = ASDR_S_AGC_ACTIVE; }
  if (all || (r & ASDR_R_IF)) { if (t < 32) (&S->if_state[0][0])[t] = 0.0f; }
  if (all || (r & ASDR_R_IMG)) { if (t < 32) (&S->img_state[0][0])[t] = 0.0f; }
  if (all || (r & ASDR_R_AF)) { if (t < 16) S->af_state[t] = 0.0f; }
  if (all || (r & ASDR_R_NB)) {
    for (int i = t; i < 768; i += 128) a.nb_hist[(size_t)ch * 768 + i] = 0;
    for (int i = t; i < ASDR_NB_MASK_ROW; i += 128) a.nb_mask[(size_t)ch * ASDR_NB_MASK_ROW + i] = 1;
    if (t < 6) (&S->nb_gain[0][0])[t] = 0.0f;
  }
  if (all || (r & ASDR_R_ALS)) {
    a.als_x[(size_t)ch * 256 + t] = 0.0f; a.als_x[(size_t)ch * 256 + 128 + t] = 0.0f;
    a.als_w[(size_t)ch * 128 + t] = 0.0f;
  }
}

extern "C" int asdr_launch_update(const UpdateArgs *a, int variant, int uniform, hipStream_t stream) {
  const int n_waves = a->n_sched / 8;
  if (n_waves <= 0) return 0;
  if (variant == ASDR_KERNEL_ALS || (variant == ASDR_KERNEL_SAM_ALS && a->xch_sam == nullptr)) { if (uniform) ASDR_LAUNCH(asdr_update_kernel_als, dim3(n_waves), dim3(64), 0, stream, *a); else ASDR_LAUNCH(asdr_update_kernel_als_mixed, dim3(n_waves), dim3(64), 0, stream, *a); }
  else if (variant == ASDR_KERNEL_ALS_SMALL && uniform == 2) {
    ASDR_LAUNCH(asdr_als_pre_kernel, dim3(n_waves), dim3(64), 0, stream, *a);
    ASDR_LAUNCH(asdr_als_kernel, dim3(n_waves), dim3(64), 0, stream, *a);
  }
  else if (variant == ASDR_KERNEL_ALS_SMALL) { if (uniform && ASDR_ONEBLK && ASDR_ONEBLK_ALS && a->n_blocks == 1 && a->run_if == nullptr) ASDR_LAUNCH(asdr_update_kernel_als_small_one, dim3(n_waves), dim3(64), 0, stream, *a); else if (uniform) ASDR_LAUNCH(asdr_update_kernel_als_small, dim3(n_waves), dim3(64), 0, stream, *a); else ASDR_LAUNCH(asdr_update_kernel_als_small_mixed, dim3(n_waves), dim3(64), 0, stream, *a); }
  else if ((variant == ASDR_KERNEL_SAM || variant == ASDR_KERNEL_SAM_ALS) && a->xch_sam != nullptr) {
    if (uniform) ASDR_LAUNCH(asdr_sam_pre_kernel_uniform, dim3(n_waves), dim3(64), 0, stream, *a);
    else ASDR_LAUNCH(asdr_sam_pre_kernel, dim3(n_waves), dim3(64), 0, stream, *a);
    ASDR_LAUNCH(asdr_sam_pll_kernel, dim3((a->n_sched + ASDR_PLL_LANES - 1) / ASDR_PLL_LANES), dim3(64), 0, stream, *a);
    if (variant == ASDR_KERNEL_SAM_ALS) {
      if (uniform) ASDR_LAUNCH(asdr_sam_post_als_kernel_uniform, dim3(n_waves), dim3(64), 0, stream, *a);
      else ASDR_LAUNCH(asdr_sam_post_als_kernel, dim3(n_waves), dim3(64), 0, stream, *a);
    } else {
      if (uniform) ASDR_LAUNCH(asdr_sam_post_kernel_uniform, dim3(n_waves), dim3(64), 0, stream, *a);
      else ASDR_LAUNCH(asdr_sam_post_kernel, dim3(n_waves), dim3(64), 0, stream, *a);
    }
  }
  else if (variant == ASDR_KERNEL_SAM) ASDR_LAUNCH(asdr_update_kernel_sam, dim3((n_waves + ASDR_SAM_WAVES - 1) / ASDR_SAM_WAVES), dim3(64 * ASDR_SAM_WAVES), 0, stream, *a);
  else {
    static int mw_on = -1, mw_min = ASDR_MW_MIN_WAVES, c16_on = ASDR_C16, c16_min = ASDR_C16_MIN_WAVES, c16_pad = 0;
    if (mw_on < 0) {
      const char *e = getenv("ASDR_MW"); mw_on = e ? atoi(e) : ASDR_MW; const char *m = getenv("ASDR_MW_MIN_WAVES"); if (m) mw_min = atoi(m);
      const char *c = getenv("ASDR_C16"); if (c) c16_on = atoi(c); const char *cm = getenv("ASDR_C16_MIN_WAVES"); if (cm) c16_min = atoi(cm);
      const char *cp = getenv("ASDR_C16_PAD"); if (cp) c16_pad = atoi(cp);
    }
    const uint32_t dm = a->direct_mode;
    const bool ssb_class = dm == ASDR_USBmode || dm == ASDR_LSBmode || dm == ASDR_CW_USBmode || dm == ASDR_CW_LSBmode || dm == ASDR_WSPRmode;
    if (uniform && c16_on && a->n_blocks == 1 && a->run_if == nullptr && a->direct_ch0 >= 0 && a->taps == nullptr && ssb_class && n_waves >= c16_min)
      ASDR_LAUNCH(asdr_update_kernel_c16, dim3(n_waves), dim3(64), (size_t)c16_pad, stream, *a);
    else
    if (uniform && mw_on && a->n_blocks == 1 && a->run_if == nullptr && a->direct_ch0 >= 0 && n_waves >= mw_min && a->uni_valid)
      ASDR_LAUNCH(asdr_update_kernel_mw_u, dim3((n_waves + ASDR_MW_WAVES - 1) / ASDR_MW_WAVES), dim3(64 * ASDR_MW_WAVES), 0, stream, *a);
    else
    if (uniform && mw_on && a->n_blocks == 1 && a->run_if == nullptr && a->direct_ch0 >= 0 && n_waves >= mw_min)
      ASDR_LAUNCH(asdr_update_kernel_mw, dim3((n_waves + ASDR_MW_WAVES - 1) / ASDR_MW_WAVES), dim3(64 * ASDR_MW_WAVES), 0, stream, *a);
    else
    if (uniform && ASDR_ONEBLK && a->n_blocks == 1 && a->run_if == nullptr) ASDR_LAUNCH(asdr_update_kernel_one, dim3(n_waves), dim3(64), 0, stream, *a);
    else if (uniform) ASDR_LAUNCH(asdr_update_kernel, dim3(n_waves), dim3(64), 0, stream, *a);
    else ASDR_LAUNCH(asdr_update_kernel_mixed, dim3(n_waves), dim3(64), 0, stream, *a);
  }
  return hipGetLastError() == hipSuccess ? 0 : -1;
}

extern "C" __global__ void asdr_als_stage_seed_kernel(UpdateArgs a, int ch0, int n) {
  const int c = (int)blockIdx.x, t = (int)threadIdx.x;
  if (c >= n) return;
  const size_t ch = (size_t)(ch0 + c);
  a.als_stage[ch * (ASDR_ALS_STAGE_SLOTS * ASDR_N) + a.als_stage_prev * ASDR_N + t] = a.als_x[ch * (2 * ASDR_N) + ((a.als_phase & 1u) ^ 1u) * ASDR_N + t];
}
extern "C" int asdr_launch_als_role(const UpdateArgs *a, int role, hipStream_t stream) {
  const int n_waves = a->n_sched / 8;
  if (n_waves <= 0) return 0;
  if (role == 2) ASDR_LAUNCH(asdr_sam_pre_loop_kernel_uniform, dim3(n_waves), dim3(64), 0, stream, *a);
  else if (role == 3) ASDR_LAUNCH(asdr_als_back_loop_kernel, dim3(n_waves), dim3(64), 0, stream, *a);
  else if (role == 0 && a->n_blocks > 1) ASDR_LAUNCH(asdr_als_pre_loop_kernel, dim3(n_waves), dim3(64), 0, stream, *a);
  else if (role == 0) ASDR_LAUNCH(asdr_als_pre_kernel, dim3(n_waves), dim3(64), 0, stream, *a);
  else ASDR_LAUNCH(asdr_als_kernel, dim3(n_waves), dim3(64), 0, stream, *a);
  return hipGetLastError() == hipSuccess ? 0 : -1;
}
extern "C" int asdr_launch_als_stage_seed(const UpdateArgs *a, int ch0, int n, hipStream_t stream) {
  if (n <= 0) return 0;
  ASDR_LAUNCH(asdr_als_stage_seed_kernel, dim3(n), dim3(ASDR_N), 0, stream, *a, ch0, n);
  return hipGetLastError() == hipSuccess ? 0 : -1;
}

extern "C" int asdr_launch_sam_role(const UpdateArgs *a, int variant, int uniform, int role, hipStream_t stream) {
  const int n_waves = a->n_sched / 8;
  if (n_waves <= 0) return 0;
  if (a->n_blocks > 1 || a->sam_sets > 1u) {
    if (!uniform || variant != ASDR_KERNEL_SAM) return -1;
    if (role == 0) ASDR_LAUNCH(asdr_sam_pre_loop_kernel_uniform, dim3(n_waves), dim3(64), 0, stream, *a);
    else if (role == 1) ASDR_LAUNCH(asdr_sam_pll_kernel, dim3((a->n_sched + ASDR_PLL_LANES - 1) / ASDR_PLL_LANES), dim3(64), 0, stream, *a);
    else ASDR_LAUNCH(asdr_sam_post_loop_kernel_uniform, dim3(n_waves), dim3(64), 0, stream, *a);
    return hipGetLastError() == hipSuccess ? 0 : -1;
  }
  if (role == 0) {
    if (uniform) ASDR_LAUNCH(asdr_sam_pre_kernel_uniform, dim3(n_waves), dim3(64), 0, stream, *a);
    else ASDR_LAUNCH(asdr_sam_pre_kernel, dim3(n_waves), dim3(64), 0, stream, *a);
  } else if (role == 1) {
    ASDR_LAUNCH(asdr_sam_pll_kernel, dim3((a->n_sched + ASDR_PLL_LANES - 1) / ASDR_PLL_LANES), dim3(64), 0, stream, *a);
  } else if (variant == ASDR_KERNEL_SAM_ALS) {
    if (uniform) ASDR_LAUNCH(asdr_sam_post_als_kernel_uniform, dim3(n_waves), dim3(64), 0, stream, *a);
    else ASDR_LAUNCH(asdr_sam_post_als_kernel, dim3(n_waves), dim3(64), 0, stream, *a);
  } else {
    if (uniform) ASDR_LAUNCH(asdr_sam_post_kernel_uniform, dim3(n_waves), dim3(64), 0, stream, *a);
    else ASDR_LAUNCH(asdr_sam_post_kernel, dim3(n_waves), dim3(64), 0, stream, *a);
  }
  return hipGetLastError() == hipSuccess ? 0 : -1;
}

extern "C" __global__ void asdr_spin_kernel(unsigned long long ticks) {
  const unsigned long long t0 = __builtin_amdgcn_s_memrealtime();
  while (__builtin_amdgcn_s_memrealtime() - t0 < ticks) __builtin_amdgcn_s_sleep(8);
}
extern "C" int asdr_launch_spin(unsigned long long ticks, hipStream_t stream) {
  ASDR_LAUNCH(asdr_spin_kernel, dim3(1), dim3(64), 0, stream, ticks);
  return hipGetLastError() == hipSuccess ? 0 : -1;
}

extern "C" int asdr_launch_reset(const UpdateArgs *a, const uint32_t *d_reset_bits, int first_row, int n_rows, hipStream_t stream) {
  ASDR_LAUNCH(asdr_reset_kernel, dim3(n_rows), dim3(128), 0, stream, *a, d_reset_bits, first_row, n_rows);
  return hipGetLastError() == hipSuccess ? 0 : -1;
}
```

include/asdr.h:

```cpp
#ifndef ASDR_H_
#define ASDR_H_

#include <stddef.h>
#include <stdint.h>

#ifdef __cplusplus
extern "C" {
#endif

#define ASDR_BLOCK_SAMPLES 128
#define ASDR_ALL (-1)
#define ASDR_NO_DEVICE (-1)

enum { ASDR_LSBmode = 0, ASDR_USBmode = 1, ASDR_CW_LSBmode = 2, ASDR_CW_USBmode = 3, ASDR_AMmode = 4,
       ASDR_SAMmode = 5, ASDR_WSPRmode = 6 };
enum { ASDR_audioAM = 0, ASDR_audioCW = 1, ASDR_audioWSPR = 2, ASDR_audio2100 = 3, ASDR_audio2300 = 4,
       ASDR_audio2500 = 5, ASDR_audio2700 = 6, ASDR_audio2900 = 7, ASDR_audio3100 = 8, ASDR_audio3300 = 9,
       ASDR_audioBypass = 10 };
enum { ASDR_AGCoff = 0, ASDR_AGCfast = 1, ASDR_AGCmedium = 2, ASDR_AGCslow = 3 };

typedef struct asdr_batch asdr_batch_t;

asdr_batch_t *asdr_create(int n_channels, int device);
void asdr_destroy(asdr_batch_t *b);
const char *asdr_last_error(void);
int asdr_n_channels(const asdr_batch_t *b);

asdr_batch_t *asdr_create_sharded(int n_channels, int n_shards, const int *devices);
int asdr_n_shards(const asdr_batch_t *b);
asdr_batch_t *asdr_shard(asdr_batch_t *b, int shard);
int asdr_shard_first_channel(const asdr_batch_t *b, int shard);
int asdr_shard_device(const asdr_batch_t *b, int shard);

int asdr_update(asdr_batch_t *b, const int16_t *I, const int16_t *Q, int16_t *out, int n_blocks);
void *asdr_host_alloc(size_t bytes);
void asdr_host_free(void *p);
int asdr_host_register(void *p, size_t bytes);
int asdr_host_unregister(void *p);
int asdr_set_host_chunks(asdr_batch_t *b, int chunks);
int asdr_host_path_info(asdr_batch_t *b, int out[2]);
int asdr_host_autopin(int on);
void asdr_host_autopin_clear(void);
int asdr_host_autopin_info(long out[4]);
int asdr_debug_host_plan(asdr_batch_t *b, int chunks, int *bound, int *need_in, int *last_part);
int asdr_debug_part_slots(asdr_batch_t *b, int part, int parts, int *out);
int asdr_debug_schedule(asdr_batch_t *b, int *channels, int cap);
int asdr_update_device(asdr_batch_t *b, const int16_t *dI, const int16_t *dQ, int16_t *dOut, int n_blocks,
                       void *stream);
int asdr_update_device_strided(asdr_batch_t *b, const int16_t *dI, const int16_t *dQ, int16_t *dOut, int n_blocks,
                               long in_stride_blocks, long out_stride_blocks, void *stream);
#define ASDR_STREAM_BATCH ((void *)(intptr_t)-1)
int asdr_lanes_overlap_probe(asdr_batch_t *b);
int asdr_set_pool_priority(int level);
int asdr_lanes_enabled(asdr_batch_t *b);
int asdr_order_after(asdr_batch_t *b, void *stream);
int asdr_order_before(asdr_batch_t *b, void *stream);
long asdr_lane_calls(asdr_batch_t *b);
long asdr_sam_role_calls(asdr_batch_t *b);
long asdr_sam_chunk_calls(asdr_batch_t *b);
long asdr_als_role_calls(asdr_batch_t *b);
int asdr_set_lanes(asdr_batch_t *b, int on, int min_waves);
int asdr_synchronize(asdr_batch_t *b);

int asdr_capture_open(asdr_batch_t *b, long capacity_blocks);
int asdr_capture_close(asdr_batch_t *b);
long asdr_capture_capacity(const asdr_batch_t *b);
long asdr_capture_position(const asdr_batch_t *b);
int asdr_capture_rewind(asdr_batch_t *b);
int16_t *asdr_capture_device_ptr(asdr_batch_t *b);
int asdr_capture_update_device(asdr_batch_t *b, const int16_t *dI, const int16_t *dQ, int n_blocks,
                               long in_stride_blocks, void *stream);
int asdr_capture_read(asdr_batch_t *b, int ch, long first_block, long n_blocks, int16_t *host_out);

void asdr_init(asdr_batch_t *b, int ch);
void asdr_setMute(asdr_batch_t *b, int ch, int muted);
int asdr_getMute(asdr_batch_t *b, int ch);
void asdr_setInputGain(asdr_batch_t *b, int ch, float gain);
void asdr_setIQgainBalance(asdr_batch_t *b, int ch, float balance);
void asdr_setOutputGain(asdr_batch_t *b, int ch, float gain);
float asdr_setDemodMode(asdr_batch_t *b, int ch, int mode);
int16_t asdr_getDemodMode(asdr_batch_t *b, int ch);
float asdr_getTuningOffset(asdr_batch_t *b, int ch);
float asdr_getBPFlower(asdr_batch_t *b, int ch);
float asdr_getBPFupper(asdr_batch_t *b, int ch);

void asdr_enableAudioFilter(asdr_batch_t *b, int ch);
void asdr_disableAudioFilter(asdr_batch_t *b, int ch);
void asdr_setAudioFilter(asdr_batch_t *b, int ch, int filter);
int asdr_getAudioFilter(asdr_batch_t *b, int ch);

void asdr_enableALSfilter(asdr_batch_t *b, int ch);
void asdr_disableALSfilter(asdr_batch_t *b, int ch);
void asdr_setALSfilterNotch(asdr_batch_t *b, int ch);
void asdr_setALSfilterPeak(asdr_batch_t *b, int ch);
void asdr_setALSfilterAdaptive(asdr_batch_t *b, int ch);
void asdr_setALSfilterStatic(asdr_batch_t *b, int ch);
void asdr_setALSfilterParams(asdr_batch_t *b, int ch, unsigned int m, float lambda, float delay);
int asdr_ALSfilterIsEnabled(asdr_batch_t *b, int ch);
int asdr_ALSfilterIsNotch(asdr_batch_t *b, int ch);
int asdr_ALSfilterIsPeak(asdr_batch_t *b, int ch);
int asdr_ALSfilterIsAdaptive(asdr_batch_t *b, int ch);

void asdr_enableAGC(asdr_batch_t *b, int ch);
void asdr_disableAGC(asdr_batch_t *b, int ch);
int asdr_AGCisEnabled(asdr_batch_t *b, int ch);
int asdr_AGCisActive(asdr_batch_t *b, int ch);
void asdr_setAGCthreshold(asdr_batch_t *b, int ch, float db);
void asdr_setAGCslope(asdr_batch_t *b, int ch, float slope);
void asdr_setAGCmode(asdr_batch_t *b, int ch, int mode);
void asdr_setAGCkneeWidth(asdr_batch_t *b, int ch, float db);
void asdr_setAGCattackTime(asdr_batch_t *b, int ch, float ms);
void asdr_setAGCreleaseTime(asdr_batch_t *b, int ch, float ms);
void asdr_setAGChangTime(asdr_batch_t *b, int ch, float ms);
void asdr_setAGCstaticGain(asdr_batch_t *b, int ch, float gain);
float asdr_getAGCthreshold(asdr_batch_t *b, int ch);
float asdr_getAGCslope(asdr_batch_t *b, int ch);
float asdr_getAGCkneeWidth(asdr_batch_t *b, int ch);
float asdr_getAGCattack(asdr_batch_t *b, int ch);
float asdr_getAGCrelease(asdr_batch_t *b, int ch);
float asdr_getAAGalphaAttack(asdr_batch_t *b, int ch);
float asdr_getAGCbetaAttack(asdr_batch_t *b, int ch);
float asdr_getAGCalphaRelease(asdr_batch_t *b, int ch);
float asdr_getAGCbetaRelease(asdr_batch_t *b, int ch);
float asdr_getAGClookup(asdr_batch_t *b, int ch, int i);
float asdr_getAGCstaticGain(asdr_batch_t *b, int ch);
float asdr_getAMcarrierLevel(asdr_batch_t *b, int ch);

void asdr_enableNoiseBlanker(asdr_batch_t *b, int ch);
void asdr_disableNoiseBlanker(asdr_batch_t *b, int ch);
void asdr_setNoiseBlankerThreshold(asdr_batch_t *b, int ch, float ratio);
void asdr_setNoiseBlankerThresholdDb(asdr_batch_t *b, int ch, float db);
int asdr_NoiseBlankerisEnabled(asdr_batch_t *b, int ch);
int asdr_NoiseBlankerDetection(asdr_batch_t *b, int ch);

float asdr_getSAMfrequency(asdr_batch_t *b, int ch);
int asdr_getSAMphaseLockStatus(asdr_batch_t *b, int ch);

int asdr_read_status(asdr_batch_t *b, int32_t *agc_active, int32_t *nb_detected, int32_t *sam_locked,
                     float *sam_frequency, float *am_carrier);
enum { ASDR_TAP_SCALED_I = 0, ASDR_TAP_SCALED_Q, ASDR_TAP_NB_I, ASDR_TAP_NB_Q, ASDR_TAP_IF_I, ASDR_TAP_IF_Q,
// ... 40 lines not shown
```

Before: 87840.

## Alternate workgroup order across launches and keep state-ring stores cache-resident

Adds an optional mode, switched on by an environment variable or a new API call, that reverses the workgroup-to-channel mapping on every other launch of the plain uniform one-block kernels. The aim is for the workgroups that start first to touch the channels whose state was written last and so is still in L2. Independently of that flag, those plain kernels now write their noise-blanker history and Hilbert ring state with ordinary stores instead of nontemporal ones, chosen at compile time, so the next block can hit that state in cache. The cost is extra cache pressure from the state traffic, which may evict other data. New counters and Python bindings expose the mode and how many launches were reversed.

```diff
diff --git a/audiosdr_amd/binding.py b/audiosdr_amd/binding.py
--- a/audiosdr_amd/binding.py
+++ b/audiosdr_amd/binding.py
@@ -52,7 +52,7 @@
             "asdr_capture_device_ptr", "asdr_capture_update_device", "asdr_capture_read",
             "asdr_create_sharded", "asdr_n_shards", "asdr_shard", "asdr_shard_first_channel", "asdr_shard_device",
             "asdr_host_alloc", "asdr_host_free", "asdr_host_register", "asdr_host_unregister", "asdr_set_host_chunks",
-            "asdr_host_path_info", "asdr_stream_pipeline_alloc_failures", "asdr_set_launch_split", "asdr_order_after", "asdr_order_before", "asdr_lane_calls", "asdr_sam_role_calls", "asdr_sam_chunk_calls", "asdr_als_role_calls", "asdr_set_lanes"] +
+            "asdr_host_path_info", "asdr_stream_pipeline_alloc_failures", "asdr_set_launch_split", "asdr_order_after", "asdr_order_before", "asdr_lane_calls", "asdr_sam_role_calls", "asdr_sam_chunk_calls", "asdr_als_role_calls", "asdr_set_lanes", "asdr_set_alternate_order", "asdr_reversed_launches"] +
            ["asdr_" + n for n in _SETTERS_VOID + _SETTERS_F + _SETTERS_I + _GETTERS_F + _GETTERS_I])
 
 _lib = None
@@ -194,6 +194,9 @@
         L.asdr_lanes_overlap_probe.argtypes = [vp]; L.asdr_lanes_overlap_probe.restype = _i
         L.asdr_lanes_enabled.argtypes = [vp]; L.asdr_lanes_enabled.restype = _i
         L.asdr_stream_pipeline_headroom_refusals.argtypes = [vp]; L.asdr_stream_pipeline_headroom_refusals.restype = C.c_long
+    if path is None or hasattr(L, "asdr_set_alternate_order"):
+        L.asdr_set_alternate_order.argtypes = [vp, _i]; L.asdr_set_alternate_order.restype = _i
+        L.asdr_reversed_launches.argtypes = [vp]; L.asdr_reversed_launches.restype = C.c_long
     if path is None:
         _lib = L
     return L
@@ -264,6 +267,12 @@
     def stream_pipeline_headroom_refusals(self):
         return int(self._L.asdr_stream_pipeline_headroom_refusals(self._h))
 
+    def set_alternate_order(self, on=True):
+        self._chk(self._L.asdr_set_alternate_order(self._h, 1 if on else 0))
+
+    def reversed_launches(self):
+        return int(self._L.asdr_reversed_launches(self._h))
+
     def set_lanes(self, on=True, min_waves=0):
         self._chk(self._L.asdr_set_lanes(self._h, 1 if on else 0, int(min_waves)))
 
diff --git a/audiosdr_amd/csrc/asdr_device.h b/audiosdr_amd/csrc/asdr_device.h
--- a/audiosdr_amd/csrc/asdr_device.h
+++ b/audiosdr_amd/csrc/asdr_device.h
@@ -137,7 +137,7 @@
   ChainConsts k;
   ChanParams uni;
   uint32_t uni_valid;
-  uint32_t pad_uni_;
+  uint32_t wg_reverse;
 } UpdateArgs;
 #define ASDR_ALS_STAGE_SLOTS 32
 #define ASDR_ALS_CHUNK 8
diff --git a/audiosdr_amd/csrc/asdr_host.cpp b/audiosdr_amd/csrc/asdr_host.cpp
--- a/audiosdr_amd/csrc/asdr_host.cpp
+++ b/audiosdr_amd/csrc/asdr_host.cpp
@@ -49,6 +49,7 @@
 extern "C" int asdr_kernels_upload_tables(void);
 namespace { void autopin_batch_created(); void autopin_batch_gone(); }
 extern "C" int asdr_launch_update(const UpdateArgs *a, int variant, int uniform, hipStream_t stream);
+extern "C" int asdr_launch_update_ordered(const UpdateArgs *a, int variant, int uniform, hipStream_t stream, int *reversed);
 extern "C" int asdr_launch_sam_role(const UpdateArgs *a, int variant, int uniform, int role, hipStream_t stream);
 extern "C" int asdr_launch_als_role(const UpdateArgs *a, int role, hipStream_t stream);
 extern "C" int asdr_launch_als_stage_seed(const UpdateArgs *a, int ch0, int n, hipStream_t stream);
@@ -292,6 +293,9 @@
   long stat_stream_headroom_refusals = 0;
   long stat_stream_alloc_failures = 0;
   uint32_t lo_parity = 0;
+  uint32_t wg_parity = 0;
+  bool alternate_order = false;
+  long stat_reversed_launches = 0;
   uint32_t nb_phase = 0;
   uint32_t als_phase = 0;
   ChainConsts k{};
@@ -842,6 +846,7 @@
   b->sam_split_min = getenv("ASDR_SAM_SPLIT_MIN") ? atoi(getenv("ASDR_SAM_SPLIT_MIN")) : ASDR_SAM_SPLIT_MIN_CHANNELS;
   b->stream_pipeline = getenv("ASDR_NO_STREAM_PIPELINE") == nullptr;
   b->uniform_params = getenv("ASDR_NO_UNIFORM_PARAMS") == nullptr;
+  b->alternate_order = getenv("ASDR_ALTERNATE_ORDER") != nullptr && getenv("ASDR_NO_ALTERNATE_ORDER") == nullptr;
   b->als_split_min = getenv("ASDR_ALS_SPLIT_MIN") ? atoi(getenv("ASDR_ALS_SPLIT_MIN")) : 0x7fffffff;
   if (getenv("ASDR_LAUNCH_SPLIT")) b->launch_split = std::max(1, std::min(atoi(getenv("ASDR_LAUNCH_SPLIT")), 8));
   if (getenv("ASDR_LAUNCH_SPLIT_MIN_WAVES")) b->launch_split_min_waves = std::max(8, atoi(getenv("ASDR_LAUNCH_SPLIT_MIN_WAVES")));
@@ -1173,9 +1178,14 @@
     b->nb_phase = (b->nb_phase + (uint32_t)(n_blocks % 3)) % 3u;
     b->als_phase = (b->als_phase + (uint32_t)n_blocks) & 1u;
     b->lo_parity ^= 1u;
+    b->wg_parity ^= (uint32_t)(n_blocks & 1);
     return 0;
   }
   const int n_launch = per_block ? n_blocks : 1;
+  auto order_bit = [&](int kind, int uniform, int direct_ch0, int lb) -> uint32_t {
+    if (!b->alternate_order || kind != ASDR_KERNEL_PLAIN || !uniform || direct_ch0 < 0 || !(per_block || n_blocks == 1)) return 0u;
+    return (b->wg_parity ^ (uint32_t)lb) & 1u;
+  };
   float *const taps = a.taps;
   if (e0 && part == 0) HIPCHK(hipEventRecord(e0, stream));
   if (use_lanes) {
@@ -1206,6 +1216,7 @@
           if (su.uniform && b->kind_direct[su.kind]) { const SlotInfo &s0 = b->sched[su.first]; al.direct_ch0 = s0.ch + lo; al.direct_mode = s0.mode; al.direct_flags = s0.flags; al.direct_lo = s0.lo; set_uni(b, al, s0.ch); }
           al.lo_cache = b->d_lo + (size_t)(1 + (l % ASDR_LANES)) * 2 * ASDR_LO_ENTRIES;
           al.lo_write = 1u;
+          al.wg_reverse = order_bit(su.kind, su.uniform, al.direct_ch0, 0);
           al.lo_writer_bit = ASDR_LO_WRITER_LANE(l % ASDR_LANES);
           if (sam_split && (su.kind == ASDR_KERNEL_SAM || su.kind == ASDR_KERNEL_SAM_ALS)) set_sam_rows(al, su.kind, first, 0);
           const int form = (als_split && su.kind == ASDR_KERNEL_ALS_SMALL && su.uniform) ? 2 : su.uniform;
@@ -1214,8 +1225,11 @@
             al.nb_phase = (b->nb_phase + (uint32_t)(lb % 3)) % 3u;
             al.als_phase = (b->als_phase + (uint32_t)lb) & 1u;
             al.lo_parity = b->lo_parity ^ (uint32_t)(lb & 1);
+            al.wg_reverse = order_bit(su.kind, su.uniform, al.direct_ch0, lb);
           }
-          if (asdr_launch_update(&al, su.kind, form, ls) != 0) return fail("update kernel launch failed");
+          int rev = 0;
+          if (asdr_launch_update_ordered(&al, su.kind, form, ls, &rev) != 0) return fail("update kernel launch failed");
+          b->stat_reversed_launches += rev;
         }
       }
     }
@@ -1226,6 +1240,7 @@
     b->nb_phase = (b->nb_phase + (uint32_t)(n_blocks % 3)) % 3u;
     b->als_phase = (b->als_phase + (uint32_t)n_blocks) & 1u;
     b->lo_parity ^= (uint32_t)(n_launch & 1);
+    b->wg_parity ^= (uint32_t)(n_launch & 1);
     return 0;
   }
   struct Item { int sub, first, slots; };
@@ -1382,6 +1397,7 @@
         a.direct_ch0 = s0.ch + (first - subs[i].first); a.direct_mode = s0.mode; a.direct_flags = s0.flags; a.direct_lo = s0.lo; set_uni(b, a, s0.ch);
         if (first != subs[i].first) a.lo_write = 0u;
       }
+      a.wg_reverse = order_bit(subs[i].kind, subs[i].uniform, a.direct_ch0, per_block ? lb : 0);
       const bool sam3 = sam_split && (subs[i].kind == ASDR_KERNEL_SAM || subs[i].kind == ASDR_KERNEL_SAM_ALS);
       if (sam3) set_sam_rows(a, subs[i].kind, first, sam_roles ? (lb & 1) : 0);
       const int form = (als_split && subs[i].kind == ASDR_KERNEL_ALS_SMALL && subs[i].uniform) ? 2 : subs[i].uniform;
@@ -1396,7 +1412,9 @@
         HIPCHK(hipEventRecord(b->ev_role[4 + pa], stream));
         continue;
       }
-      if (asdr_launch_update(&a, subs[i].kind, form, s) != 0) return fail("update kernel launch failed");
+      int rev = 0;
+      if (asdr_launch_update_ordered(&a, subs[i].kind, form, s, &rev) != 0) return fail("update kernel launch failed");
+      b->stat_reversed_launches += rev;
       if (it != main_item) HIPCHK(hipEventRecord(b->ev_join[n_aux - 1], s));
     }
     for (int j = 0; j < n_aux; j++) HIPCHK(hipStreamWaitEvent(stream, b->ev_join[j], 0));
@@ -1410,6 +1428,7 @@
   b->nb_phase = (b->nb_phase + (uint32_t)(n_blocks % 3)) % 3u;
   b->als_phase = (b->als_phase + (uint32_t)n_blocks) & 1u;
   b->lo_parity ^= (uint32_t)(parity_launches & 1);
+  b->wg_parity ^= (uint32_t)(n_launch & 1);
   return 0;
 }
 
@@ -1864,6 +1883,18 @@
   HIPCHK(hipStreamWaitEvent(b->stream, b->ev_fork, 0));
   return 0;
 }
+int asdr_set_alternate_order(asdr_batch_t *b, int on) {
+  if (!b) return fail("null batch");
+  if (is_sharded(b)) { for (asdr_batch *sh : b->shards) sh->alternate_order = on != 0; return 0; }
+  b->alternate_order = on != 0;
+  return 0;
+}
+
+long asdr_reversed_launches(asdr_batch_t *b) {
+  if (is_sharded(b)) { long t = 0; for (asdr_batch *sh : b->shards) t += sh->stat_reversed_launches; return t; }
+  return b ? b->stat_reversed_launches : -1;
+}
+
 long asdr_lane_calls(asdr_batch_t *b) {
   if (is_sharded(b)) { long t = 0; for (asdr_batch *sh : b->shards) t += sh->stat_lane_calls; return t; }
   return b ? b->stat_lane_calls : -1;
diff --git a/audiosdr_amd/csrc/asdr_kernels.hip b/audiosdr_amd/csrc/asdr_kernels.hip
--- a/audiosdr_amd/csrc/asdr_kernels.hip
+++ b/audiosdr_amd/csrc/asdr_kernels.hip
@@ -422,6 +422,11 @@
   const i4v tv = {v.x, v.y, v.z, v.w};
   __builtin_nontemporal_store(tv, reinterpret_cast<i4v *>(p));
 }
+#ifndef ASDR_STATE_POLICY
+#define ASDR_STATE_POLICY 1
+#endif
+template <bool PLAIN> __device__ __forceinline__ void store4_state(float *p, const float *v) { if constexpr (PLAIN) store4(p, v); else store4_nt(p, v); }
+template <bool PLAIN> __device__ __forceinline__ void store_int4_state(int4 *p, int4 v) { if constexpr (PLAIN) *p = v; else store_int4_nt(p, v); }
 __device__ __forceinline__ void store4e(float *p, const float *v) { *reinterpret_cast<float4 *>(p) = make_float4(v[0], v[2], v[4], v[6]); }
 __device__ __forceinline__ void store8(float *p, const float *v) {
   float4 *q = reinterpret_cast<float4 *>(p);
@@ -941,6 +946,9 @@
 #ifndef ASDR_MW_ROT
 #define ASDR_MW_ROT 0
 #endif
+  constexpr bool ORDERED = (ROLE == 0) && !HAS_ALS && !HAS_SAM && UNIFORM && ONEBLK_ && (STRIDE == ASDR_STRIDE);
+  constexpr bool ST_PLAIN = ORDERED && (ASDR_STATE_POLICY >= 1), LD_PLAIN = ORDERED && (ASDR_STATE_POLICY >= 2);
+  const int wg_l = (ORDERED && a.wg_reverse != 0u) ? (int)(gridDim.x - 1u - blockIdx.x) : (int)blockIdx.x;
   const uint32_t mw_b = blockIdx.x;
   const uint32_t mw_rot = (ASDR_MW_ROT == 0) ? mw_b : (ASDR_MW_ROT == 1) ? (mw_b >> 3) : (ASDR_MW_ROT == 2) ? ((mw_b >> 3) + (mw_b >> 8)) :
                           (ASDR_MW_ROT == 3) ? ((mw_b * 0x9E3779B1u) >> 30) : (ASDR_MW_ROT == 4) ? ((mw_b >> 3) % 3u) : (mw_b >> 5);
@@ -964,8 +972,8 @@
     }
   };
   constexpr int MWX = 16;
-  auto mw_channel = [&](int q) -> int { const int sidx = (int)blockIdx.x * (8 * WAVES) + q; return (sidx < a.n_sched) ? a.direct_ch0 + sidx : a.n_channels; };
-  const int wave_g = STREAM ? (int)blockIdx.x % a.stream_waves : (int)blockIdx.x * WAVES + wave;
+  auto mw_channel = [&](int q) -> int { const int sidx = wg_l * (8 * WAVES) + q; return (sidx < a.n_sched) ? a.direct_ch0 + sidx : a.n_channels; };
+  const int wave_g = STREAM ? wg_l % a.stream_waves : wg_l * WAVES + wave;
   float *const lds = lds_wg + wave * 8 * STRIDE;
   const int lane = threadIdx.x & 63, c8 = lane >> 3, s8_ = lane & 7;
 #ifndef ASDR_MW_SINE_LDS
@@ -1090,7 +1098,7 @@
     const int k0 = 16 * s8, kA = 8 * s8, kF = 4 * s8;
     const bool lead = (s8 == 0);
 #ifdef ASDR_TIMELINE
-    const int tl_wg = ((int)blockIdx.x == 0) ? 0 : (((int)blockIdx.x == 683) ? 1 : (((int)blockIdx.x == 1365) ? 2 : (((int)blockIdx.x == 2047) ? 3 : -1)));
+    const int tl_wg = (wg_l == 0) ? 0 : ((wg_l == 683) ? 1 : ((wg_l == 1365) ? 2 : ((wg_l == 2047) ? 3 : -1)));
     const int tl_slot = STREAM ? ((wave_g == 0) ? 2 * (3 + ROLE) + (blk & 1) : -1)
                                : (MW ? ((tl_wg < 0) ? -1 : 4 * tl_wg + wave)
                                      : ((wave_g == 0) ? 0 : ((wave_g == 2731) ? 1 : ((wave_g == 5461) ? 2 : ((wave_g == 8191) ? 3 : -1)))));
@@ -1182,7 +1190,8 @@
       const int4 *old4 = reinterpret_cast<const int4 *>(hist + ns * 256 + kA), *mid4 = reinterpret_cast<const int4 *>(hist + ns_mid * 256 + kA);
 #if ASDR_NT_LOADS >= 2
       rmi[0].v = mid4[0]; rmi[1].v = mid4[8]; rmq[0].v = mid4[16]; rmq[1].v = mid4[24];
-      roi[0].v = load_int4_nt(old4); roi[1].v = load_int4_nt(old4 + 8); roq[0].v = load_int4_nt(old4 + 16); roq[1].v = load_int4_nt(old4 + 24);
+      if constexpr (LD_PLAIN) { roi[0].v = old4[0]; roi[1].v = old4[8]; roq[0].v = old4[16]; roq[1].v = old4[24]; }
+      else { roi[0].v = load_int4_nt(old4); roi[1].v = load_int4_nt(old4 + 8); roq[0].v = load_int4_nt(old4 + 16); roq[1].v = load_int4_nt(old4 + 24); }
 #else
       rmi[0].v = mid4[0]; rmi[1].v = mid4[8]; rmq[0].v = mid4[16]; rmq[1].v = mid4[24];
       roi[0].v = old4[0]; roi[1].v = old4[8]; roq[0].v = old4[16]; roq[1].v = old4[24];
@@ -1248,7 +1257,7 @@
       const bool own_tail = (s8 >= 1);
       if (C16 && nb_en) {
         int4 *ni = reinterpret_cast<int4 *>(hist + ns_new * 256 + kA);
-        store_int4_nt(ni, ri[0].v); store_int4_nt(ni + 8, ri[1].v); store_int4_nt(ni + 16, rq[0].v); store_int4_nt(ni + 24, rq[1].v);
+        store_int4_state<ST_PLAIN>(ni, ri[0].v); store_int4_state<ST_PLAIN>(ni + 8, ri[1].v); store_int4_state<ST_PLAIN>(ni + 16, rq[0].v); store_int4_state<ST_PLAIN>(ni + 24, rq[1].v);
         if (lead) { S->nb_gain[ns_new][0] = gain_i; S->nb_gain[ns_new][1] = gain_q; }
       }
       const bool unit_ring = UNIT_OK && __all(g_oi == 1.0f && g_oq == 1.0f && (!nb_en || (g_mi == 1.0f && g_mq == 1.0f)));
@@ -1318,7 +1327,7 @@
       if (nb_en && !C16) {
         int4 *ni = reinterpret_cast<int4 *>(hist + ns_new * 256 + kA);
 #ifndef ASDR_TEMPORAL_RINGS
-        store_int4_nt(ni, ri[0].v); store_int4_nt(ni + 8, ri[1].v); store_int4_nt(ni + 16, rq[0].v); store_int4_nt(ni + 24, rq[1].v);
+        store_int4_state<ST_PLAIN>(ni, ri[0].v); store_int4_state<ST_PLAIN>(ni + 8, ri[1].v); store_int4_state<ST_PLAIN>(ni + 16, rq[0].v); store_int4_state<ST_PLAIN>(ni + 24, rq[1].v);
 #else
         ni[0] = ri[0].v; ni[8] = ri[1].v; ni[16] = rq[0].v; ni[24] = rq[1].v;
 #endif
@@ -1818,7 +1827,7 @@
     if constexpr (HAS_SAM && WAVES > 1) {
       __syncthreads();
       if (ABL_ON(ABL_SAM) && wave == 0 && lane_i < 8 * WAVES) {
-        const int sj = (int)blockIdx.x * WAVES * 8 + lane_i;
+        const int sj = wg_l * WAVES * 8 + lane_i;
         int chj = a.n_channels; uint32_t modej = a.params[a.n_channels].mode;
         if (sj < a.n_sched) { const int4 sl = *reinterpret_cast<const int4 *>(a.sched + sj); chj = sl.x; modej = (uint32_t)sl.y; }
         if (modej == ASDR_SAMmode) {
@@ -1939,7 +1948,7 @@
               _Pragma("unroll")                                                                                                               \
               for (int j = 0; j < 4; ++j) qn[4 * m + j] = mq[j];                                                                              \
             } else { store4(L + W0 + kF + 32 * m, mi); store4(L + W1 + kF + 32 * m, mq); }                                                    \
-            store4_nt(hi_ring + hs * 128 + 32 * m, mi);                                                                                       \
+            store4_state<ST_PLAIN>(hi_ring + hs * 128 + 32 * m, mi);                                                                                       \
           }
         if (lo_hit || mix_uni) { C16_MIX_LOOP(true) }
         else {
@@ -1985,7 +1994,7 @@
           for (int j = 0; j < 4; ++j) qn[4 * m + j] = mq[j];
         } else { store4(L + W0 + kF + 32 * m, mi); store4(L + W1 + kF + 32 * m, mq); }
 #ifndef ASDR_TEMPORAL_RINGS
-        if (is_ssb) store4_nt(hi_ring + hs * 128 + 32 * m, mi);
+        if (is_ssb) store4_state<ST_PLAIN>(hi_ring + hs * 128 + 32 * m, mi);
 #else
         if (is_ssb) store4(hi_ring + hs * 128 + 32 * m, mi);
 #endif
@@ -2042,7 +2051,7 @@
             L[XP + 127 + k] = hq_m[4 * m + j];
             if (k < 63) L[XP + 255 + k] = qn[4 * m + j];
           }
-          store4_nt(hq_ring + hs * 128 + 32 * m, qn + 4 * m);
+          store4_state<ST_PLAIN>(hq_ring + hs * 128 + 32 * m, qn + 4 * m);
         }
         if (lead) S->hil_slot = hs ^ 1u;
         WAVE_SYNC();
@@ -2111,7 +2120,7 @@
           for (int j = 0; j < 4; ++j) L[XP + 255 + kF + 32 * m + j] = qn[4 * m + j];
           }
 #ifndef ASDR_TEMPORAL_RINGS
-          store4_nt(hq_ring + hs * 128 + 32 * m, qn + 4 * m);
+          store4_state<ST_PLAIN>(hq_ring + hs * 128 + 32 * m, qn + 4 * m);
 #else
           store4(hq_ring + hs * 128 + 32 * m, qn + 4 * m);
 #endif
@@ -3360,8 +3369,9 @@
   }
 }
 
-extern "C" int asdr_launch_update(const UpdateArgs *a, int variant, int uniform, hipStream_t stream) {
+extern "C" int asdr_launch_update_ordered(const UpdateArgs *a, int variant, int uniform, hipStream_t stream, int *reversed) {
   const int n_waves = a->n_sched / 8;
+  if (reversed) *reversed = 0;
   if (n_waves <= 0) return 0;
   if (variant == ASDR_KERNEL_ALS || (variant == ASDR_KERNEL_SAM_ALS && a->xch_sam == nullptr)) { if (uniform) ASDR_LAUNCH(asdr_update_kernel_als, dim3(n_waves), dim3(64), 0, stream, *a); else ASDR_LAUNCH(asdr_update_kernel_als_mixed, dim3(n_waves), dim3(64), 0, stream, *a); }
   else if (variant == ASDR_KERNEL_ALS_SMALL && uniform == 2) {
@@ -3395,17 +3405,21 @@
       ASDR_LAUNCH(asdr_update_kernel_c16, dim3(n_waves), dim3(64), (size_t)c16_pad, stream, *a);
     else
     if (uniform && mw_on && a->n_blocks == 1 && a->run_if == nullptr && a->direct_ch0 >= 0 && n_waves >= mw_min && a->uni_valid)
-      ASDR_LAUNCH(asdr_update_kernel_mw_u, dim3((n_waves + ASDR_MW_WAVES - 1) / ASDR_MW_WAVES), dim3(64 * ASDR_MW_WAVES), 0, stream, *a);
+    { if (reversed) *reversed = (int)a->wg_reverse;
+      ASDR_LAUNCH(asdr_update_kernel_mw_u, dim3((n_waves + ASDR_MW_WAVES - 1) / ASDR_MW_WAVES), dim3(64 * ASDR_MW_WAVES), 0, stream, *a); }
     else
     if (uniform && mw_on && a->n_blocks == 1 && a->run_if == nullptr && a->direct_ch0 >= 0 && n_waves >= mw_min)
-      ASDR_LAUNCH(asdr_update_kernel_mw, dim3((n_waves + ASDR_MW_WAVES - 1) / ASDR_MW_WAVES), dim3(64 * ASDR_MW_WAVES), 0, stream, *a);
+    { if (reversed) *reversed = (int)a->wg_reverse;
+      ASDR_LAUNCH(asdr_update_kernel_mw, dim3((n_waves + ASDR_MW_WAVES - 1) / ASDR_MW_WAVES), dim3(64 * ASDR_MW_WAVES), 0, stream, *a); }
     else
-    if (uniform && ASDR_ONEBLK && a->n_blocks == 1 && a->run_if == nullptr) ASDR_LAUNCH(asdr_update_kernel_one, dim3(n_waves), dim3(64), 0, stream, *a);
+    if (uniform && ASDR_ONEBLK && a->n_blocks == 1 && a->run_if == nullptr) { if (reversed) *reversed = (int)a->wg_reverse; ASDR_LAUNCH(asdr_update_kernel_one, dim3(n_waves), dim3(64), 0, stream, *a); }
     else if (uniform) ASDR_LAUNCH(asdr_update_kernel, dim3(n_waves), dim3(64), 0, stream, *a);
     else ASDR_LAUNCH(asdr_update_kernel_mixed, dim3(n_waves), dim3(64), 0, stream, *a);
   }
   return hipGetLastError() == hipSuccess ? 0 : -1;
 }
+
+extern "C" int asdr_launch_update(const UpdateArgs *a, int variant, int uniform, hipStream_t stream) { return asdr_launch_update_ordered(a, variant, uniform, stream, nullptr); }
 
 extern "C" __global__ void asdr_als_stage_seed_kernel(UpdateArgs a, int ch0, int n) {
   const int c = (int)blockIdx.x, t = (int)threadIdx.x;
diff --git a/include/asdr.h b/include/asdr.h
--- a/include/asdr.h
+++ b/include/asdr.h
@@ -56,6 +56,8 @@
 int asdr_order_after(asdr_batch_t *b, void *stream);
 int asdr_order_before(asdr_batch_t *b, void *stream);
 long asdr_lane_calls(asdr_batch_t *b);
+int asdr_set_alternate_order(asdr_batch_t *b, int on);
+long asdr_reversed_launches(asdr_batch_t *b);
 long asdr_sam_role_calls(asdr_batch_t *b);
 long asdr_sam_chunk_calls(asdr_batch_t *b);
 long asdr_als_role_calls(asdr_batch_t *b);
```

Result: faster. 89830 (median of 6 runs) (+2.3%).
